# aliftffd/ViT-vs-Raw-IQ

Measured on AMD Instinct MI355X. Metric: IQ frames/sec training (fwd+loss+bwd+clip+AdamW), higher is better.
Workload: dtype bf16; 1 GPU; ViT-Tiny/16 224x224 C=1 19cls (BASELINE configs[1]); config_id=B, per_gpu_batch=256, global_batch=256, parallelism=dp1, hipgraph=True

## Files before the change

### include/iqvit.h

```cpp
#ifndef IQVIT_H
#define IQVIT_H
#include <stddef.h>
#include <stdint.h>

#ifdef __cplusplus
extern "C" {
#endif

typedef void* iq_stream_t;

enum { IQ_STATUS_OK = 0, IQ_STATUS_ARG = 1, IQ_STATUS_UNSUPPORTED = 2, IQ_STATUS_LAUNCH = 3 };

typedef struct iq_dropout {
  uint64_t seed;
  uint32_t step;
  uint32_t site;
  float p;
  const uint32_t* step_dev;
} iq_dropout_t;
#define IQ_SITE_IMPAIR 0xFFFFFFFFu
#define IQ_SITE_SYNTH 0xFFFFFFFEu

int iq_ln_supported(int D);
int iq_ln_fwd(const void* z, const float* gamma, const float* beta, void* x, float* mean, float* rstd, int M, int D,
              float eps, iq_stream_t stream);
size_t iq_ln_bwd_ws_bytes(int D);
int iq_ln_bwd(const void* dx, const void* z, const float* mean, const float* rstd, const float* gamma, void* dz,
              void* dy, const iq_dropout_t* drop, float* dgamma, float* dbeta, float* ws, int accumulate, int M,
              int D, iq_stream_t stream);
int iq_ln_bwd_partial_rows(int M, int D);

typedef struct iq_epilogue {
  const float* bias;
  int relu;
  const float* pe;
  int tok, seq, cls_off;
  iq_dropout_t drop;
  const void* gate;
  int ldg;
  float gate_scale;
  const void* residual;
  int ldr;
} iq_epilogue_t;
int iq_gemm_bf16_nt(const void* A, int lda, const void* B, int ldb, void* C, int ldc, int M, int N, int K,
                    const iq_epilogue_t* epi, iq_stream_t stream);

int iq_gemm_ln_supported(int D, int K);
int iq_gemm_bf16_ln(const void* A, int lda, const void* W, int ldw, const float* bias, const void* residual, int ldr,
                    const iq_dropout_t* drop, const float* gamma, const float* beta, float eps, void* Z, void* X,
                    float* mean, float* rstd, int M, int D, int K, iq_stream_t stream);

int iq_gemm_lnbwd_supported(int D, int K);
int iq_gemm_lnbwd_partial_rows(int M);
int iq_gemm_bf16_lnbwd(const void* A, int lda, const void* Wt, int ldw, const void* residual, int ldr, const void* z,
                       const float* mean, const float* rstd, const float* gamma, const iq_dropout_t* drop, void* dz,
                       void* dy, float* partial, int M, int D, int K, iq_stream_t stream);

int iq_ffn_chain_supported(int S, int D, int F);
int iq_ffn_chain_bwd_partial_rows(int M);
size_t iq_ffn_chain_gate_bytes(int M, int F);
int iq_ffn_chain_bwd(const void* dO, const void* W2t, const void* gate_bits, float gate_scale, void* gH, const void* W1t,
                     const void* residual, const void* z1, const float* mean, const float* rstd, const float* gamma,
                     const iq_dropout_t* drop, void* dz, void* dy, float* partial, const void* Wot, void* dA, int frames, int S,
                     int D, int F, iq_stream_t stream);
int iq_qkv_dgrad_ffn_chain_bwd(const void* gQKV, const void* Wqkv_t, const void* residual0, const void* z2, const float* mean2,
                               const float* rstd2, const float* gamma2, const iq_dropout_t* drop2, void* dz2, void* dy2, float* partial2,
                               const void* W2t, const void* gate_bits, float gate_scale, void* gH, const void* W1t, const void* residual,
                               const void* z1, const float* mean, const float* rstd, const float* gamma, const iq_dropout_t* drop, void* dz,
                               void* dy, float* partial, const void* Wot, void* dA, int frames, int S, int D, int F, iq_stream_t stream);
int iq_ffn_chain_fwd(const void* X1, const void* W1, const float* b1, const iq_dropout_t* drop1, void* H, const void* W2,
                     const float* b2, const iq_dropout_t* drop2, const float* gamma, const float* beta, float eps, void* Z,
                     void* X, float* mean, float* rstd, void* gate_bits, int frames, int S, int D, int F, iq_stream_t stream);
int iq_attn_out_ffn_chain_fwd(const void* A, const void* Wo, const float* bo, const iq_dropout_t* drop0, const void* R,
                              const float* gamma1, const float* beta1, void* Z1, void* X1, float* mean1, float* rstd1,
                              const void* W1, const float* b1, const iq_dropout_t* drop1, void* H, const void* W2, const float* b2,
                              const iq_dropout_t* drop2, const float* gamma2, const float* beta2, float eps, void* Z2, void* X,
                              float* mean2, float* rstd2, void* gate_bits, const void* Wq, const float* bq, void* Yq, int frames,
                              int S, int D, int F, iq_stream_t stream);

size_t iq_wgrad_ws_bytes(int M, int N, int K);
int iq_gemm_bf16_wgrad(const void* dY, int ldy, const void* X, int ldx, float* dW, float* dbias, int M, int N, int K,
                       float* ws, size_t ws_bytes, int accumulate, iq_stream_t stream);

typedef struct iq_wgrad_problem {
  const void* dY;
  int ldy;
  const void* X;
  int ldx;
  float* dW;
  float* dbias;
  int N, K;
} iq_wgrad_problem_t;
typedef struct iq_reduce_seg {
  const float* partials;
  int rows;
  int64_t row_stride;
  float* out;
  int64_t n;
} iq_reduce_seg_t;
size_t iq_wgrad_grouped_ws_bytes(const iq_wgrad_problem_t* probs, int nprob, int M, int max_workgroups);
int iq_gemm_bf16_wgrad_grouped(const iq_wgrad_problem_t* probs, int nprob, int M, float* ws, size_t ws_bytes,
                               int accumulate, int max_workgroups, const iq_reduce_seg_t* extra, int nextra,
                               iq_stream_t stream);

#define IQ_REDUCE_JOB_SEGS 12
typedef struct iq_reduce_job_seg {
  const float* partials;
  float* out;
  int64_t n;
  int64_t stride;
  int rows;
  int blk0;
  int tall;
} iq_reduce_job_seg_t;
typedef struct iq_reduce_job {
  iq_reduce_job_seg_t seg[IQ_REDUCE_JOB_SEGS];
  int nseg;
  int nblk;
  int accumulate;
} iq_reduce_job_t;
int iq_gemm_bf16_wgrad_grouped_deferred(const iq_wgrad_problem_t* probs, int nprob, int M, float* ws, size_t ws_bytes,
                                        int accumulate, int max_workgroups, const iq_reduce_seg_t* extra, int nextra,
                                        iq_reduce_job_t* job, iq_stream_t stream);
int iq_reduce_job_run(const iq_reduce_job_t* job, iq_stream_t stream);
int iq_gemm_lnbwd_ride_workgroups(int M, int D, int K, int job_blocks);
int iq_gemm_bf16_lnbwd_ride(const void* A, int lda, const void* Wt, int ldw, const void* residual, int ldr, const void* z,
                            const float* mean, const float* rstd, const float* gamma, const iq_dropout_t* drop, void* dz,
                            void* dy, float* partial, int M, int D, int K, const iq_reduce_job_t* job, iq_stream_t stream);

int iq_attn_supported(int S, int dh);
int iq_attn_fwd(const void* qkv, void* out, float* lse, int B, int S, int H, int dh, iq_stream_t stream);
int iq_attn_bwd(const void* qkv, const void* out, const void* dout, const float* lse, void* dqkv, int B, int S, int H,
                int dh, iq_stream_t stream);
int iq_attn_fwd_masked(const void* qkv, void* out, float* lse, const uint8_t* mask, long mask_hstride, int B, int S,
                       int H, int dh, iq_stream_t stream);
int iq_attn_bwd_masked(const void* qkv, const void* out, const void* dout, const float* lse, void* dqkv,
                       const uint8_t* mask, long mask_hstride, int B, int S, int H, int dh, iq_stream_t stream);
int iq_attn_probs(const void* qkv, const float* lse, float* out, long out_bstride, int B, int S, int H, int dh,
                  int rows, int heads, iq_stream_t stream);
int iq_attn_grad_probs(const void* qkv, const float* lse, const void* dout, float* out, long out_bstride, int B, int S,
                       int H, int dh, int rows, int heads, int positive, iq_stream_t stream);
int iq_attn_relevance_step(const void* qkv, const float* lse, const void* dout, const float* r_in, float* r_out, int B,
                           int S, int H, int dh, iq_stream_t stream);

int iq_frames_preprocess(const float* raw, float* out, int n_frames, int len, int take, const float* stats,
                         iq_stream_t stream);
typedef struct iq_impair {
  float phase_lo, phase_hi;
  float cfo_lo, cfo_hi;
  int   rot90;
  int   conj;
  int   shift_max;
  float gain_db_lo, gain_db_hi;
  float snr_db_lo, snr_db_hi;
  uint64_t seed; uint32_t step;
  uint64_t frame_base;
} iq_impair_t;
int iq_frames_impair(const float* raw, float* out, float* drawn, int n_frames, int len, int take, const float* stats,
                     const iq_impair_t* imp, iq_stream_t stream);
#define IQ_SYNTH_MAX_CLASSES 128
#define IQ_SYNTH_MAX_SNRS 64
typedef struct iq_synth_class { int kind; int offset; int count; } iq_synth_class_t;
typedef struct iq_synth {
  const float* points;
  const iq_synth_class_t* classes; int n_classes;
  const float* snrs_db; int n_snrs;
  int balanced;
  uint64_t seed; uint32_t stream;
  uint64_t frame_base;
} iq_synth_t;
int iq_frames_synth(float* raw , int64_t* labels, float* snr ,
                    float* drawn ,
                    int32_t* symbols , int n_frames, int len, const iq_synth_t* par, iq_stream_t stream);
typedef struct iq_waveform {
  const float* points; const iq_synth_class_t* classes; int n_classes;
  const float* snrs_db; int n_snrs; int balanced;
  uint64_t seed; uint32_t stream; uint64_t frame_base;
  int sps;
  int span;
  int n_phase;
  int timing;
  const float* pulse;
  const int32_t* fpulse;
  int n_taps;
  float los;
  float tap_sigma[8];
} iq_waveform_t;
int iq_frames_waveform(float* raw , int64_t* labels, float* snr, float* drawn ,
                       int32_t* symbols , float* taps , int n_frames, int len,
                       const iq_waveform_t* par, iq_stream_t stream);
enum { IQ_RX_GIVEN = 0, IQ_RX_OERDER_MEYR = 1, IQ_RX_ENERGY = 2 };
typedef struct iq_receiver {
  int sps;
  int span;
  int n_frac;
  int mode;
  int normalise;
  const float* table;
  const int32_t* u;
} iq_receiver_t;
int iq_frames_receive(const float* raw , float* sym , float* est ,
                      float* energy , int n_frames, int len, const iq_receiver_t* par, iq_stream_t stream);
int iq_frames_receive_bwd(const float* dsym , const float* sym, const float* est, float* dx ,
                          int n_frames, int len, const iq_receiver_t* par, iq_stream_t stream);
typedef struct iq_spectrogram {
  int n_fft;
  int hop;
  int pad;
  int width;
  int mode;
  float inv_norm, floor, scale, shift;
} iq_spectrogram_t;
int iq_frames_spectrogram(const float* x , const float* table ,
                          float* out , int n_frames, int len, const iq_spectrogram_t* par,
                          iq_stream_t stream);
int iq_frames_spectrogram_bwd(const float* x, const float* table, const float* dout ,
                              float* dx , int n_frames, int len, const iq_spectrogram_t* par,
                              iq_stream_t stream);
typedef struct iq_cyclic {
  int n_fft;
  int hop;
  int pad;
  int columns;
  int kind;
  int mode;
  float inv_norm, floor, scale, shift;
} iq_cyclic_t;
int iq_frames_cyclic(const float* x , const float* table , const float* rot ,
                     float* out , int n_frames, int len, const iq_cyclic_t* par, iq_stream_t stream);
int iq_frames_cyclic_bwd(const float* x, const float* table, const float* rot, const float* dout ,
                         float* dx , int n_frames, int len, const iq_cyclic_t* par, iq_stream_t stream);
typedef struct iq_constellation {
  int height, width;
  int radius;
  int n_frac;
  int mode;
  float x_scale, x_off, y_scale, y_off;
  float inv_norm, floor, scale, shift;
} iq_constellation_t;
int iq_frames_constellation(const float* x , const float* table ,
                            float* out , int n_frames, int len, const iq_constellation_t* par,
                            iq_stream_t stream);
int iq_frames_constellation_bwd(const float* x, const float* table, const float* dout ,
                                float* dx , int n_frames, int len, const iq_constellation_t* par,
                                iq_stream_t stream);
enum { IQ_CR_GIVEN = 0, IQ_CR_ESTIMATE = 1 };
typedef struct iq_carrier {
  int order;
  int n1, n2;
  int k_max;
  int refine;
  int planar;
  int mode;
  const float* t1;
  const float* t2;
  const float* tw;
  const int32_t* fth;
} iq_carrier_t;
int iq_frames_carrier(const float* x, float* out, float* est , int32_t* fth_out ,
                      float* power , int n_frames, int len,
                      const iq_carrier_t* par, iq_stream_t stream);
int iq_frames_carrier_bwd(const float* dout, float* dx, int n_frames, int len, const iq_carrier_t* par, iq_stream_t stream);
enum { IQ_EQ_GIVEN = 0, IQ_EQ_CMA = 1 };
typedef struct iq_equaliser {
  int taps;
  int iters;
  int planar;
  int mode;
  float mu;
  float modulus;
  const float* w;
  const float* w0;
} iq_equaliser_t;
int iq_frames_equalise(const float* x, float* out, float* w_out , float* est , int n_frames,
                       int len, const iq_equaliser_t* par, iq_stream_t stream);
int iq_frames_equalise_bwd(const float* dout, float* dx, int n_frames, int len, const iq_equaliser_t* par, iq_stream_t stream);
enum { IQ_LIK_MAX = 0, IQ_LIK_MEAN = 1 };
typedef struct iq_likelihood {
  const float* points;
  const iq_synth_class_t* classes;
  int n_classes;
  const float* rot;
  int n_rot;
  int planar;
  int mode;
  const float* gain;
} iq_likelihood_t;
int iq_frames_likelihood(const float* x, const float* sigma2 , float* loglik ,
                         float* rot_ll , int* best_rot ,
                         int* pred , int n_frames, int len,
                         const iq_likelihood_t* par, iq_stream_t stream);
enum { IQ_EM_TABLE = 0, IQ_EM_GIVEN = 1 };
typedef struct iq_likelihood_em {
  const float* points;
  const iq_synth_class_t* classes;
  int n_classes;
  const float* starts;
  int n_starts;
  int iters;
  int planar;
  int mode;
  float f0;
  float floor;
  const float* h0;
  const float* v0;
} iq_likelihood_em_t;
int iq_frames_likelihood_em(const float* x, float* loglik , float* h , float* v ,
                            int* best_start , float* start_ll , int* pred ,
                            float* snr_db , int n_frames, int len, const iq_likelihood_em_t* par,
                            iq_stream_t stream);
int iq_frames_likelihood_bwd(const float* x, const float* sigma2 , const float* dloglik ,
                             const float* loglik , const float* rot_ll ,
                             const int* best_rot , float* dx , int n_frames, int len,
                             const iq_likelihood_t* par, iq_stream_t stream);
int iq_frames_likelihood_em_bwd(const float* x, const float* dloglik , const float* h ,
                                const float* v , float* dx , int n_frames, int len,
                                const iq_likelihood_em_t* par, iq_stream_t stream);
typedef struct iq_cumulants {
  int planar;
  const float* sigma2;
  const float* mu;
  const float* w;
  const float* bias;
  int n_classes;
} iq_cumulants_t;
int iq_frames_cumulants(const float* x, float* feat , float* mom ,
                        float* score , int* pred ,
                        int n_frames, int len, const iq_cumulants_t* par, iq_stream_t stream);
int iq_patchify(const float* src, void* patches, int kind, int B, int C, int H, int W, int p, int Kpad,
                iq_stream_t stream);
int iq_cls_rows(const float* cls, const float* pe, void* x0, int B, int S, int D, const iq_dropout_t* drop,
                iq_stream_t stream);
int iq_embed_bwd_gather(const void* dx0, void* demb, float* dcls, int B, int S, int tok, int D, int has_cls,
                        const iq_dropout_t* drop, int accumulate, iq_stream_t stream);
int iq_embed_dgrad(const void* demb, const void* w_bf16, int Kpad, float* dsrc, int kind, int B, int C, int H, int W, int p,
                   int D, iq_stream_t stream);
int iq_linf_step(float* x_adv, const float* grad, const float* x0, float alpha, float eps, float lo, float hi, size_t n,
                 iq_stream_t stream);

int iq_head_fwd(const void* x, const float* ln_g, const float* ln_b, const float* W, const float* b, float* featn,
                float* hstat, float* logits, int B, int S, int D, int K, int pool, iq_stream_t stream);
int iq_ce_fwd_bwd(const float* logits, const int64_t* labels, int B, int K, float smoothing, float denom,
                  float* loss_sum, int32_t* n_correct, float* dlogits, iq_stream_t stream);
int iq_head_bwd(const float* dlogits, const float* featn, const float* hstat, const float* ln_g, const float* ln_b,
                const float* W, float* dW, float* db, float* dln_g, float* dln_b, void* dx, int B, int S, int D, int K,
                int pool, int accumulate, iq_stream_t stream);

size_t iq_gradnorm_ws_bytes(size_t n);
int iq_gradnorm_sq(const float* g, size_t n, float grad_scale, float* ws, float* out, iq_stream_t stream);
int iq_adamw_step(float* p, const float* g, float* m, float* v, void* shadow_bf16, size_t n, float lr, float beta1,
                  float beta2, float eps, float weight_decay, int step, const float* gnorm_sq, float max_norm,
                  float grad_scale, const float* dyn, iq_stream_t stream);
int iq_counter_add(uint32_t* ctr_u32, uint32_t inc_u32, float* ctr_f32, float inc_f32, iq_stream_t stream);
int iq_cast_bf16(const float* src, void* dst, size_t n, iq_stream_t stream);
int iq_transpose_cast_bf16(const float* src, void* dst, int rows, int cols, iq_stream_t stream);

typedef struct iq_model_cfg {
  int kind;
  int in_channels;
  int img_h, img_w, patch;
  int seq_length, conv_k, use_cls;
  int num_classes, d_model, n_head, n_layers, ffn_hidden;
  float drop_prob;
} iq_model_cfg_t;

typedef struct iq_model iq_model_t;

int iq_model_create(const iq_model_cfg_t* cfg, iq_model_t** out);
void iq_model_destroy(iq_model_t* m);
const char* iq_model_last_error(const iq_model_t* m);
int iq_model_tokens(const iq_model_t* m);
size_t iq_model_param_floats(const iq_model_t* m);
int iq_model_param_entries(const iq_model_t* m);
int iq_model_param_entry(const iq_model_t* m, int i, char* name, int name_cap, size_t* offset, int* ndim, int* dims);
size_t iq_model_shadow_bytes(const iq_model_t* m);
size_t iq_model_workspace_bytes(const iq_model_t* m, int batch, int training);
int iq_model_bind(iq_model_t* m, float* params, float* grads, const float* pe, void* shadow);
int iq_model_bind_step_counter(iq_model_t* m, uint32_t* counter);
int iq_model_refresh_shadow(iq_model_t* m, iq_stream_t stream);
int iq_model_refresh_transposed(iq_model_t* m, iq_stream_t stream);
int iq_model_forward(iq_model_t* m, const float* src, int batch, void* workspace, size_t ws_bytes, int training,
                     uint64_t seed, uint32_t step, float* enc_out, float* logits, iq_stream_t stream);
int iq_model_backward(iq_model_t* m, const float* dlogits, const float* denc, int batch, void* workspace,
                      size_t ws_bytes, int accumulate, int stage_hi, int stage_lo, iq_stream_t stream);
int iq_model_grad_range(const iq_model_t* m, int stage_hi, int stage_lo, size_t* off, size_t* len);
#define IQ_BWD_PARAM_GRADS 1
int iq_model_backward_input(iq_model_t* m, const float* dlogits, const float* denc, int batch, void* workspace,
                            size_t ws_bytes, float* dsrc, int flags, iq_stream_t stream);
int iq_model_attention(iq_model_t* m, const void* workspace, size_t ws_bytes, int batch, int layer, int rows,
                       int heads, float* out, long out_bstride, iq_stream_t stream);
int iq_model_attention_rollout(iq_model_t* m, const void* workspace, size_t ws_bytes, int batch, float alpha,
                               float* out, iq_stream_t stream);
int iq_model_attention_relevance(iq_model_t* m, const float* dlogits, int batch, void* workspace, size_t ws_bytes,
                                 float* rel, float* const* maps, int rows, int heads, int positive, long out_bstride,
                                 iq_stream_t stream);

#define IQ_PROF_FAMILIES 8
int iq_prof_enable(int on);
int iq_prof_collect(double* ms, long long* count);
size_t iq_prof_kernels(char* out, size_t cap, int reset);

#ifdef __cplusplus
}
#endif
#endif
```

### vit-vs-raw-iq_amd/_native.py

```python
from __future__ import annotations

import ctypes as C
import os

_HERE = os.path.dirname(os.path.abspath(__file__))
LIB_PATH = os.environ.get("IQ_LIBIQVIT") or os.path.join(_HERE, "libiqvit.so")

BWD_PARAM_GRADS = 1

STATUS = {0: "ok", 1: "invalid argument", 2: "unsupported shape/configuration", 3: "HIP launch error"}


class IqError(RuntimeError):
    pass


class Dropout(C.Structure):
    _fields_ = [("seed", C.c_uint64), ("step", C.c_uint32), ("site", C.c_uint32), ("p", C.c_float),
                ("step_dev", C.c_void_p)]


class Impair(C.Structure):
    _fields_ = [("phase_lo", C.c_float), ("phase_hi", C.c_float), ("cfo_lo", C.c_float), ("cfo_hi", C.c_float),
                ("rot90", C.c_int), ("conj", C.c_int), ("shift_max", C.c_int), ("gain_db_lo", C.c_float),
                ("gain_db_hi", C.c_float), ("snr_db_lo", C.c_float), ("snr_db_hi", C.c_float), ("seed", C.c_uint64),
                ("step", C.c_uint32), ("frame_base", C.c_uint64)]


class SynthClass(C.Structure):
    _fields_ = [("kind", C.c_int), ("offset", C.c_int), ("count", C.c_int)]


class Synth(C.Structure):
    _fields_ = [("points", C.c_void_p), ("classes", C.POINTER(SynthClass)), ("n_classes", C.c_int),
                ("snrs_db", C.POINTER(C.c_float)), ("n_snrs", C.c_int), ("balanced", C.c_int), ("seed", C.c_uint64),
                ("stream", C.c_uint32), ("frame_base", C.c_uint64)]


class Waveform(C.Structure):
    _fields_ = [("points", C.c_void_p), ("classes", C.POINTER(SynthClass)), ("n_classes", C.c_int),
                ("snrs_db", C.POINTER(C.c_float)), ("n_snrs", C.c_int), ("balanced", C.c_int), ("seed", C.c_uint64),
                ("stream", C.c_uint32), ("frame_base", C.c_uint64), ("sps", C.c_int), ("span", C.c_int), ("n_phase", C.c_int),
                ("timing", C.c_int), ("pulse", C.c_void_p), ("fpulse", C.c_void_p), ("n_taps", C.c_int), ("los", C.c_float),
                ("tap_sigma", C.c_float * 8)]


class Receiver(C.Structure):
    _fields_ = [("sps", C.c_int), ("span", C.c_int), ("n_frac", C.c_int), ("mode", C.c_int), ("normalise", C.c_int),
                ("table", C.c_void_p), ("u", C.c_void_p)]


class Spectrogram(C.Structure):
    _fields_ = [("n_fft", C.c_int), ("hop", C.c_int), ("pad", C.c_int), ("width", C.c_int), ("mode", C.c_int),
                ("inv_norm", C.c_float), ("floor", C.c_float), ("scale", C.c_float), ("shift", C.c_float)]


class Constellation(C.Structure):
    _fields_ = [("height", C.c_int), ("width", C.c_int), ("radius", C.c_int), ("n_frac", C.c_int), ("mode", C.c_int),
                ("x_scale", C.c_float), ("x_off", C.c_float), ("y_scale", C.c_float), ("y_off", C.c_float),
                ("inv_norm", C.c_float), ("floor", C.c_float), ("scale", C.c_float), ("shift", C.c_float)]


class Carrier(C.Structure):
    _fields_ = [("order", C.c_int), ("n1", C.c_int), ("n2", C.c_int), ("k_max", C.c_int), ("refine", C.c_int),
                ("planar", C.c_int), ("mode", C.c_int), ("t1", C.c_void_p), ("t2", C.c_void_p), ("tw", C.c_void_p),
                ("fth", C.c_void_p)]


class Equaliser(C.Structure):
    _fields_ = [("taps", C.c_int), ("iters", C.c_int), ("planar", C.c_int), ("mode", C.c_int), ("mu", C.c_float),
                ("modulus", C.c_float), ("w", C.c_void_p), ("w0", C.c_void_p)]


class Likelihood(C.Structure):
    _fields_ = [("points", C.c_void_p), ("classes", C.POINTER(SynthClass)), ("n_classes", C.c_int), ("rot", C.c_void_p),
                ("n_rot", C.c_int), ("planar", C.c_int), ("mode", C.c_int), ("gain", C.c_void_p)]


class LikelihoodEm(C.Structure):
    _fields_ = [("points", C.c_void_p), ("classes", C.POINTER(SynthClass)), ("n_classes", C.c_int), ("starts", C.c_void_p),
                ("n_starts", C.c_int), ("iters", C.c_int), ("planar", C.c_int), ("mode", C.c_int), ("f0", C.c_float),
                ("floor", C.c_float), ("h0", C.c_void_p), ("v0", C.c_void_p)]


class Cumulants(C.Structure):
    _fields_ = [("planar", C.c_int), ("sigma2", C.c_void_p), ("mu", C.c_void_p), ("w", C.c_void_p), ("bias", C.c_void_p),
                ("n_classes", C.c_int)]


class Cyclic(C.Structure):
    _fields_ = [("n_fft", C.c_int), ("hop", C.c_int), ("pad", C.c_int), ("columns", C.c_int), ("kind", C.c_int),
                ("mode", C.c_int), ("inv_norm", C.c_float), ("floor", C.c_float), ("scale", C.c_float), ("shift", C.c_float)]


class Epilogue(C.Structure):
    _fields_ = [("bias", C.c_void_p), ("relu", C.c_int), ("pe", C.c_void_p), ("tok", C.c_int), ("seq", C.c_int),
                ("cls_off", C.c_int), ("drop", Dropout), ("gate", C.c_void_p), ("ldg", C.c_int),
                ("gate_scale", C.c_float), ("residual", C.c_void_p), ("ldr", C.c_int)]


class WgradProblem(C.Structure):
    _fields_ = [("dY", C.c_void_p), ("ldy", C.c_int), ("X", C.c_void_p), ("ldx", C.c_int), ("dW", C.c_void_p),
                ("dbias", C.c_void_p), ("N", C.c_int), ("K", C.c_int)]


class ReduceSeg(C.Structure):
    _fields_ = [("partials", C.c_void_p), ("rows", C.c_int), ("row_stride", C.c_int64), ("out", C.c_void_p),
                ("n", C.c_int64)]


class ReduceJobSeg(C.Structure):
    _fields_ = [("partials", C.c_void_p), ("out", C.c_void_p), ("n", C.c_int64), ("stride", C.c_int64), ("rows", C.c_int),
                ("blk0", C.c_int), ("tall", C.c_int)]


class ReduceJob(C.Structure):
    _fields_ = [("seg", ReduceJobSeg * 12), ("nseg", C.c_int), ("nblk", C.c_int), ("accumulate", C.c_int)]


class ModelCfg(C.Structure):
    _fields_ = [("kind", C.c_int), ("in_channels", C.c_int), ("img_h", C.c_int), ("img_w", C.c_int),
                ("patch", C.c_int), ("seq_length", C.c_int), ("conv_k", C.c_int), ("use_cls", C.c_int),
                ("num_classes", C.c_int), ("d_model", C.c_int), ("n_head", C.c_int), ("n_layers", C.c_int),
                ("ffn_hidden", C.c_int), ("drop_prob", C.c_float)]


_P, _I, _Z, _F = C.c_void_p, C.c_int, C.c_size_t, C.c_float
_U64, _U32 = C.c_uint64, C.c_uint32

SIGNATURES = {
    "iq_ln_supported": (_I, [_I]),
    "iq_ln_fwd": (_I, [_P, _P, _P, _P, _P, _P, _I, _I, _F, _P]),
    "iq_ln_bwd_ws_bytes": (_Z, [_I]),
    "iq_ln_bwd_partial_rows": (_I, [_I, _I]),
    "iq_ln_bwd": (_I, [_P, _P, _P, _P, _P, _P, _P, C.POINTER(Dropout), _P, _P, _P, _I, _I, _I, _P]),
    "iq_gemm_bf16_nt": (_I, [_P, _I, _P, _I, _P, _I, _I, _I, _I, C.POINTER(Epilogue), _P]),
    "iq_gemm_ln_supported": (_I, [_I, _I]),
    "iq_gemm_bf16_ln": (_I, [_P, _I, _P, _I, _P, _P, _I, C.POINTER(Dropout), _P, _P, _F, _P, _P, _P, _P, _I, _I, _I, _P]),
    "iq_gemm_lnbwd_supported": (_I, [_I, _I]),
    "iq_gemm_lnbwd_partial_rows": (_I, [_I]),
    "iq_gemm_bf16_lnbwd": (_I, [_P, _I, _P, _I, _P, _I, _P, _P, _P, _P, C.POINTER(Dropout), _P, _P, _P, _I, _I, _I, _P]),
    "iq_ffn_chain_supported": (_I, [_I, _I, _I]),
    "iq_ffn_chain_bwd_partial_rows": (_I, [_I]),
    "iq_ffn_chain_bwd": (_I, [_P, _P, _P, _F, _P, _P, _P, _P, _P, _P, _P, C.POINTER(Dropout), _P, _P, _P, _P, _P, _I, _I, _I, _I, _P]),
    "iq_qkv_dgrad_ffn_chain_bwd": (_I, [_P, _P, _P, _P, _P, _P, _P, C.POINTER(Dropout), _P, _P, _P,
                                        _P, _P, _F, _P, _P, _P, _P, _P, _P, _P, C.POINTER(Dropout), _P, _P, _P, _P, _P, _I, _I, _I, _I, _P]),
    "iq_ffn_chain_gate_bytes": (_Z, [_I, _I]),
    "iq_ffn_chain_fwd": (_I, [_P, _P, _P, C.POINTER(Dropout), _P, _P, _P, C.POINTER(Dropout), _P, _P, _F, _P, _P, _P, _P, _P, _I, _I,
                              _I, _I, _P]),
    "iq_attn_out_ffn_chain_fwd": (_I, [_P, _P, _P, C.POINTER(Dropout), _P, _P, _P, _P, _P, _P, _P,
                                       _P, _P, C.POINTER(Dropout), _P, _P, _P, C.POINTER(Dropout), _P, _P, _F, _P, _P, _P, _P, _P,
                                       _P, _P, _P, _I, _I, _I, _I, _P]),
    "iq_wgrad_ws_bytes": (_Z, [_I, _I, _I]),
    "iq_gemm_bf16_wgrad": (_I, [_P, _I, _P, _I, _P, _P, _I, _I, _I, _P, _Z, _I, _P]),
    "iq_wgrad_grouped_ws_bytes": (_Z, [_P, _I, _I, _I]),
    "iq_gemm_bf16_wgrad_grouped": (_I, [_P, _I, _I, _P, _Z, _I, _I, _P, _I, _P]),
    "iq_gemm_bf16_wgrad_grouped_deferred": (_I, [_P, _I, _I, _P, _Z, _I, _I, _P, _I, C.POINTER(ReduceJob), _P]),
    "iq_reduce_job_run": (_I, [C.POINTER(ReduceJob), _P]),
    "iq_gemm_bf16_lnbwd_ride": (_I, [_P, _I, _P, _I, _P, _I, _P, _P, _P, _P, C.POINTER(Dropout), _P, _P, _P, _I, _I, _I,
                                     C.POINTER(ReduceJob), _P]),
    "iq_gemm_lnbwd_ride_workgroups": (_I, [_I, _I, _I, _I]),
    "iq_attn_supported": (_I, [_I, _I]),
    "iq_attn_fwd": (_I, [_P, _P, _P, _I, _I, _I, _I, _P]),
    "iq_attn_bwd": (_I, [_P, _P, _P, _P, _P, _I, _I, _I, _I, _P]),
    "iq_attn_fwd_masked": (_I, [_P, _P, _P, _P, C.c_long, _I, _I, _I, _I, _P]),
    "iq_attn_bwd_masked": (_I, [_P, _P, _P, _P, _P, _P, C.c_long, _I, _I, _I, _I, _P]),
    "iq_attn_probs": (_I, [_P, _P, _P, C.c_long, _I, _I, _I, _I, _I, _I, _P]),
    "iq_attn_grad_probs": (_I, [_P, _P, _P, _P, C.c_long, _I, _I, _I, _I, _I, _I, _I, _P]),
    "iq_attn_relevance_step": (_I, [_P, _P, _P, _P, _P, _I, _I, _I, _I, _P]),
    "iq_frames_preprocess": (_I, [_P, _P, _I, _I, _I, C.POINTER(C.c_float), _P]),
    "iq_frames_impair": (_I, [_P, _P, _P, _I, _I, _I, C.POINTER(C.c_float), C.POINTER(Impair), _P]),
    "iq_frames_synth": (_I, [_P, _P, _P, _P, _P, _I, _I, C.POINTER(Synth), _P]),
    "iq_frames_waveform": (_I, [_P, _P, _P, _P, _P, _P, _I, _I, C.POINTER(Waveform), _P]),
    "iq_frames_receive": (_I, [_P, _P, _P, _P, _I, _I, C.POINTER(Receiver), _P]),
    "iq_frames_receive_bwd": (_I, [_P, _P, _P, _P, _I, _I, C.POINTER(Receiver), _P]),
    "iq_frames_spectrogram": (_I, [_P, _P, _P, _I, _I, C.POINTER(Spectrogram), _P]),
    "iq_frames_spectrogram_bwd": (_I, [_P, _P, _P, _P, _I, _I, C.POINTER(Spectrogram), _P]),
    "iq_frames_cyclic": (_I, [_P, _P, _P, _P, _I, _I, C.POINTER(Cyclic), _P]),
    "iq_frames_cyclic_bwd": (_I, [_P, _P, _P, _P, _P, _I, _I, C.POINTER(Cyclic), _P]),
    "iq_frames_constellation": (_I, [_P, _P, _P, _I, _I, C.POINTER(Constellation), _P]),
    "iq_frames_constellation_bwd": (_I, [_P, _P, _P, _P, _I, _I, C.POINTER(Constellation), _P]),
    "iq_frames_carrier": (_I, [_P, _P, _P, _P, _P, _I, _I, C.POINTER(Carrier), _P]),
    "iq_frames_carrier_bwd": (_I, [_P, _P, _I, _I, C.POINTER(Carrier), _P]),
    "iq_frames_equalise": (_I, [_P, _P, _P, _P, _I, _I, C.POINTER(Equaliser), _P]),
    "iq_frames_equalise_bwd": (_I, [_P, _P, _I, _I, C.POINTER(Equaliser), _P]),
    "iq_frames_likelihood": (_I, [_P, _P, _P, _P, _P, _P, _I, _I, C.POINTER(Likelihood), _P]),
    "iq_frames_likelihood_em": (_I, [_P, _P, _P, _P, _P, _P, _P, _P, _I, _I, C.POINTER(LikelihoodEm), _P]),
    "iq_frames_likelihood_bwd": (_I, [_P, _P, _P, _P, _P, _P, _P, _I, _I, C.POINTER(Likelihood), _P]),
    "iq_frames_likelihood_em_bwd": (_I, [_P, _P, _P, _P, _P, _I, _I, C.POINTER(LikelihoodEm), _P]),
    "iq_frames_cumulants": (_I, [_P, _P, _P, _P, _P, _I, _I, C.POINTER(Cumulants), _P]),
    "iq_patchify": (_I, [_P, _P, _I, _I, _I, _I, _I, _I, _I, _P]),
    "iq_cls_rows": (_I, [_P, _P, _P, _I, _I, _I, C.POINTER(Dropout), _P]),
    "iq_embed_bwd_gather": (_I, [_P, _P, _P, _I, _I, _I, _I, _I, C.POINTER(Dropout), _I, _P]),
    "iq_embed_dgrad": (_I, [_P, _P, _I, _P, _I, _I, _I, _I, _I, _I, _I, _P]),
    "iq_linf_step": (_I, [_P, _P, _P, _F, _F, _F, _F, _Z, _P]),
    "iq_head_fwd": (_I, [_P, _P, _P, _P, _P, _P, _P, _P, _I, _I, _I, _I, _I, _P]),
    "iq_ce_fwd_bwd": (_I, [_P, _P, _I, _I, _F, _F, _P, _P, _P, _P]),
    "iq_head_bwd": (_I, [_P, _P, _P, _P, _P, _P, _P, _P, _P, _P, _P, _I, _I, _I, _I, _I, _I, _P]),
    "iq_gradnorm_ws_bytes": (_Z, [_Z]),
    "iq_gradnorm_sq": (_I, [_P, _Z, _F, _P, _P, _P]),
    "iq_adamw_step": (_I, [_P, _P, _P, _P, _P, _Z, _F, _F, _F, _F, _F, _I, _P, _F, _F, _P, _P]),
    "iq_counter_add": (_I, [_P, _U32, _P, _F, _P]),
    "iq_cast_bf16": (_I, [_P, _P, _Z, _P]),
    "iq_transpose_cast_bf16": (_I, [_P, _P, _I, _I, _P]),
    "iq_model_create": (_I, [C.POINTER(ModelCfg), C.POINTER(_P)]),
    "iq_model_destroy": (None, [_P]),
    "iq_model_last_error": (C.c_char_p, [_P]),
    "iq_model_tokens": (_I, [_P]),
    "iq_model_param_floats": (_Z, [_P]),
    "iq_model_param_entries": (_I, [_P]),
    "iq_model_param_entry": (_I, [_P, _I, C.c_char_p, _I, C.POINTER(_Z), C.POINTER(_I), C.POINTER(_I)]),
    "iq_model_shadow_bytes": (_Z, [_P]),
    "iq_model_workspace_bytes": (_Z, [_P, _I, _I]),
    "iq_model_bind": (_I, [_P, _P, _P, _P, _P]),
    "iq_model_bind_step_counter": (_I, [_P, _P]),
    "iq_model_refresh_shadow": (_I, [_P, _P]),
    "iq_model_refresh_transposed": (_I, [_P, _P]),
    "iq_model_forward": (_I, [_P, _P, _I, _P, _Z, _I, _U64, _U32, _P, _P, _P]),
    "iq_model_backward": (_I, [_P, _P, _P, _I, _P, _Z, _I, _I, _I, _P]),
    "iq_model_grad_range": (_I, [_P, _I, _I, C.POINTER(_Z), C.POINTER(_Z)]),
    "iq_model_backward_input": (_I, [_P, _P, _P, _I, _P, _Z, _P, _I, _P]),
    "iq_model_attention": (_I, [_P, _P, _Z, _I, _I, _I, _I, _P, C.c_long, _P]),
    "iq_model_attention_rollout": (_I, [_P, _P, _Z, _I, _F, _P, _P]),
    "iq_model_attention_relevance": (_I, [_P, _P, _I, _P, _Z, _P, C.POINTER(_P), _I, _I, _I, C.c_long, _P]),
    "iq_prof_enable": (_I, [_I]),
    "iq_prof_collect": (_I, [C.POINTER(C.c_double), C.POINTER(C.c_longlong)]),
    "iq_prof_kernels": (_Z, [C.c_char_p, _Z, _I]),
}

_lib = None


def lib():
    global _lib
    if _lib is None:
        if not os.path.exists(LIB_PATH):
            raise IqError(
                f"{LIB_PATH} not found: the HIP extension is not built. Run "
                "`python -c 'import __graft_entry__ as g; g.build()'` (or `make -C vit-vs-raw-iq_amd/csrc`). "
                "There is no CPU fallback.")
        L = C.CDLL(LIB_PATH)
        for name, (res, args) in SIGNATURES.items():
            fn = getattr(L, name)
            fn.restype = res
            fn.argtypes = args
        _lib = L
    return _lib


def check(rc, what, model=None):
    if rc != 0:
        detail = ""
        if model is not None:
            msg = lib().iq_model_last_error(model)
            if msg:
                detail = ": " + msg.decode()
        raise IqError(f"{what} failed: {STATUS.get(rc, rc)}{detail}")


def ptr(t):
    return None if t is None else t.data_ptr()


def stream_handle():
    import torch
    return torch.cuda.current_stream().cuda_stream
```

### vit-vs-raw-iq_amd/csrc/ffn_chain.hip

```cpp
#include <stdlib.h>

#include <type_traits>

#include "common.h"
#include "iqvit.h"
#include "prof.h"

namespace {

constexpr int FC_CHUNK = 64, FC_NS = 3, FC_MAXW = 7;

struct FfnChainParams {
  const bf16* X1; const bf16* W1; const bf16* W2;
  const float* b1; const float* b2; const float* gamma; const float* beta;
  bf16* H; bf16* Z; bf16* X; float* mean; float* rstd;
  uint32_t* gate;
  int M, F;
  float eps;
  int drop1_on, drop2_on; IqRng rng1, rng2; uint32_t thresh1, thresh2; float dscale1, dscale2;
  const bf16* A0; const bf16* W0; const bf16* R0; const float* b0; const float* gamma0; const float* beta0;
  bf16* Z0; bf16* X1out; float* mean0; float* rstd0;
  int drop0_on; IqRng rng0; uint32_t thresh0; float dscale0;
  const bf16* Wq; const float* bq; bf16* Yq;
};

template <int CPR> __device__ __forceinline__ int fc_swz(int row, int ch) {
  return CPR == 16 ? (ch ^ (row & 15)) : CPR == 8 ? (ch ^ ((row >> 1) & 7)) : ((ch & ~7) | ((ch & 7) ^ ((row >> 1) & 7)));
}
template <int OFF>
__device__ __forceinline__ void lds_read128(bf16x8& dst, uint32_t addr) {
  asm volatile("ds_read_b128 %0, %1 offset:%2" : "=v"(dst) : "v"(addr), "n"(OFF));
}
#define FC_LGKM_WAIT(N)                                  \
  do {                                                   \
    asm volatile("s_waitcnt lgkmcnt(%0)" ::"n"(N) : "memory"); \
    __builtin_amdgcn_sched_barrier(0);                   \
  } while (0)

__device__ __forceinline__ int fc_kperm(int g) { return ((g & 1) << 1) | (g >> 1); }

template <int D, int NW, int RG, bool DROP1, int MODE>
__global__ __launch_bounds__(NW * 64, 2) void ffn_chain_fwd_kernel(const FfnChainParams p) {
  constexpr int RW = 16 * RG;
  constexpr bool PRE = MODE >= 1, POST = MODE == 2;
  constexpr int XCPR = D / 8;
  constexpr int KS1 = D / 32;
  constexpr int NT2 = D / 16, NP2 = NT2 / 2;
  constexpr int W1_BYTES = FC_CHUNK * D * 2, W2_BYTES = D * FC_CHUNK * 2, SLOT = W1_BYTES + W2_BYTES;
  constexpr int W1_PIECES = W1_BYTES / 1024, PIECES = SLOT / 1024;
  constexpr int PPW = (PIECES + NW - 1) / NW;
  static_assert(PPW + 8 * RG < 64, "counted vmcnt");
  extern __shared__ __attribute__((aligned(16))) unsigned char smem[];
  const int tid = threadIdx.x, lane = tid & 63;
  const int wave = __builtin_amdgcn_readfirstlane(tid >> 6);
  constexpr int nwave = NW;
  const int g = lane >> 4, c16 = lane & 15;
  const bool odd = (g & 1) != 0;
  const int F = p.F;
  const int nchunk = F / FC_CHUNK;
  const long row0 = ((long)blockIdx.x * nwave + wave) * RW;
  const bool have = row0 < p.M;

  auto issue_chunk = [&](int c) {
    unsigned char* slot = smem + (c % FC_NS) * SLOT;
    const char* base1 = reinterpret_cast<const char*>(p.W1 + (long)c * FC_CHUNK * D);
    const char* base2 = reinterpret_cast<const char*>(p.W2 + (long)c * FC_CHUNK);
    int ln = lane;
    asm volatile("" : "+v"(ln));
#pragma unroll
    for (int i = 0; i < PPW; ++i) {
      const int pc = min(wave + i * NW, PIECES - 1);
      const int lin = pc * 64 + ln;
      unsigned off;
      if (pc < W1_PIECES) {
        const int r = lin / XCPR, sl = lin - r * XCPR;
        const int q = fc_swz<XCPR>(r, sl);
        off = (unsigned)((r * D + ((q & ~3) | fc_kperm(q & 3)) * 8) * 2);
      } else {
        const int l2 = lin - W1_PIECES * 64;
        const int r = l2 >> 3, sl = l2 & 7;
        const int q = fc_swz<8>(r, sl);
        off = (unsigned)((r * F + ((q & ~3) | fc_kperm(q & 3)) * 8) * 2);
      }
      const char* base = pc < W1_PIECES ? base1 : base2;
      __builtin_amdgcn_global_load_lds((gbl_cvoid_t*)(base + off), (lds_void_t*)(slot + pc * 1024), 16, 0, 0);
    }
  };
  constexpr int NBQ = 3 * D / FC_CHUNK, NQ = (NBQ + 1) / 2;
  static_assert(2 * W1_BYTES == SLOT, "two projection blocks fill a ring slot");
  const int ntot = nchunk + (POST ? NQ : 0);
  auto issue_any = [&](int c) {
    if (!POST || c < nchunk) { issue_chunk(c); return; }
    const int q = c - nchunk;
    unsigned char* slot = smem + (c % FC_NS) * SLOT;
    int ln = lane;
    asm volatile("" : "+v"(ln));
#pragma unroll
    for (int i = 0; i < PPW; ++i) {
      const int pc = min(wave + i * NW, PIECES - 1);
      const int lin = pc * 64 + ln;
      const int r = lin / XCPR, sl = lin - r * XCPR;
      const int qq = fc_swz<XCPR>(r & 63, sl);
      const int grow = min(q * 2 * FC_CHUNK + r, 3 * D - 1);
      const unsigned off = (unsigned)((grow * D + ((qq & ~3) | fc_kperm(qq & 3)) * 8) * 2);
      __builtin_amdgcn_global_load_lds((gbl_cvoid_t*)(reinterpret_cast<const char*>(p.Wq) + off), (lds_void_t*)(slot + pc * 1024), 16, 0, 0);
    }
  };
  constexpr int NB0 = D / FC_CHUNK;
  if (PRE) {
    constexpr int PRE_PIECES = NB0 * W1_PIECES, PRE_PPW = (PRE_PIECES + NW - 1) / NW;
    static_assert(NB0 * W1_BYTES <= 2 * SLOT, "projection weight blocks fit ring slots 1 and 2");
#pragma unroll
    for (int i = 0; i < PRE_PPW; ++i) {
      const int pc = min(wave + i * NW, PRE_PIECES - 1);
      const int lin = pc * 64 + lane;
      const int r = lin / XCPR, sl = lin - r * XCPR;
      const int q = fc_swz<XCPR>(r & 63, sl);
      const unsigned off = (unsigned)((r * D + ((q & ~3) | fc_kperm(q & 3)) * 8) * 2);
      __builtin_amdgcn_global_load_lds((gbl_cvoid_t*)(reinterpret_cast<const char*>(p.W0) + off),
                                       (lds_void_t*)(smem + SLOT + pc * 1024), 16, 0, 0);
    }
  }
  issue_chunk(0);
  if (!PRE && ntot > 1) issue_any(1);

  bf16x8 xf[RG][KS1];
  {
    const bf16* src = PRE ? p.A0 : p.X1;
#pragma unroll
    for (int rg = 0; rg < RG; ++rg) {
      const long r = min(row0 + rg * 16 + c16, (long)p.M - 1);
#pragma unroll
      for (int ks = 0; ks < KS1; ++ks)
        xf[rg][ks] = have ? *reinterpret_cast<const bf16x8*>(src + r * D + 32 * ks + 8 * fc_kperm(g)) : bf16x8{};
    }
  }
  bf16x8 res0[PRE ? RG : 1][PRE ? KS1 : 1];
  if (PRE) {
#pragma unroll
    for (int rg = 0; rg < RG; ++rg) {
      const long r = min(row0 + rg * 16 + c16, (long)p.M - 1);
#pragma unroll
      for (int jp = 0; jp < KS1; ++jp)
        res0[rg][jp] = have ? *reinterpret_cast<const bf16x8*>(p.R0 + r * D + 32 * jp + 8 * fc_kperm(g)) : bf16x8{};
    }
  }
  const IqRng rng1 = DROP1 ? rng_resolve(p.rng1) : p.rng1;
  const IqRng rng2 = p.drop2_on ? rng_resolve(p.rng2) : p.rng2;
  float* b1s = reinterpret_cast<float*>(smem + FC_NS * SLOT);
  float* vecs = b1s + F;
  for (int i = tid; i < F / 4; i += NW * 64) reinterpret_cast<f32x4*>(b1s)[i] = reinterpret_cast<const f32x4*>(p.b1)[i];
  for (int i = tid; i < (PRE ? 6 : 3) * (D / 4); i += NW * 64) {
    const int v = i / (D / 4), j = i - v * (D / 4);
    const float* src = v == 0 ? p.b2 : v == 1 ? p.gamma : v == 2 ? p.beta : v == 3 ? p.b0 : v == 4 ? p.gamma0 : p.beta0;
    reinterpret_cast<f32x4*>(vecs)[i] = reinterpret_cast<const f32x4*>(src)[j];
  }
  if (POST)
    for (int i = tid; i < 3 * D / 4; i += NW * 64) reinterpret_cast<f32x4*>(vecs + 6 * D)[i] = reinterpret_cast<const f32x4*>(p.bq)[i];
  asm volatile("s_waitcnt vmcnt(0)" ::: "memory");
#pragma unroll
  for (int rg = 0; rg < RG; ++rg)
#pragma unroll
    for (int ks = 0; ks < KS1; ++ks) asm volatile("" : "+v"(xf[rg][ks]));
  if (PRE) {
#pragma unroll
    for (int rg = 0; rg < RG; ++rg)
#pragma unroll
      for (int jp = 0; jp < KS1; ++jp) asm volatile("" : "+v"(res0[rg][jp]));
  }

  const uint32_t lds0 = (uint32_t)(uintptr_t)(lds_void_t*)smem;
  constexpr int W1_KMASK = XCPR == 24 ? 1 : KS1 - 1;
  uint32_t w1off[KS1], w2off[2];
  auto w1at = [&](int ks) -> uint32_t { return w1off[ks & W1_KMASK] + (XCPR == 24 ? 128u * (uint32_t)(ks >> 1) : 0u); };
#pragma unroll
  for (int ks = 0; ks < KS1; ++ks) w1off[ks] = (uint32_t)(c16 * (D * 2) + fc_swz<XCPR>(c16, 4 * (ks & W1_KMASK) + g) * 16);
#pragma unroll
  for (int jp = 0; jp < 2; ++jp) w2off[jp] = (uint32_t)(W1_BYTES + c16 * 128 + fc_swz<8>(c16, 4 * jp + g) * 16);

  if (PRE) {
    __syncthreads();
    if (have) {
      const IqRng rng0 = p.drop0_on ? rng_resolve(p.rng0) : p.rng0;
      bf16x8 zb[RG][KS1];
#pragma unroll
      for (int b = 0; b < NB0; ++b) {
#pragma unroll
        for (int jp = 0; jp < 2; ++jp) {
          const int col = 32 * (2 * b + jp) + (odd ? 16 + 4 * (g - 1) : 4 * g);
          f32x4 acc1[RG][2];
#pragma unroll
          for (int rg = 0; rg < RG; ++rg) { acc1[rg][0] = f32x4{0.f, 0.f, 0.f, 0.f}; acc1[rg][1] = f32x4{0.f, 0.f, 0.f, 0.f}; }
          bf16x8 wp[2][2];
          const uint32_t blk = lds0 + SLOT + b * W1_BYTES;
          auto read_w0 = [&](int ks, bf16x8 (&dst)[2]) {
            const uint32_t a0 = blk + w1at(ks);
            if (jp == 0) { lds_read128<0 * 16 * D * 2>(dst[0], a0); lds_read128<1 * 16 * D * 2>(dst[1], a0); }
            else { lds_read128<2 * 16 * D * 2>(dst[0], a0); lds_read128<3 * 16 * D * 2>(dst[1], a0); }
          };
          read_w0(0, wp[0]);
#pragma unroll
          for (int ks = 0; ks < KS1; ++ks) {
            if (ks + 1 < KS1) { read_w0(ks + 1, wp[(ks + 1) & 1]); FC_LGKM_WAIT(2); }
            else FC_LGKM_WAIT(0);
#pragma unroll
            for (int t = 0; t < 2; ++t) {
#pragma unroll
              for (int rg = 0; rg < RG; ++rg)
                acc1[rg][t] = __builtin_amdgcn_mfma_f32_16x16x32_bf16(wp[ks & 1][t], xf[rg][ks], acc1[rg][t], 0, 0, 0);
            }
            __builtin_amdgcn_sched_barrier(0);
          }
          const f32x4 b_lo = *reinterpret_cast<const f32x4*>(vecs + 3 * D + col), b_hi = *reinterpret_cast<const f32x4*>(vecs + 3 * D + col + 4);
#pragma unroll
          for (int rg = 0; rg < RG; ++rg) {
            float w[8];
#pragma unroll
            for (int r = 0; r < 4; ++r) {
              const float va = acc1[rg][0][r], vb = acc1[rg][1][r];
              const auto sw = __builtin_amdgcn_permlane16_swap(__float_as_uint(va), __float_as_uint(vb), false, false);
              w[r] = __uint_as_float(sw[0]) + b_lo[r];
              w[4 + r] = __uint_as_float(sw[1]) + b_hi[r];
            }
            const long grow = row0 + rg * 16 + c16;
            if (p.drop0_on) {
              const uint32_t keep = dropout_keep8(rng0, (uint64_t)(grow * D + col) >> 3, p.thresh0);
#pragma unroll
              for (int e = 0; e < 8; ++e) w[e] = ((keep >> e) & 1u) ? w[e] * p.dscale0 : 0.f;
            }
#pragma unroll
            for (int e = 0; e < 8; ++e) w[e] += (float)res0[rg][2 * b + jp][e];
            zb[rg][2 * b + jp] = pack8(w);
            if (grow < p.M) *reinterpret_cast<bf16x8*>(p.Z0 + grow * D + col) = zb[rg][2 * b + jp];
          }
        }
      }
      const float invD0 = 1.0f / (float)D;
#pragma unroll
      for (int rg = 0; rg < RG; ++rg) {
        const long grow = row0 + rg * 16 + c16;
        float s1 = 0.f;
#pragma unroll
        for (int jp = 0; jp < KS1; ++jp)
#pragma unroll
          for (int e = 0; e < 8; ++e) s1 += (float)zb[rg][jp][e];
        s1 += __shfl_xor(s1, 16, 64);
        s1 += __shfl_xor(s1, 32, 64);
        const float mean = s1 * invD0;
        float s2 = 0.f;
#pragma unroll
        for (int jp = 0; jp < KS1; ++jp)
#pragma unroll
          for (int e = 0; e < 8; ++e) { const float d = (float)zb[rg][jp][e] - mean; s2 += d * d; }
        s2 += __shfl_xor(s2, 16, 64);
        s2 += __shfl_xor(s2, 32, 64);
        const float rstd = 1.0f / sqrtf(s2 * invD0 + p.eps);
        if (g == 0 && grow < p.M) { p.mean0[grow] = mean; p.rstd0[grow] = rstd; }
#pragma unroll
        for (int jp = 0; jp < KS1; ++jp) {
          const int col = 32 * jp + (odd ? 16 + 4 * (g - 1) : 4 * g);
          const f32x4 g_lo = *reinterpret_cast<const f32x4*>(vecs + 4 * D + col), g_hi = *reinterpret_cast<const f32x4*>(vecs + 4 * D + col + 4);
          const f32x4 e_lo = *reinterpret_cast<const f32x4*>(vecs + 5 * D + col), e_hi = *reinterpret_cast<const f32x4*>(vecs + 5 * D + col + 4);
          float y[8];
#pragma unroll
          for (int e = 0; e < 4; ++e) {
            y[e] = g_lo[e] * (((float)zb[rg][jp][e] - mean) * rstd) + e_lo[e];
            y[4 + e] = g_hi[e] * (((float)zb[rg][jp][4 + e] - mean) * rstd) + e_hi[e];
          }
          xf[rg][jp] = pack8(y);
          if (grow < p.M) *reinterpret_cast<bf16x8*>(p.X1out + grow * D + col) = xf[rg][jp];
        }
      }
    }
    __syncthreads();
    if (ntot > 1) issue_any(1);
#pragma unroll
    for (int rg = 0; rg < RG; ++rg)
#pragma unroll
      for (int ks = 0; ks < KS1; ++ks) asm volatile("" : "+v"(xf[rg][ks]));
  }

  f32x4 acc2[RG][NT2];
#pragma unroll
  for (int rg = 0; rg < RG; ++rg)
#pragma unroll
    for (int j = 0; j < NT2; ++j) acc2[rg][j] = f32x4{0.f, 0.f, 0.f, 0.f};
  const bool full = row0 + RW <= p.M;
  const bool gated = p.gate != nullptr;
  for (int c = 0; c < nchunk; ++c) {
#ifdef FC_NO_RING
    if (c > 0) goto ring_done;
#endif
    if (c == 0) asm volatile("s_waitcnt lgkmcnt(0)" ::: "memory");
    else if (!full || nchunk < 3) asm volatile("s_waitcnt vmcnt(0)" ::: "memory");
    else if (gated && c + 1 < ntot) asm volatile("s_waitcnt vmcnt(%0)" :: "n"(PPW + 4 * RG + 2) : "memory");
    else if (gated) asm volatile("s_waitcnt vmcnt(%0)" :: "n"(4 * RG + 2) : "memory");
    else if (c + 1 < ntot) asm volatile("s_waitcnt vmcnt(%0)" :: "n"(PPW + 4 * RG) : "memory");
    else asm volatile("s_waitcnt vmcnt(%0)" :: "n"(4 * RG) : "memory");
    __builtin_amdgcn_s_barrier();
    asm volatile("" ::: "memory");
    if (c + 2 < ntot) issue_any(c + 2);
#ifdef FC_NO_RING
  ring_done:
#endif
    if (!have) continue;
    const int f0 = c * FC_CHUNK;
    const uint32_t slot_addr = lds0 + (c % FC_NS) * SLOT;
    bf16x8 hf[RG][2];
    uint32_t gbits = 0;
    bf16x8 wp[2][2];
#pragma unroll
    for (int jp = 0; jp < 2; ++jp) {
      f32x4 acc1[RG][2];
#pragma unroll
      for (int rg = 0; rg < RG; ++rg) { acc1[rg][0] = f32x4{0.f, 0.f, 0.f, 0.f}; acc1[rg][1] = f32x4{0.f, 0.f, 0.f, 0.f}; }
      auto read_w1 = [&](int ks, bf16x8 (&dst)[2]) {
        const uint32_t a0 = slot_addr + w1at(ks);
        if (jp == 0) { lds_read128<0 * 16 * D * 2>(dst[0], a0); lds_read128<1 * 16 * D * 2>(dst[1], a0); }
        else { lds_read128<2 * 16 * D * 2>(dst[0], a0); lds_read128<3 * 16 * D * 2>(dst[1], a0); }
      };
      read_w1(0, wp[0]);
#pragma unroll
      for (int ks = 0; ks < KS1; ++ks) {
        if (ks + 1 < KS1) { read_w1(ks + 1, wp[(ks + 1) & 1]); FC_LGKM_WAIT(2); }
        else FC_LGKM_WAIT(0);
#pragma unroll
        for (int t = 0; t < 2; ++t) {
#ifdef FC_NO_MFMA
          asm volatile("" :: "v"(wp[ks & 1][t]));
#else
#pragma unroll
          for (int rg = 0; rg < RG; ++rg)
            acc1[rg][t] = __builtin_amdgcn_mfma_f32_16x16x32_bf16(wp[ks & 1][t], xf[rg][ks], acc1[rg][t], 0, 0, 0);
#endif
        }
        __builtin_amdgcn_sched_barrier(0);
      }
      const int col = f0 + 32 * jp + (odd ? 16 + 4 * (g - 1) : 4 * g);
      const f32x4 b_lo = *reinterpret_cast<const f32x4*>(b1s + col), b_hi = *reinterpret_cast<const f32x4*>(b1s + col + 4);
#pragma unroll
      for (int rg = 0; rg < RG; ++rg) {
        float w[8];
#pragma unroll
        for (int r = 0; r < 4; ++r) {
          const float va = acc1[rg][0][r], vb = acc1[rg][1][r];
          const auto sw = __builtin_amdgcn_permlane16_swap(__float_as_uint(va), __float_as_uint(vb), false, false);
          w[r] = fmaxf(__uint_as_float(sw[0]) + b_lo[r], 0.f);
          w[4 + r] = fmaxf(__uint_as_float(sw[1]) + b_hi[r], 0.f);
        }
        const long grow = row0 + rg * 16 + c16;
        if (DROP1) {
          const uint32_t keep = dropout_keep8(rng1, (uint64_t)(grow * F + col) >> 3, p.thresh1);
#pragma unroll
          for (int e = 0; e < 8; ++e) w[e] = ((keep >> e) & 1u) ? w[e] * p.dscale1 : 0.f;
        }
        hf[rg][jp] = pack8(w);
#pragma unroll
        for (int e = 0; e < 8; ++e) gbits |= (w[e] > 0.f ? 1u : 0u) << (8 * (2 * jp + rg) + e);
#ifndef FC_NO_HSTORE
        if (grow < p.M) *reinterpret_cast<bf16x8*>(p.H + grow * F + col) = hf[rg][jp];
#endif
      }
    }
    {
      if (gated) p.gate[((row0 / RW) * nchunk + c) * 64 + lane] = gbits;
    }
    constexpr int NG4 = NT2 / 4, NGRP = 2 * NG4;
    bf16x8 wq[2][4];
    auto read_w2 = [&](auto qc, bf16x8 (&dst)[4]) {
      constexpr int q = decltype(qc)::value;
      constexpr int jp = q / NG4, j0 = 4 * (q % NG4);
      const uint32_t a0 = slot_addr + w2off[jp];
      lds_read128<(j0 + 0) * 16 * 128>(dst[0], a0);
      lds_read128<(j0 + 1) * 16 * 128>(dst[1], a0);
      lds_read128<(j0 + 2) * 16 * 128>(dst[2], a0);
      lds_read128<(j0 + 3) * 16 * 128>(dst[3], a0);
    };
    auto p2 = [&](auto self, auto qc) -> void {
      constexpr int q = decltype(qc)::value;
      if constexpr (q < NGRP) {
        if constexpr (q + 1 < NGRP) { read_w2(std::integral_constant<int, q + 1>{}, wq[(q + 1) & 1]); FC_LGKM_WAIT(4); }
        else FC_LGKM_WAIT(0);
        constexpr int jp = q / NG4, j0 = 4 * (q % NG4);
#pragma unroll
        for (int t = 0; t < 4; ++t) {
#ifdef FC_NO_MFMA
          asm volatile("" :: "v"(wq[q & 1][t]), "v"(hf[0][jp]), "v"(hf[RG - 1][jp]));
#else
#pragma unroll
          for (int rg = 0; rg < RG; ++rg)
            acc2[rg][j0 + t] = __builtin_amdgcn_mfma_f32_16x16x32_bf16(wq[q & 1][t], hf[rg][jp], acc2[rg][j0 + t], 0, 0, 0);
#endif
        }
        __builtin_amdgcn_sched_barrier(0);
        self(self, std::integral_constant<int, q + 1>{});
      }
    };
    read_w2(std::integral_constant<int, 0>{}, wq[0]);
    p2(p2, std::integral_constant<int, 0>{});
  }
  if (!POST && !have) return;

  const float invD = 1.0f / (float)D;
  if (have) {
#pragma unroll
  for (int rg = 0; rg < RG; ++rg) {
    const long grow = row0 + rg * 16 + c16;
    float z[NP2][8];
    float s1 = 0.f;
#pragma unroll
    for (int jp = 0; jp < NP2; ++jp) {
      const int col = 32 * jp + (odd ? 16 + 4 * (g - 1) : 4 * g);
      const f32x4 b_lo = *reinterpret_cast<const f32x4*>(vecs + col), b_hi = *reinterpret_cast<const f32x4*>(vecs + col + 4);
      float w[8];
#pragma unroll
      for (int r = 0; r < 4; ++r) {
        const float va = acc2[rg][2 * jp][r], vb = acc2[rg][2 * jp + 1][r];
        const auto sw = __builtin_amdgcn_permlane16_swap(__float_as_uint(va), __float_as_uint(vb), false, false);
        w[r] = __uint_as_float(sw[0]) + b_lo[r];
        w[4 + r] = __uint_as_float(sw[1]) + b_hi[r];
      }
      if (p.drop2_on) {
        const uint32_t keep = dropout_keep8(rng2, (uint64_t)(grow * D + col) >> 3, p.thresh2);
#pragma unroll
        for (int e = 0; e < 8; ++e) w[e] = ((keep >> e) & 1u) ? w[e] * p.dscale2 : 0.f;
      }
#pragma unroll
      for (int e = 0; e < 8; ++e) w[e] += (float)xf[rg][jp][e];
      const bf16x8 zb = pack8(w);
      if (grow < p.M) *reinterpret_cast<bf16x8*>(p.Z + grow * D + col) = zb;
      unpack8(zb, z[jp]);
#pragma unroll
      for (int e = 0; e < 8; ++e) s1 += z[jp][e];
    }
    s1 += __shfl_xor(s1, 16, 64);
    s1 += __shfl_xor(s1, 32, 64);
    const float mean = s1 * invD;
    float s2 = 0.f;
#pragma unroll
    for (int jp = 0; jp < NP2; ++jp)
#pragma unroll
      for (int e = 0; e < 8; ++e) { const float d = z[jp][e] - mean; s2 += d * d; }
    s2 += __shfl_xor(s2, 16, 64);
    s2 += __shfl_xor(s2, 32, 64);
    const float rstd = 1.0f / sqrtf(s2 * invD + p.eps);
    if (grow < p.M) {
      if (g == 0) { p.mean[grow] = mean; p.rstd[grow] = rstd; }
#pragma unroll
      for (int jp = 0; jp < NP2; ++jp) {
        const int col = 32 * jp + (odd ? 16 + 4 * (g - 1) : 4 * g);
        const f32x4 g_lo = *reinterpret_cast<const f32x4*>(vecs + D + col), g_hi = *reinterpret_cast<const f32x4*>(vecs + D + col + 4);
        const f32x4 e_lo = *reinterpret_cast<const f32x4*>(vecs + 2 * D + col), e_hi = *reinterpret_cast<const f32x4*>(vecs + 2 * D + col + 4);
        float y[8];
#pragma unroll
        for (int e = 0; e < 4; ++e) {
          y[e] = g_lo[e] * ((z[jp][e] - mean) * rstd) + e_lo[e];
          y[4 + e] = g_hi[e] * ((z[jp][4 + e] - mean) * rstd) + e_hi[e];
        }
        const bf16x8 yb = pack8(y);
        *reinterpret_cast<bf16x8*>(p.X + grow * D + col) = yb;
        if (POST) xf[rg][jp] = yb;
      }
    }
  }
  }
  if (!POST) return;

  for (int q = 0; q < NQ; ++q) {
    const int c = nchunk + q;
    if (q == 0 || !full) asm volatile("s_waitcnt vmcnt(0)" ::: "memory");
    else if (c + 1 < ntot) asm volatile("s_waitcnt vmcnt(%0)" :: "n"(PPW + 8 * RG) : "memory");
    else asm volatile("s_waitcnt vmcnt(%0)" :: "n"(8 * RG) : "memory");
    __builtin_amdgcn_s_barrier();
    asm volatile("" ::: "memory");
    if (c + 2 < ntot) issue_any(c + 2);
    if (!have) continue;
    const uint32_t slot_addr = lds0 + (c % FC_NS) * SLOT;
#pragma unroll
    for (int bl = 0; bl < 2; ++bl) {
      if (2 * q + bl >= NBQ) break;
#pragma unroll
      for (int jp = 0; jp < 2; ++jp) {
        f32x4 acc1[RG][2];
#pragma unroll
        for (int rg = 0; rg < RG; ++rg) { acc1[rg][0] = f32x4{0.f, 0.f, 0.f, 0.f}; acc1[rg][1] = f32x4{0.f, 0.f, 0.f, 0.f}; }
        bf16x8 wp[2][2];
        const uint32_t blk = slot_addr + bl * W1_BYTES;
        auto read_wq = [&](int ks, bf16x8 (&dst)[2]) {
          const uint32_t a0 = blk + w1at(ks);
          if (jp == 0) { lds_read128<0 * 16 * D * 2>(dst[0], a0); lds_read128<1 * 16 * D * 2>(dst[1], a0); }
          else { lds_read128<2 * 16 * D * 2>(dst[0], a0); lds_read128<3 * 16 * D * 2>(dst[1], a0); }
        };
        read_wq(0, wp[0]);
#pragma unroll
        for (int ks = 0; ks < KS1; ++ks) {
          if (ks + 1 < KS1) { read_wq(ks + 1, wp[(ks + 1) & 1]); FC_LGKM_WAIT(2); }
          else FC_LGKM_WAIT(0);
#pragma unroll
          for (int t = 0; t < 2; ++t) {
#pragma unroll
            for (int rg = 0; rg < RG; ++rg)
              acc1[rg][t] = __builtin_amdgcn_mfma_f32_16x16x32_bf16(wp[ks & 1][t], xf[rg][ks], acc1[rg][t], 0, 0, 0);
          }
          __builtin_amdgcn_sched_barrier(0);
        }
        const int col = FC_CHUNK * (2 * q + bl) + 32 * jp + (odd ? 16 + 4 * (g - 1) : 4 * g);
        const f32x4 b_lo = *reinterpret_cast<const f32x4*>(vecs + 6 * D + col), b_hi = *reinterpret_cast<const f32x4*>(vecs + 6 * D + col + 4);
#pragma unroll
        for (int rg = 0; rg < RG; ++rg) {
          float w[8];
#pragma unroll
          for (int r = 0; r < 4; ++r) {
            const float va = acc1[rg][0][r], vb = acc1[rg][1][r];
            const auto sw = __builtin_amdgcn_permlane16_swap(__float_as_uint(va), __float_as_uint(vb), false, false);
            w[r] = __uint_as_float(sw[0]) + b_lo[r];
            w[4 + r] = __uint_as_float(sw[1]) + b_hi[r];
          }
          const long grow = row0 + rg * 16 + c16;
          if (grow < p.M) *reinterpret_cast<bf16x8*>(p.Yq + grow * (3 * D) + col) = pack8(w);
        }
      }
    }
  }
}

struct FfnChainBwdParams {
  const bf16* dO; const bf16* W2t; const bf16* W1t;
  const uint32_t* gate; const bf16* R; const bf16* Z1;
  const float* mean; const float* rstd; const float* gamma;
  bf16* gH; bf16* dZ; bf16* dY; float* partial;
  int M, F;
  float gate_scale;
  int drop_on; IqRng rng; uint32_t thresh; float dscale;
  const bf16* Wot; bf16* dA;
  const bf16* A0; const bf16* W0t; const bf16* R0; const bf16* Z0; const float* mean0; const float* rstd0; const float* gamma0;
  IqRng rng0; bf16* dZ0; bf16* dY0; float* partial0;
};

template <int D, int NW, int RG, bool DROP, int MODE>
__global__ __launch_bounds__(NW * 64, 2) void ffn_chain_bwd_kernel(const FfnChainBwdParams p) {
  constexpr int RW = 16 * RG;
  constexpr bool POSTB = MODE >= 1, PREB = MODE == 2;
  constexpr int XCPR = D / 8;
  constexpr int KS1 = D / 32;
  constexpr int NT2 = D / 16, NP2 = NT2 / 2;
  constexpr int W1_BYTES = FC_CHUNK * D * 2, W2_BYTES = D * FC_CHUNK * 2, SLOT = W1_BYTES + W2_BYTES;
  constexpr int W1_PIECES = W1_BYTES / 1024, PIECES = SLOT / 1024;
  constexpr int PPW = (PIECES + NW - 1) / NW;
  extern __shared__ __attribute__((aligned(16))) unsigned char smem[];
  const int tid = threadIdx.x, lane = tid & 63;
  const int wave = __builtin_amdgcn_readfirstlane(tid >> 6);
  const int g = lane >> 4, c16 = lane & 15;
  const bool odd = (g & 1) != 0;
  const int F = p.F;
  const int nchunk = F / FC_CHUNK;
  const long row0 = ((long)blockIdx.x * NW + wave) * RW;
  const bool have = row0 < p.M;
  const bool full = row0 + RW <= p.M;

  auto issue_chunk = [&](int c) {
    unsigned char* slot = smem + (c % FC_NS) * SLOT;
    const char* base1 = reinterpret_cast<const char*>(p.W2t + (long)c * FC_CHUNK * D);
    const char* base2 = reinterpret_cast<const char*>(p.W1t + (long)c * FC_CHUNK);
#pragma unroll
    for (int i = 0; i < PPW; ++i) {
      const int pc = min(wave + i * NW, PIECES - 1);
      const int lin = pc * 64 + lane;
      unsigned off;
      if (pc < W1_PIECES) {
        const int r = lin / XCPR, sl = lin - r * XCPR;
        const int q = fc_swz<XCPR>(r, sl);
        off = (unsigned)((r * D + ((q & ~3) | fc_kperm(q & 3)) * 8) * 2);
      } else {
        const int l2 = lin - W1_PIECES * 64;
        const int r = l2 >> 3, sl = l2 & 7;
        const int q = fc_swz<8>(r, sl);
        off = (unsigned)((r * F + ((q & ~3) | fc_kperm(q & 3)) * 8) * 2);
      }
      const char* base = pc < W1_PIECES ? base1 : base2;
      __builtin_amdgcn_global_load_lds((gbl_cvoid_t*)(base + off), (lds_void_t*)(slot + pc * 1024), 16, 0, 0);
    }
  };
  long rowc[RG];
#pragma unroll
  for (int rg = 0; rg < RG; ++rg) rowc[rg] = min(row0 + rg * 16 + c16, (long)p.M - 1);
  const uint32_t lds0 = (uint32_t)(uintptr_t)(lds_void_t*)smem;
  constexpr int W1_KMASK = XCPR == 24 ? 1 : KS1 - 1;
  uint32_t w1off[KS1], w2off[2];
  auto w1at = [&](int ks) -> uint32_t { return w1off[ks & W1_KMASK] + (XCPR == 24 ? 128u * (uint32_t)(ks >> 1) : 0u); };
#pragma unroll
  for (int ks = 0; ks < KS1; ++ks) w1off[ks] = (uint32_t)(c16 * (D * 2) + fc_swz<XCPR>(c16, 4 * (ks & W1_KMASK) + g) * 16);
#pragma unroll
  for (int jp = 0; jp < 2; ++jp) w2off[jp] = (uint32_t)(W1_BYTES + c16 * 128 + fc_swz<8>(c16, 4 * jp + g) * 16);

  bf16x8 xf[RG][KS1];
  f32x4 acc2[RG][NT2];
#pragma unroll
  for (int rg = 0; rg < RG; ++rg)
#pragma unroll
    for (int j = 0; j < NT2; ++j) acc2[rg][j] = f32x4{0.f, 0.f, 0.f, 0.f};
  auto second_product = [&](uint32_t img2, bf16x8 (&h)[RG][2]) {
    constexpr int NG4 = NT2 / 4, NGRP = 2 * NG4;
    bf16x8 wq[2][4];
    auto read_w2 = [&](auto qc, bf16x8 (&dst)[4]) {
      constexpr int q = decltype(qc)::value;
      constexpr int jp = q / NG4, j0 = 4 * (q % NG4);
      const uint32_t a0 = img2 + w2off[jp];
      lds_read128<(j0 + 0) * 16 * 128>(dst[0], a0);
      lds_read128<(j0 + 1) * 16 * 128>(dst[1], a0);
      lds_read128<(j0 + 2) * 16 * 128>(dst[2], a0);
      lds_read128<(j0 + 3) * 16 * 128>(dst[3], a0);
    };
    auto p2 = [&](auto self, auto qc) -> void {
      constexpr int q = decltype(qc)::value;
      if constexpr (q < NGRP) {
        if constexpr (q + 1 < NGRP) { read_w2(std::integral_constant<int, q + 1>{}, wq[(q + 1) & 1]); FC_LGKM_WAIT(4); }
        else FC_LGKM_WAIT(0);
        constexpr int jp = q / NG4, j0 = 4 * (q % NG4);
#pragma unroll
        for (int t = 0; t < 4; ++t) {
#pragma unroll
          for (int rg = 0; rg < RG; ++rg)
            acc2[rg][j0 + t] = __builtin_amdgcn_mfma_f32_16x16x32_bf16(wq[q & 1][t], h[rg][jp], acc2[rg][j0 + t], 0, 0, 0);
        }
        __builtin_amdgcn_sched_barrier(0);
        self(self, std::integral_constant<int, q + 1>{});
      }
    };
    read_w2(std::integral_constant<int, 0>{}, wq[0]);
    p2(p2, std::integral_constant<int, 0>{});
  };

  constexpr int LDI = D;
  constexpr int IMG = RW * LDI * 2;
  static_assert(SLOT % IMG == 0 && NW <= 2 * (SLOT / IMG), "whole wave images, all of them in two ring slots");
  auto ln_tail = [&](const bf16* Rp, const bf16* Zp, const float* meanp, const float* rstdp, const float* gammap, const IqRng& rngx,
                     uint32_t thr, float dsc, bf16* dZp, bf16* dYp, bf16* img, float* wsp, auto reload_c) {
    constexpr bool reload = decltype(reload_c)::value;
#pragma unroll
    for (int rg = 0; rg < RG; ++rg) {
      const long gr = min(row0 + rg * 16 + c16, (long)p.M - 1);
  #pragma unroll
      for (int jp = 0; jp < NP2; ++jp) {
        const int col = 32 * jp + (odd ? 16 + 4 * (g - 1) : 4 * g);
        const bf16x8 res = *reinterpret_cast<const bf16x8*>(Rp + gr * D + col);
        float w[8];
  #pragma unroll
        for (int r = 0; r < 4; ++r) {
          const float va = acc2[rg][2 * jp][r], vb = acc2[rg][2 * jp + 1][r];
          const auto sw = __builtin_amdgcn_permlane16_swap(__float_as_uint(va), __float_as_uint(vb), false, false);
          w[r] = __uint_as_float(sw[0]);
          w[4 + r] = __uint_as_float(sw[1]);
        }
  #pragma unroll
        for (int e = 0; e < 8; ++e) w[e] += (float)res[e];
        *reinterpret_cast<bf16x8*>(img + (rg * 16 + c16) * LDI + col) = pack8(w);
      }
    }
    asm volatile("s_waitcnt lgkmcnt(0)" ::: "memory");
    {
      constexpr int LPR = 8, NV = D / (8 * LPR);
      const int lj = lane & 7, rsub = lane >> 3;
      const float invD = 1.0f / (float)D;
      float gmm[NV][8], ag[NV][8], ab[NV][8];
  #pragma unroll
      for (int v = 0; v < NV; ++v) {
        const f32x4 a4 = *reinterpret_cast<const f32x4*>(gammap + (v * LPR + lj) * 8), b4 = *reinterpret_cast<const f32x4*>(gammap + (v * LPR + lj) * 8 + 4);
  #pragma unroll
        for (int e = 0; e < 4; ++e) { gmm[v][e] = a4[e]; gmm[v][4 + e] = b4[e]; }
  #pragma unroll
        for (int e = 0; e < 8; ++e) { ag[v][e] = 0.f; ab[v][e] = 0.f; }
      }
  #pragma unroll 1
      for (int it = 0; it < RW / 8; ++it) {
        const int rl = it * 8 + rsub;
        const long row = row0 + rl;
        const bool ok = row < p.M;
        const long gr = min(row, (long)p.M - 1);
        const float mean = meanp[gr], rstd = rstdp[gr];
        float xh[NV][8], dy[NV][8];
        float s1 = 0.f, s2 = 0.f;
  #pragma unroll
        for (int v = 0; v < NV; ++v) {
          bf16x8 td = *reinterpret_cast<const bf16x8*>(img + rl * LDI + (v * LPR + lj) * 8);
          bf16x8 tz = *reinterpret_cast<const bf16x8*>(Zp + gr * D + (v * LPR + lj) * 8);
          if (!ok) { td = bf16x8{}; tz = bf16x8{}; }
          unpack8(tz, xh[v]);
          unpack8(td, dy[v]);
  #pragma unroll
          for (int e = 0; e < 8; ++e) {
            xh[v][e] = ok ? (xh[v][e] - mean) * rstd : 0.f;
            ag[v][e] += dy[v][e] * xh[v][e];
            ab[v][e] += dy[v][e];
            dy[v][e] *= gmm[v][e];
            s1 += dy[v][e];
            s2 += dy[v][e] * xh[v][e];
          }
        }
  #pragma unroll
        for (int o = LPR / 2; o > 0; o >>= 1) { s1 += __shfl_xor(s1, o, 64); s2 += __shfl_xor(s2, o, 64); }
        const float c1 = s1 * invD, c2 = s2 * invD;
        if (ok) {
  #pragma unroll
          for (int v = 0; v < NV; ++v) {
            float o[8];
  #pragma unroll
            for (int e = 0; e < 8; ++e) o[e] = rstd * (dy[v][e] - c1 - xh[v][e] * c2);
            const long off = row * D + (v * LPR + lj) * 8;
            bf16x8 ob = pack8(o);
            *reinterpret_cast<bf16x8*>(dZp + off) = ob;
            if (DROP) {
              const uint32_t keep = dropout_keep8(rngx, (uint64_t)off >> 3, thr);
  #pragma unroll
              for (int e = 0; e < 8; ++e) o[e] = ((keep >> e) & 1u) ? o[e] * dsc : 0.f;
              ob = pack8(o);
              *reinterpret_cast<bf16x8*>(dYp + off) = ob;
            }
            if (reload) *reinterpret_cast<bf16x8*>(img + rl * LDI + (v * LPR + lj) * 8) = ob;
          }
        }
      }
      if (reload) {
        asm volatile("s_waitcnt lgkmcnt(0)" ::: "memory");
  #pragma unroll
        for (int rg = 0; rg < RG; ++rg)
  #pragma unroll
          for (int ks = 0; ks < KS1; ++ks)
            xf[rg][ks] = *reinterpret_cast<const bf16x8*>(img + (rg * 16 + c16) * LDI + 32 * ks + 8 * fc_kperm(g));
      }
      float* prow = wsp;
  #pragma unroll
      for (int v = 0; v < NV; ++v) {
  #pragma unroll
        for (int e = 0; e < 8; ++e) {
          float a = ag[v][e], b2 = ab[v][e];
  #pragma unroll
          for (int o = 8; o < 64; o <<= 1) { a += __shfl_xor(a, o, 64); b2 += __shfl_xor(b2, o, 64); }
          ag[v][e] = a; ab[v][e] = b2;
        }
        if (rsub == 0) {
          const int c = (v * LPR + lj) * 8;
          *reinterpret_cast<f32x4*>(prow + c) = f32x4{ag[v][0], ag[v][1], ag[v][2], ag[v][3]};
          *reinterpret_cast<f32x4*>(prow + c + 4) = f32x4{ag[v][4], ag[v][5], ag[v][6], ag[v][7]};
          *reinterpret_cast<f32x4*>(prow + D + c) = f32x4{ab[v][0], ab[v][1], ab[v][2], ab[v][3]};
          *reinterpret_cast<f32x4*>(prow + D + c + 4) = f32x4{ab[v][4], ab[v][5], ab[v][6], ab[v][7]};
        }
      }
    }
};
  float* wsum = reinterpret_cast<float*>(smem + FC_NS * SLOT) + wave * (2 * D);
  auto reduce_partial = [&](float* dst) {
    for (int i = tid; i < 2 * D; i += NW * 64) {
      float t = 0.f;
#pragma unroll
      for (int w = 0; w < NW; ++w) t += reinterpret_cast<const float*>(smem + FC_NS * SLOT)[w * (2 * D) + i];
      dst[(long)blockIdx.x * (2 * D) + i] = t;
    }
  };
  const uint32_t* gate_wave = p.gate + (row0 / RW) * nchunk * 64;
  const uint32_t lane4 = (uint32_t)lane * 4u;
  uint32_t gnext;
  auto load_gate = [&](int c) {
    const uint32_t* src = gate_wave + c * 64;
    asm volatile("s_nop 4\n\tglobal_load_dword %0, %1, %2" : "=v"(gnext) : "v"(lane4), "s"(src) : "memory");
  };
  const uint32_t gh_lane = (uint32_t)((c16 * F + (odd ? 16 + 4 * (g - 1) : 4 * g)) * 2);
  const IqRng rng = DROP ? rng_resolve(p.rng) : p.rng;

  if (PREB) {
    constexpr int K0 = 3 * D, NC0 = K0 / FC_CHUNK, NQ0 = (NC0 + 1) / 2;
    auto issue_pre = [&](int i) {
      unsigned char* slot = smem + (i % FC_NS) * SLOT;
      int ln = lane;
      asm volatile("" : "+v"(ln));
#pragma unroll
      for (int k = 0; k < PPW; ++k) {
        const int pc = min(wave + k * NW, PIECES - 1);
        const int h = pc >= W1_PIECES ? 1 : 0;
        const int l2 = (pc - h * W1_PIECES) * 64 + ln;
        const int r = l2 >> 3, sl = l2 & 7;
        const int q = fc_swz<8>(r, sl);
        const int col = min((2 * i + h) * FC_CHUNK, K0 - FC_CHUNK) + ((q & ~3) | fc_kperm(q & 3)) * 8;
        const unsigned off = (unsigned)((r * K0 + col) * 2);
        __builtin_amdgcn_global_load_lds((gbl_cvoid_t*)(reinterpret_cast<const char*>(p.W0t) + off), (lds_void_t*)(slot + pc * 1024), 16, 0, 0);
      }
    };
    bf16x8 aF[2][2][RG][2];
    auto load_a = [&](int i) {
#pragma unroll
      for (int h = 0; h < 2; ++h) {
        if (2 * i + h >= NC0) break;
#pragma unroll
        for (int rg = 0; rg < RG; ++rg)
#pragma unroll
          for (int jp = 0; jp < 2; ++jp) {
            const bf16* src = p.A0 + rowc[rg] * K0 + (2 * i + h) * FC_CHUNK + 32 * jp + 8 * fc_kperm(g);
            asm volatile("global_load_dwordx4 %0, %1, off" : "=v"(aF[i & 1][h][rg][jp]) : "v"(src) : "memory");
          }
      }
    };
    if (have) load_a(0);
    issue_pre(0);
    if (NQ0 > 1) issue_pre(1);
    const IqRng rng0 = DROP ? rng_resolve(p.rng0) : p.rng0;
#pragma unroll
    for (int i = 0; i < NQ0; ++i) {
      if (i == 0 || i + 1 >= NQ0) asm volatile("s_waitcnt vmcnt(0)" ::: "memory");
      else asm volatile("s_waitcnt vmcnt(%0)" :: "n"(PPW) : "memory");
      __builtin_amdgcn_s_barrier();
      asm volatile("" ::: "memory");
      if (have && i + 1 < NQ0) load_a(i + 1);
      if (i + 2 < NQ0) issue_pre(i + 2);
      if (!have) continue;
      const uint32_t slot_addr = lds0 + (i % FC_NS) * SLOT;
#pragma unroll
      for (int h = 0; h < 2; ++h) {
        if (2 * i + h >= NC0) break;
#pragma unroll
        for (int rg = 0; rg < RG; ++rg)
#pragma unroll
          for (int jp = 0; jp < 2; ++jp) asm volatile("" : "+v"(aF[i & 1][h][rg][jp]));
        second_product(slot_addr + h * W1_BYTES - W1_BYTES, aF[i & 1][h]);
      }
    }
    __syncthreads();
    issue_chunk(0);
    if (have) load_gate(0);
    bf16* img0 = reinterpret_cast<bf16*>(smem + (wave < SLOT / IMG ? SLOT + wave * IMG : 2 * SLOT + (wave - SLOT / IMG) * IMG));
    if (have) ln_tail(p.R0, p.Z0, p.mean0, p.rstd0, p.gamma0, rng0, p.thresh, p.dscale, p.dZ0, p.dY0, img0, wsum, std::true_type{});
    else for (int i = lane; i < 2 * D; i += 64) wsum[i] = 0.f;
    asm volatile("s_waitcnt vmcnt(0)" ::: "memory");
    __syncthreads();
    if (nchunk > 1) issue_chunk(1);
    reduce_partial(p.partial0);
#pragma unroll
    for (int rg = 0; rg < RG; ++rg)
#pragma unroll
      for (int j = 0; j < NT2; ++j) acc2[rg][j] = f32x4{0.f, 0.f, 0.f, 0.f};
  } else {
    issue_chunk(0);
    if (nchunk > 1) issue_chunk(1);
#pragma unroll
    for (int rg = 0; rg < RG; ++rg)
#pragma unroll
      for (int ks = 0; ks < KS1; ++ks)
        xf[rg][ks] = have ? *reinterpret_cast<const bf16x8*>(p.dO + rowc[rg] * D + 32 * ks + 8 * fc_kperm(g)) : bf16x8{};
    if (have) load_gate(0);
    asm volatile("s_waitcnt vmcnt(0)" ::: "memory");
  }
#pragma unroll
  for (int rg = 0; rg < RG; ++rg) {
#pragma unroll
    for (int ks = 0; ks < KS1; ++ks) asm volatile("" : "+v"(xf[rg][ks]));
  }
  asm volatile("" : "+v"(gnext));

  for (int c = 0; c < nchunk; ++c) {
    if (c > 0) {
      if (full) asm volatile("s_waitcnt vmcnt(%0)" :: "n"(2 * RG) : "memory");
      else asm volatile("s_waitcnt vmcnt(0)" ::: "memory");
    }
    __builtin_amdgcn_s_barrier();
    asm volatile("" ::: "memory");
    if (c + 2 < nchunk) issue_chunk(c + 2);
    if (!have) continue;
    asm volatile("" : "+v"(gnext));
    const uint32_t gmask = gnext;
    const int f0 = c * FC_CHUNK;
    const uint32_t slot_addr = lds0 + (c % FC_NS) * SLOT;
    bf16x8 hf[RG][2];
    bf16x8 wp[2][2];
#pragma unroll
    for (int jp = 0; jp < 2; ++jp) {
      f32x4 acc1[RG][2];
#pragma unroll
      for (int rg = 0; rg < RG; ++rg) { acc1[rg][0] = f32x4{0.f, 0.f, 0.f, 0.f}; acc1[rg][1] = f32x4{0.f, 0.f, 0.f, 0.f}; }
      auto read_w1 = [&](int ks, bf16x8 (&dst)[2]) {
        const uint32_t a0 = slot_addr + w1at(ks);
        if (jp == 0) { lds_read128<0 * 16 * D * 2>(dst[0], a0); lds_read128<1 * 16 * D * 2>(dst[1], a0); }
        else { lds_read128<2 * 16 * D * 2>(dst[0], a0); lds_read128<3 * 16 * D * 2>(dst[1], a0); }
      };
      read_w1(0, wp[0]);
#pragma unroll
      for (int ks = 0; ks < KS1; ++ks) {
        if (ks + 1 < KS1) { read_w1(ks + 1, wp[(ks + 1) & 1]); FC_LGKM_WAIT(2); }
        else FC_LGKM_WAIT(0);
#pragma unroll
        for (int t = 0; t < 2; ++t) {
#pragma unroll
          for (int rg = 0; rg < RG; ++rg)
            acc1[rg][t] = __builtin_amdgcn_mfma_f32_16x16x32_bf16(wp[ks & 1][t], xf[rg][ks], acc1[rg][t], 0, 0, 0);
        }
        __builtin_amdgcn_sched_barrier(0);
      }
#pragma unroll
      for (int rg = 0; rg < RG; ++rg) {
        float w[8];
#pragma unroll
        for (int r = 0; r < 4; ++r) {
          const float va = acc1[rg][0][r], vb = acc1[rg][1][r];
          const auto sw = __builtin_amdgcn_permlane16_swap(__float_as_uint(va), __float_as_uint(vb), false, false);
          w[r] = __uint_as_float(sw[0]);
          w[4 + r] = __uint_as_float(sw[1]);
        }
#pragma unroll
        for (int e = 0; e < 8; ++e) w[e] = ((gmask >> (8 * (2 * jp + rg) + e)) & 1u) ? w[e] * p.gate_scale : 0.f;
        hf[rg][jp] = pack8(w);
      }
    }
    asm volatile("" ::: "memory");
    if (c + 1 < nchunk) load_gate(c + 1);
#pragma unroll
    for (int rg = 0; rg < RG; ++rg) {
      const bf16* base = p.gH + (row0 + rg * 16) * F + f0;
      if (row0 + rg * 16 + c16 < p.M) {
        asm volatile("s_nop 4\n\tglobal_store_dwordx4 %0, %1, %2\n\tglobal_store_dwordx4 %0, %3, %2 offset:64"
                     :: "v"(gh_lane), "v"(hf[rg][0]), "s"(base), "v"(hf[rg][1]) : "memory");
      }
    }
    second_product(slot_addr, hf);
  }
  const int sC = (nchunk - 1) % FC_NS;
  const int s2 = (sC + 2) % FC_NS, s3 = (sC + 1) % FC_NS;
  bf16* img = reinterpret_cast<bf16*>(smem + (wave < SLOT / IMG ? s2 * SLOT + wave * IMG : s3 * SLOT + (wave - SLOT / IMG) * IMG));
  constexpr int NB0 = D / FC_CHUNK;
  auto issue_wot = [&](int b0, int nb, unsigned char* dst) {
    const int pieces = nb * W1_PIECES;
    for (int pc = wave; pc < pieces; pc += NW) {
      const int lin = pc * 64 + lane;
      const int r = lin / XCPR, sl = lin - r * XCPR;
      const int q = fc_swz<XCPR>(r & 63, sl);
      const unsigned off = (unsigned)(((b0 * FC_CHUNK + r) * D + ((q & ~3) | fc_kperm(q & 3)) * 8) * 2);
      __builtin_amdgcn_global_load_lds((gbl_cvoid_t*)(reinterpret_cast<const char*>(p.Wot) + off), (lds_void_t*)(dst + pc * 1024), 16, 0, 0);
    }
  };
  if (POSTB) {
    __syncthreads();
    issue_wot(0, 2, smem + sC * SLOT);
  }
  if (have) ln_tail(p.R, p.Z1, p.mean, p.rstd, p.gamma, rng, p.thresh, p.dscale, p.dZ, p.dY, img, wsum, std::integral_constant<bool, POSTB>{});
  else for (int i = lane; i < 2 * D; i += 64) wsum[i] = 0.f;
  if (POSTB) asm volatile("s_waitcnt vmcnt(0)" ::: "memory");
  __syncthreads();
  if (POSTB && NB0 > 2) issue_wot(2, NB0 - 2, smem + s2 * SLOT);
  reduce_partial(p.partial);
  if (!POSTB) return;
#pragma unroll
  for (int b = 0; b < NB0; ++b) {
    if (b == 2) {
      asm volatile("s_waitcnt vmcnt(0)" ::: "memory");
      __syncthreads();
    }
    if (!have) continue;
    const uint32_t blk = lds0 + (b < 2 ? sC * SLOT + b * W1_BYTES : s2 * SLOT);
#pragma unroll
    for (int jp = 0; jp < 2; ++jp) {
      f32x4 acc1[RG][2];
#pragma unroll
      for (int rg = 0; rg < RG; ++rg) { acc1[rg][0] = f32x4{0.f, 0.f, 0.f, 0.f}; acc1[rg][1] = f32x4{0.f, 0.f, 0.f, 0.f}; }
      bf16x8 wp[2][2];
      auto read_w = [&](int ks, bf16x8 (&dst)[2]) {
        const uint32_t a0 = blk + w1at(ks);
        if (jp == 0) { lds_read128<0 * 16 * D * 2>(dst[0], a0); lds_read128<1 * 16 * D * 2>(dst[1], a0); }
        else { lds_read128<2 * 16 * D * 2>(dst[0], a0); lds_read128<3 * 16 * D * 2>(dst[1], a0); }
      };
      read_w(0, wp[0]);
#pragma unroll
      for (int ks = 0; ks < KS1; ++ks) {
        if (ks + 1 < KS1) { read_w(ks + 1, wp[(ks + 1) & 1]); FC_LGKM_WAIT(2); }
        else FC_LGKM_WAIT(0);
#pragma unroll
        for (int t = 0; t < 2; ++t) {
#pragma unroll
          for (int rg = 0; rg < RG; ++rg)
            acc1[rg][t] = __builtin_amdgcn_mfma_f32_16x16x32_bf16(wp[ks & 1][t], xf[rg][ks], acc1[rg][t], 0, 0, 0);
        }
        __builtin_amdgcn_sched_barrier(0);
      }
      const int col = FC_CHUNK * b + 32 * jp + (odd ? 16 + 4 * (g - 1) : 4 * g);
#pragma unroll
      for (int rg = 0; rg < RG; ++rg) {
        float w[8];
#pragma unroll
        for (int r = 0; r < 4; ++r) {
          const float va = acc1[rg][0][r], vb = acc1[rg][1][r];
          const auto sw = __builtin_amdgcn_permlane16_swap(__float_as_uint(va), __float_as_uint(vb), false, false);
          w[r] = __uint_as_float(sw[0]);
          w[4 + r] = __uint_as_float(sw[1]);
        }
        const long grow = row0 + rg * 16 + c16;
        if (grow < p.M) *reinterpret_cast<bf16x8*>(p.dA + grow * D + col) = pack8(w);
      }
    }
  }
}

struct ChainShape { int rg, nw; };
inline ChainShape chain_shape(int M) {
  if (M <= 20480) return ChainShape{1, 5};
  if (M <= 32768) return ChainShape{1, 8};
  return ChainShape{2, FC_MAXW};
}
inline int chain_waves(int M) { return chain_shape(M).nw; }
inline long chain_units(int M) { const int rw = 16 * chain_shape(M).rg; return ((long)M + rw - 1) / rw; }

template <int D, int NW, int RG>
int launch_chain(const FfnChainParams& p, hipStream_t st) {
  constexpr int SLOT = 2 * FC_CHUNK * D * 2;
  const size_t lds = (size_t)FC_NS * SLOT + ((size_t)p.F + 9 * D) * sizeof(float);
  const long units = ((long)p.M + 16 * RG - 1) / (16 * RG);
  const int grid = (int)((units + NW - 1) / NW);
#define FC_LAUNCH(DROP_, MODE_)                                                                                               \
  do {                                                                                                                        \
    auto k = ffn_chain_fwd_kernel<D, NW, RG, DROP_, MODE_>;                                                                   \
    static const hipError_t attr = hipFuncSetAttribute((const void*)k, hipFuncAttributeMaxDynamicSharedMemorySize, 160 * 1024); \
    (void)attr;                                                                                                               \
    k<<<grid, NW * 64, lds, st>>>(p);                                                                                         \
  } while (0)
  if (p.A0 && p.Wq) { if (p.drop1_on) FC_LAUNCH(true, 2); else FC_LAUNCH(false, 2); }
  else if (p.A0) { if (p.drop1_on) FC_LAUNCH(true, 1); else FC_LAUNCH(false, 1); }
  else { if (p.drop1_on) FC_LAUNCH(true, 0); else FC_LAUNCH(false, 0); }
#undef FC_LAUNCH
  return iq_launch_status();
}
template <int D>
int launch_chain_d(const FfnChainParams& p, hipStream_t st) {
  const ChainShape sh = chain_shape(p.M);
  if (sh.rg == 2) return launch_chain<D, FC_MAXW, 2>(p, st);
  return sh.nw == 5 ? launch_chain<D, 5, 1>(p, st) : launch_chain<D, 8, 1>(p, st);
}

template <int D, int NW, int RG>
int launch_chain_bwd(const FfnChainBwdParams& p, hipStream_t st) {
  constexpr int SLOT = 2 * FC_CHUNK * D * 2;
  const size_t lds = (size_t)FC_NS * SLOT + (size_t)NW * 2 * D * sizeof(float);
  const long units = ((long)p.M + 16 * RG - 1) / (16 * RG);
  const int grid = (int)((units + NW - 1) / NW);
#define FC_LAUNCHB(DROP_, MODE_)                                                                                              \
  do {                                                                                                                        \
    auto k = ffn_chain_bwd_kernel<D, NW, RG, DROP_, MODE_>;                                                                   \
    static const hipError_t attr = hipFuncSetAttribute((const void*)k, hipFuncAttributeMaxDynamicSharedMemorySize, 160 * 1024); \
    (void)attr;                                                                                                               \
    k<<<grid, NW * 64, lds, st>>>(p);                                                                                         \
  } while (0)
  if (p.A0) { if (p.drop_on) FC_LAUNCHB(true, 2); else FC_LAUNCHB(false, 2); }
  else if (p.Wot) { if (p.drop_on) FC_LAUNCHB(true, 1); else FC_LAUNCHB(false, 1); }
  else { if (p.drop_on) FC_LAUNCHB(true, 0); else FC_LAUNCHB(false, 0); }
#undef FC_LAUNCHB
  return iq_launch_status();
}
template <int D>
int launch_chain_bwd_d(const FfnChainBwdParams& p, hipStream_t st) {
  const ChainShape sh = chain_shape(p.M);
  if (sh.rg == 2) return launch_chain_bwd<D, FC_MAXW, 2>(p, st);
  return sh.nw == 5 ? launch_chain_bwd<D, 5, 1>(p, st) : launch_chain_bwd<D, 8, 1>(p, st);
}

}

extern "C" int iq_ffn_chain_supported(int S, int D, int F) {
  if (!(D == 128 || D == 192) || F < FC_CHUNK || (F % FC_CHUNK) || S <= 0) return 0;
  return (size_t)FC_NS * 2 * FC_CHUNK * D * 2 + ((size_t)F + 9 * D) * sizeof(float) <= (size_t)160 * 1024 ? 1 : 0;
}

namespace {
struct ChainPre {
  const void* A0; const void* W0; const float* b0; const iq_dropout_t* drop0; const void* R0;
  const float* gamma0; const float* beta0; void* Z0; float* mean0; float* rstd0;
  const void* Wq; const float* bq; void* Yq;
};

int chain_fwd(const ChainPre* pre, const void* X1, const void* W1, const float* b1, const iq_dropout_t* drop1, void* H, const void* W2,
              const float* b2, const iq_dropout_t* drop2, const float* gamma, const float* beta, float eps, void* Z, void* X,
              float* mean, float* rstd, void* gate_bits, int frames, int S, int D, int F, iq_stream_t stream) {
  if (frames <= 0) return IQ_OK;
  if (!X1 || !W1 || !b1 || !H || !W2 || !b2 || !gamma || !beta || !Z || !X || !mean || !rstd) return IQ_ERR_ARG;
  if (!iq_ffn_chain_supported(S, D, F)) return IQ_ERR_UNSUPPORTED;
  if (((uintptr_t)X1 | (uintptr_t)W1 | (uintptr_t)W2 | (uintptr_t)H | (uintptr_t)Z | (uintptr_t)X | (uintptr_t)b1 | (uintptr_t)b2 |
       (uintptr_t)gamma | (uintptr_t)beta) % 16) return IQ_ERR_ARG;
  if ((long)frames * S > 0x7FFFFFFFL) return IQ_ERR_UNSUPPORTED;
  FfnChainParams p = {};
  p.X1 = (const bf16*)X1; p.W1 = (const bf16*)W1; p.W2 = (const bf16*)W2;
  p.b1 = b1; p.b2 = b2; p.gamma = gamma; p.beta = beta;
  p.H = (bf16*)H; p.Z = (bf16*)Z; p.X = (bf16*)X; p.mean = mean; p.rstd = rstd;
  p.gate = (uint32_t*)gate_bits;
  if ((uintptr_t)gate_bits % 16) return IQ_ERR_ARG;
  p.M = frames * S; p.F = F; p.eps = eps;
  if (!dropout_unpack(drop1, &p.drop1_on, &p.rng1, &p.thresh1, &p.dscale1) ||
      !dropout_unpack(drop2, &p.drop2_on, &p.rng2, &p.thresh2, &p.dscale2)) return IQ_ERR_ARG;
  if (pre) {
    if (!pre->A0 || !pre->W0 || !pre->b0 || !pre->R0 || !pre->gamma0 || !pre->beta0 || !pre->Z0 || !pre->mean0 || !pre->rstd0)
      return IQ_ERR_ARG;
    if (((uintptr_t)pre->A0 | (uintptr_t)pre->W0 | (uintptr_t)pre->b0 | (uintptr_t)pre->R0 | (uintptr_t)pre->gamma0 |
         (uintptr_t)pre->beta0 | (uintptr_t)pre->Z0) % 16) return IQ_ERR_ARG;
    p.A0 = (const bf16*)pre->A0; p.W0 = (const bf16*)pre->W0; p.R0 = (const bf16*)pre->R0; p.b0 = pre->b0;
    p.gamma0 = pre->gamma0; p.beta0 = pre->beta0; p.Z0 = (bf16*)pre->Z0; p.X1out = (bf16*)X1; p.mean0 = pre->mean0; p.rstd0 = pre->rstd0;
    if (!dropout_unpack(pre->drop0, &p.drop0_on, &p.rng0, &p.thresh0, &p.dscale0)) return IQ_ERR_ARG;
    if (pre->Wq || pre->bq || pre->Yq) {
      if (!pre->Wq || !pre->bq || !pre->Yq || ((uintptr_t)pre->Wq | (uintptr_t)pre->bq | (uintptr_t)pre->Yq) % 16) return IQ_ERR_ARG;
      p.Wq = (const bf16*)pre->Wq; p.bq = pre->bq; p.Yq = (bf16*)pre->Yq;
    }
  }
  hipStream_t st = (hipStream_t)stream;
  IQ_PROF(IQ_FAM_GEMM_NT, st);
  const double M = (double)p.M;
  double more_bytes = 0.0, more_flops = 0.0;
  if (pre) { more_bytes += 2.0 * (M * D * 3 + (double)D * D) + 8.0 * M; more_flops += 2.0 * M * D * D; }
  if (p.Wq) { more_bytes += 2.0 * (M * 3 * D + 3.0 * D * D); more_flops += 6.0 * M * D * D; }
  IQ_PROF_K(2.0 * (M * D * 3 + M * F + 2.0 * D * F) + 8.0 * M + more_bytes, 4.0 * M * D * F + more_flops,
            "ffn_chain_fwd_kernel<%d, %d, %d, %s, %d>", D, chain_waves(p.M), chain_shape(p.M).rg, p.drop1_on ? "true" : "false", p.Wq ? 2 : pre ? 1 : 0);
  return D == 192 ? launch_chain_d<192>(p, st) : launch_chain_d<128>(p, st);
}
}

extern "C" int iq_ffn_chain_fwd(const void* X1, const void* W1, const float* b1, const iq_dropout_t* drop1, void* H,
                                const void* W2, const float* b2, const iq_dropout_t* drop2, const float* gamma,
                                const float* beta, float eps, void* Z, void* X, float* mean, float* rstd, void* gate_bits,
                                int frames, int S, int D, int F, iq_stream_t stream) {
  return chain_fwd(nullptr, X1, W1, b1, drop1, H, W2, b2, drop2, gamma, beta, eps, Z, X, mean, rstd, gate_bits, frames, S, D, F, stream);
}

extern "C" int iq_attn_out_ffn_chain_fwd(const void* A, const void* Wo, const float* bo, const iq_dropout_t* drop0, const void* R,
                                         const float* gamma1, const float* beta1, void* Z1, void* X1, float* mean1, float* rstd1,
                                         const void* W1, const float* b1, const iq_dropout_t* drop1, void* H, const void* W2,
                                         const float* b2, const iq_dropout_t* drop2, const float* gamma2, const float* beta2, float eps,
                                         void* Z2, void* X, float* mean2, float* rstd2, void* gate_bits, const void* Wq,
                                         const float* bq, void* Yq, int frames, int S, int D, int F, iq_stream_t stream) {
  const ChainPre pre = {A, Wo, bo, drop0, R, gamma1, beta1, Z1, mean1, rstd1, Wq, bq, Yq};
  return chain_fwd(&pre, X1, W1, b1, drop1, H, W2, b2, drop2, gamma2, beta2, eps, Z2, X, mean2, rstd2, gate_bits, frames, S, D, F, stream);
}

extern "C" int iq_ffn_chain_bwd_partial_rows(int M) {
  if (M <= 0) return 0;
  const int nw = chain_waves(M);
  return (int)((chain_units(M) + nw - 1) / nw);
}

extern "C" size_t iq_ffn_chain_gate_bytes(int M, int F) {
  if (M <= 0 || F <= 0) return 0;
  return (size_t)chain_units(M) * (size_t)(F / FC_CHUNK) * 64 * sizeof(uint32_t);
}

namespace {
struct ChainBwdPre {
  const void* A0; const void* W0t; const void* R0; const void* Z0; const float* mean0; const float* rstd0; const float* gamma0;
  const iq_dropout_t* drop0; void* dZ0; void* dY0; float* partial0;
};

int chain_bwd(const ChainBwdPre* pre, const void* dO, const void* W2t, const void* gate_bits, float gate_scale, void* gH, const void* W1t,
              const void* residual, const void* z1, const float* mean, const float* rstd, const float* gamma, const iq_dropout_t* drop,
              void* dz, void* dy, float* partial, const void* Wot, void* dA, int frames, int S, int D, int F, iq_stream_t stream) {
  if (frames <= 0) return IQ_OK;
  if ((Wot == nullptr) != (dA == nullptr) || ((uintptr_t)Wot | (uintptr_t)dA) % 16) return IQ_ERR_ARG;
  if ((!pre && !dO) || !W2t || !gate_bits || !gH || !W1t || !residual || !z1 || !mean || !rstd || !gamma || !dz || !partial) return IQ_ERR_ARG;
  if (!iq_ffn_chain_supported(S, D, F)) return IQ_ERR_UNSUPPORTED;
  if (((uintptr_t)dO | (uintptr_t)W2t | (uintptr_t)W1t | (uintptr_t)gate_bits | (uintptr_t)gH | (uintptr_t)residual | (uintptr_t)z1 |
       (uintptr_t)dz | (uintptr_t)dy | (uintptr_t)gamma | (uintptr_t)partial) % 16) return IQ_ERR_ARG;
  if ((long)frames * S > 0x7FFFFFFFL) return IQ_ERR_UNSUPPORTED;
  FfnChainBwdParams p = {};
  p.dO = (const bf16*)dO; p.W2t = (const bf16*)W2t; p.W1t = (const bf16*)W1t;
  p.gate = (const uint32_t*)gate_bits; p.R = (const bf16*)residual; p.Z1 = (const bf16*)z1;
  p.mean = mean; p.rstd = rstd; p.gamma = gamma;
  p.gH = (bf16*)gH; p.dZ = (bf16*)dz; p.dY = (bf16*)dy; p.partial = partial;
  p.M = frames * S; p.F = F; p.gate_scale = gate_scale;
  p.Wot = (const bf16*)Wot; p.dA = (bf16*)dA;
  if (!dropout_unpack(drop, &p.drop_on, &p.rng, &p.thresh, &p.dscale) || (p.drop_on && !dy)) return IQ_ERR_ARG;
  if (pre) {
    if (!Wot) return IQ_ERR_ARG;
    if (!pre->A0 || !pre->W0t || !pre->R0 || !pre->Z0 || !pre->mean0 || !pre->rstd0 || !pre->gamma0 || !pre->dZ0 || !pre->partial0)
      return IQ_ERR_ARG;
    if (((uintptr_t)pre->A0 | (uintptr_t)pre->W0t | (uintptr_t)pre->R0 | (uintptr_t)pre->Z0 | (uintptr_t)pre->gamma0 |
         (uintptr_t)pre->dZ0 | (uintptr_t)pre->dY0 | (uintptr_t)pre->partial0) % 16) return IQ_ERR_ARG;
    const float p0 = pre->drop0 ? pre->drop0->p : 0.f, p1 = drop ? drop->p : 0.f;
    if (p0 != p1 || (p.drop_on && !pre->dY0)) return IQ_ERR_ARG;
    p.A0 = (const bf16*)pre->A0; p.W0t = (const bf16*)pre->W0t; p.R0 = (const bf16*)pre->R0; p.Z0 = (const bf16*)pre->Z0;
    p.mean0 = pre->mean0; p.rstd0 = pre->rstd0; p.gamma0 = pre->gamma0;
    p.dZ0 = (bf16*)pre->dZ0; p.dY0 = (bf16*)pre->dY0; p.partial0 = pre->partial0;
    int on0; uint32_t thresh0; float dscale0;
    (void)dropout_unpack(pre->drop0, &on0, &p.rng0, &thresh0, &dscale0);
  }
  hipStream_t st = (hipStream_t)stream;
  IQ_PROF(IQ_FAM_GEMM_NT, st);
  const double M = (double)p.M;
  double bytes = 2.0 * (M * D * (4 + (p.drop_on ? 1 : 0) + (Wot ? 1 : 0)) + 2.0 * M * F + 2.0 * D * F + (Wot ? (double)D * D : 0.0)) + 8.0 * M;
  double flops = 4.0 * M * D * F + (Wot ? 2.0 * M * D * D : 0.0);
  if (pre) {
    bytes += 2.0 * (M * 3 * D + M * D * (3 + (p.drop_on ? 1 : 0) - 1) + 3.0 * D * D) + 8.0 * M;
    flops += 6.0 * M * D * D;
  }
  IQ_PROF_K(bytes, flops, "ffn_chain_bwd_kernel<%d, %d, %d, %s, %d>", D, chain_waves(p.M), chain_shape(p.M).rg, p.drop_on ? "true" : "false", pre ? 2 : Wot ? 1 : 0);
  return D == 192 ? launch_chain_bwd_d<192>(p, st) : launch_chain_bwd_d<128>(p, st);
}
}

extern "C" int iq_ffn_chain_bwd(const void* dO, const void* W2t, const void* gate_bits, float gate_scale, void* gH, const void* W1t,
                                const void* residual, const void* z1, const float* mean, const float* rstd, const float* gamma,
                                const iq_dropout_t* drop, void* dz, void* dy, float* partial, const void* Wot, void* dA, int frames,
                                int S, int D, int F, iq_stream_t stream) {
  return chain_bwd(nullptr, dO, W2t, gate_bits, gate_scale, gH, W1t, residual, z1, mean, rstd, gamma, drop, dz, dy, partial, Wot, dA,
                   frames, S, D, F, stream);
}

extern "C" int iq_qkv_dgrad_ffn_chain_bwd(const void* gQKV, const void* Wqkv_t, const void* residual0, const void* z2, const float* mean2,
                                          const float* rstd2, const float* gamma2, const iq_dropout_t* drop2, void* dz2, void* dy2,
                                          float* partial2, const void* W2t, const void* gate_bits, float gate_scale, void* gH,
                                          const void* W1t, const void* residual, const void* z1, const float* mean, const float* rstd,
                                          const float* gamma, const iq_dropout_t* drop, void* dz, void* dy, float* partial, const void* Wot,
                                          void* dA, int frames, int S, int D, int F, iq_stream_t stream) {
  const ChainBwdPre pre = {gQKV, Wqkv_t, residual0, z2, mean2, rstd2, gamma2, drop2, dz2, dy2, partial2};
  return chain_bwd(&pre, nullptr, W2t, gate_bits, gate_scale, gH, W1t, residual, z1, mean, rstd, gamma, drop, dz, dy, partial, Wot, dA,
                   frames, S, D, F, stream);
}
```

### vit-vs-raw-iq_amd/csrc/model.hip

```cpp
#include <hip/hip_runtime.h>
#include <stdio.h>
#include <string.h>

#include <string>
#include <vector>

#include "attn_maps.h"
#include "common.h"
#include "iqvit.h"
#include "prof.h"

int head_bwd_dx_launch(const float* dlogits, const float* featn, const float* hstat, const float* ln_g, const float* W, void* dx,
                       int B, int S, int D, int K, int pool, hipStream_t st);
int embed_bwd_gather_launch(const void* dx0, void* demb, int B, int S, int tok, int D, int has_cls, const iq_dropout_t* drop,
                            hipStream_t st);

namespace {

struct Entry {
  std::string name;
  size_t off;
  int ndim;
  int dims[4];
};

struct LayerOff {
  size_t wqkv, bqkv, wo, bo, g1, be1, w1, b1, w2, b2, g2, be2, end;
  size_t t_wqkv, t_wo, t_w1, t_w2;
};

inline size_t align_up(size_t v, size_t a) { return (v + a - 1) / a * a; }

struct WsPlan {
  size_t step_ctr, patches, x0, head_feat, head_stat;
  struct L { size_t qkv, att, lse, z1, mean1, rstd1, x1, hid, gate, z2, mean2, rstd2, x2; };
  std::vector<L> layers;
  size_t gA, gB, gAtt, demb, wgrad_ws, wgrad_ws_bytes, ln_part[3], embw_scratch;
  size_t gZ, gY, gZ1, gY1, gH, gQKV;
  size_t total;
};

__global__ void bf16_to_f32_kernel(const bf16* __restrict__ s, float* __restrict__ d, size_t n8) {
  for (size_t i = (size_t)blockIdx.x * blockDim.x + threadIdx.x; i < n8; i += (size_t)gridDim.x * blockDim.x) {
    const bf16x8 v = reinterpret_cast<const bf16x8*>(s)[i];
    f32x4 a = {(float)v[0], (float)v[1], (float)v[2], (float)v[3]};
    f32x4 b = {(float)v[4], (float)v[5], (float)v[6], (float)v[7]};
    reinterpret_cast<f32x4*>(d)[2 * i] = a;
    reinterpret_cast<f32x4*>(d)[2 * i + 1] = b;
  }
}
__global__ void f32_into_bf16_kernel(const float* __restrict__ s, bf16* __restrict__ d, size_t n8, int add) {
  for (size_t i = (size_t)blockIdx.x * blockDim.x + threadIdx.x; i < n8; i += (size_t)gridDim.x * blockDim.x) {
    const f32x4 a = reinterpret_cast<const f32x4*>(s)[2 * i], b = reinterpret_cast<const f32x4*>(s)[2 * i + 1];
    float f[8] = {a[0], a[1], a[2], a[3], b[0], b[1], b[2], b[3]};
    if (add) {
      const bf16x8 o = reinterpret_cast<const bf16x8*>(d)[i];
#pragma unroll
      for (int e = 0; e < 8; ++e) f[e] += (float)o[e];
    }
    reinterpret_cast<bf16x8*>(d)[i] = pack8(f);
  }
}
__global__ void cast_pad_kernel(const float* __restrict__ s, bf16* __restrict__ d, int rows, int cols, int ld) {
  const long n = (long)rows * ld;
  for (long i = (long)blockIdx.x * blockDim.x + threadIdx.x; i < n; i += (long)gridDim.x * blockDim.x) {
    const int r = (int)(i / ld), c = (int)(i % ld);
    d[i] = (bf16)(c < cols ? s[(long)r * cols + c] : 0.f);
  }
}
__global__ void unpad_kernel(const float* __restrict__ s, float* __restrict__ d, int rows, int cols, int ld, int add) {
  const long n = (long)rows * cols;
  for (long i = (long)blockIdx.x * blockDim.x + threadIdx.x; i < n; i += (long)gridDim.x * blockDim.x) {
    const int r = (int)(i / cols), c = (int)(i % cols);
    const float v = s[(long)r * ld + c];
    d[i] = add ? d[i] + v : v;
  }
}
struct TransDesc { unsigned long long src_off, dst_off; int rows, cols, tile0, tiles_x; };
__global__ __launch_bounds__(256) void transpose_table_kernel(const float* __restrict__ params, unsigned char* __restrict__ shadow,
                                                              const TransDesc* __restrict__ tab, int nent) {
  __shared__ float t[32][33];
  int e = 0;
  while (e + 1 < nent && (int)blockIdx.x >= tab[e + 1].tile0) ++e;
  const TransDesc d = tab[e];
  const int local = blockIdx.x - d.tile0;
  const int bx = (local % d.tiles_x) * 32, by = (local / d.tiles_x) * 32;
  const float* src = params + d.src_off;
  bf16* dst = reinterpret_cast<bf16*>(shadow + d.dst_off);
  const int tx = threadIdx.x & 31, ty = threadIdx.x >> 5;
  for (int i = ty; i < 32; i += 8) {
    const int r = by + i, c = bx + tx;
    t[i][tx] = (r < d.rows && c < d.cols) ? src[(long)r * d.cols + c] : 0.f;
  }
  __syncthreads();
  for (int i = ty; i < 32; i += 8) {
    const int c = bx + i, r = by + tx;
    if (c < d.cols && r < d.rows) dst[(long)c * d.rows + r] = (bf16)t[tx][i];
  }
}

__global__ void rel_start_kernel(float* r, int n, int S, int cls) {
  for (int i = blockIdx.x * blockDim.x + threadIdx.x; i < n; i += gridDim.x * blockDim.x) {
    const int k = i % S;
    r[i] = cls ? (k == 0 ? 1.f : 0.f) : 1.0f / S;
  }
}

struct RelHook {
  float* const* maps;
  int rows, heads, positive;
  long bstride;
  float* rel;
  float* r[2];
};

__global__ void set_u32_kernel(uint32_t* p, uint32_t v, int bump) {
  if (threadIdx.x == 0 && blockIdx.x == 0) *p = bump ? *p + 1u : v;
}

inline int blocks_for(size_t n, int cap = 4096) {
  size_t b = (n + 255) / 256;
  if (b > (size_t)cap) b = cap;
  if (b < 1) b = 1;
  return (int)b;
}

}

struct iq_model {
  iq_model_cfg_t c;
  int S, tok, has_cls, P, Ppad, dh, pool, head_ln;
  std::vector<Entry> entries;
  size_t nparam;
  size_t emb_w, emb_b, cls, emb_end;
  std::vector<LayerOff> L;
  size_t hln_g, hln_b, head_w, head_b, head_begin;
  size_t sh_flat, sh_embw, sh_table, shadow_bytes;
  std::vector<TransDesc> ttab;
  int ttiles = 0;
  const void* table_uploaded_to = nullptr;
  float* params = nullptr;
  float* grads = nullptr;
  const float* pe = nullptr;
  unsigned char* shadow = nullptr;
  std::string err;
  uint32_t* step_ctr = nullptr;
  uint64_t last_seed = 0;
  bool last_tr = false;
  bool last_train_fwd = false;
  const void* fwd_ws = nullptr;
  int fwd_batch = 0;

  iq_dropout_t bwd_site(uint32_t id, const uint32_t* step_dev, bool tr) const {
    iq_dropout_t d;
    d.seed = last_seed; d.step = 0; d.site = id; d.p = tr ? c.drop_prob : 0.f; d.step_dev = step_dev;
    return d;
  }

  size_t add(const std::string& name, std::vector<int> dims, size_t& cur, bool aligned = true) {
    if (aligned) cur = align_up(cur, 64);
    Entry e;
    e.name = name; e.off = cur; e.ndim = (int)dims.size();
    size_t n = 1;
    for (int i = 0; i < 4; ++i) { e.dims[i] = i < e.ndim ? dims[i] : 1; n *= (size_t)e.dims[i]; }
    entries.push_back(e);
    cur += n;
    return e.off;
  }
  const bf16* sh(size_t off) const { return reinterpret_cast<const bf16*>(shadow + sh_flat) + off; }
  const bf16* sht(size_t byte_off) const { return reinterpret_cast<const bf16*>(shadow + byte_off); }
};

namespace {

int fail(iq_model* m, int code, const std::string& msg) {
  if (m) m->err = msg;
  return code;
}

WsPlan plan_ws(const iq_model* m, int B) {
  WsPlan w;
  const size_t D = m->c.d_model, F = m->c.ffn_hidden, S = m->S, H = m->c.n_head;
  const size_t M = (size_t)B * S, MT = (size_t)B * m->tok;
  size_t cur = 0;
  auto take = [&](size_t bytes) { size_t o = cur; cur = align_up(cur + bytes, 256); return o; };
  w.step_ctr = take(256);
  w.patches = take(MT * m->Ppad * 2);
  w.x0 = take(M * D * 2);
  w.head_feat = take((size_t)B * D * 4);
  w.head_stat = take((size_t)B * 2 * 4);
  w.layers.resize(m->c.n_layers);
  for (auto& l : w.layers) {
    l.qkv = take(M * 3 * D * 2);
    l.att = take(M * D * 2);
    l.lse = take((size_t)B * H * S * 4);
    l.z1 = take(M * D * 2);
    l.mean1 = take(M * 4);
    l.rstd1 = take(M * 4);
    l.x1 = take(M * D * 2);
    l.hid = take(M * F * 2);
    l.gate = take(iq_ffn_chain_gate_bytes((int)M, (int)F));
    l.z2 = take(M * D * 2);
    l.mean2 = take(M * 4);
    l.rstd2 = take(M * 4);
    l.x2 = take(M * D * 2);
  }
  w.gA = take(M * D * 2);
  w.gB = take(M * D * 2);
  w.gZ = take(M * D * 2);
  w.gY = take(M * D * 2);
  w.gZ1 = take(M * D * 2);
  w.gY1 = take(M * D * 2);
  w.gH = take(M * F * 2);
  w.gQKV = take(M * 3 * D * 2);
  w.gAtt = take(M * D * 2);
  w.demb = take(MT * D * 2);
  size_t wb = 0;
  auto mx = [&](size_t v) { if (v > wb) wb = v; };
  {
    iq_wgrad_problem_t g[4];
    memset(g, 0, sizeof(g));
    g[0].N = (int)D; g[0].K = (int)F;
    g[1].N = (int)F; g[1].K = (int)D;
    g[2].N = (int)D; g[2].K = (int)D;
    g[3].N = (int)(3 * D); g[3].K = (int)D;
    mx(iq_wgrad_grouped_ws_bytes(g, 4, (int)M, 0));
    for (int k = 0; k < 4; ++k) mx(iq_wgrad_grouped_ws_bytes(g + k, 1, (int)M, 0));
  }
  mx(iq_wgrad_ws_bytes((int)MT, (int)D, m->Ppad));
  w.wgrad_ws_bytes = wb;
  w.wgrad_ws = take(wb);
  size_t ln_rows_fused = (size_t)iq_gemm_lnbwd_partial_rows((int)M);
  if ((size_t)iq_ffn_chain_bwd_partial_rows((int)M) > ln_rows_fused) ln_rows_fused = (size_t)iq_ffn_chain_bwd_partial_rows((int)M);
  ln_rows_fused *= 2 * D * sizeof(float);
  const size_t ln_bytes = ln_rows_fused > iq_ln_bwd_ws_bytes((int)D) ? ln_rows_fused : iq_ln_bwd_ws_bytes((int)D);
  for (int k = 0; k < 3; ++k) w.ln_part[k] = take(ln_bytes);
  w.embw_scratch = take((size_t)D * m->Ppad * 4 + 256);
  w.total = cur;
  return w;
}

inline bool use_fused_ln(int D, int K) { return iq_gemm_ln_supported(D, K) && (D <= 192 || K <= 256); }

struct Route {
  bool chain;
  bool chain_takes_qkv_dgrad;
};
inline Route layer_route(int M, int S, int D, int F) {
  Route r;
  r.chain = iq_ffn_chain_supported(S, D, F) && M >= 8192;
  r.chain_takes_qkv_dgrad = r.chain && M <= 32768;
  return r;
}

#define IQ_TRY(expr, what)                                                              \
  do {                                                                                  \
    int rc_ = (expr);                                                                   \
    if (rc_ != IQ_OK) return fail(m, rc_, std::string(what) + " failed (status " + std::to_string(rc_) + ")"); \
  } while (0)

iq_dropout_t site(const iq_model* m, uint64_t seed, const uint32_t* step_dev, uint32_t id, bool training) {
  iq_dropout_t d;
  d.seed = seed; d.step = 0; d.site = id; d.p = training ? m->c.drop_prob : 0.f; d.step_dev = step_dev;
  return d;
}

}

extern "C" int iq_model_create(const iq_model_cfg_t* cfg, iq_model_t** out) {
  if (!cfg || !out) return IQ_ERR_ARG;
  *out = nullptr;
  iq_model* m = new iq_model();
  m->c = *cfg;
  const iq_model_cfg_t& c = m->c;
  auto bad = [&](const char* msg) { fprintf(stderr, "iq_model_create: %s\n", msg); delete m; return IQ_ERR_UNSUPPORTED; };
  if (c.d_model <= 0 || c.n_head <= 0 || c.n_layers < 0 || c.ffn_hidden <= 0 || c.num_classes <= 0 || c.in_channels <= 0)
    { delete m; return IQ_ERR_ARG; }
  if (c.d_model % c.n_head) return bad("d_model must be divisible by n_head");
  m->dh = c.d_model / c.n_head;
  if (m->dh != 16 && m->dh != 32 && m->dh != 64) return bad("head dim (d_model/n_head) must be 16, 32 or 64");
  if (c.ffn_hidden % 8) return bad("ffn_hidden must be a multiple of 8");
  if (!iq_ln_supported(c.d_model)) return bad("d_model not supported by the LayerNorm kernel");
  if (!(c.drop_prob >= 0.f && c.drop_prob < 1.f)) return bad("drop_prob must be in [0,1)");
  if (c.kind == 0) {
    if (c.patch <= 0 || c.img_h < c.patch || c.img_w < c.patch) return bad("bad image / patch size");
    m->tok = (c.img_h / c.patch) * (c.img_w / c.patch);
    m->has_cls = 1;
    m->P = c.in_channels * c.patch * c.patch;
    m->pool = 0;
    m->head_ln = 0;
  } else if (c.kind == 1) {
    if (c.conv_k <= 0 || c.seq_length < c.conv_k || (c.seq_length % c.conv_k)) return bad("bad seq_length / segment_size");
    m->tok = c.seq_length / c.conv_k;
    m->has_cls = c.use_cls ? 1 : 0;
    m->P = c.in_channels * c.conv_k;
    m->pool = m->has_cls ? 0 : 1;
    m->head_ln = 1;
  } else {
    delete m;
    return IQ_ERR_ARG;
  }
  m->S = m->tok + m->has_cls;
  m->Ppad = (int)align_up((size_t)m->P, 32);
  if (!iq_attn_supported(m->S, m->dh)) return bad("sequence too long for the attention backward kernel at this head dim");

  const int D = c.d_model, F = c.ffn_hidden, K = c.num_classes;
  size_t cur = 0;
  const std::string emb = c.kind == 0 ? "encoder.patch_embedding.projection" : "encoder.sequence_embedding.projection";
  if (c.kind == 0) m->emb_w = m->add(emb + ".weight", {D, c.in_channels, c.patch, c.patch}, cur);
  else m->emb_w = m->add(emb + ".weight", {D, c.in_channels, c.conv_k}, cur);
  m->emb_b = m->add(emb + ".bias", {D}, cur);
  m->cls = 0;
  if (m->has_cls) m->cls = m->add("encoder.cls_token", {1, 1, D}, cur);
  cur = align_up(cur, 64);
  m->emb_end = cur;
  m->L.resize(c.n_layers);
  for (int i = 0; i < c.n_layers; ++i) {
    LayerOff& o = m->L[i];
    const std::string p = "encoder.layers." + std::to_string(i) + ".";
    o.wqkv = m->add(p + "attention.w_q.weight", {D, D}, cur);
    m->add(p + "attention.w_k.weight", {D, D}, cur, false);
    m->add(p + "attention.w_v.weight", {D, D}, cur, false);
    o.bqkv = m->add(p + "attention.w_q.bias", {D}, cur);
    m->add(p + "attention.w_k.bias", {D}, cur, false);
    m->add(p + "attention.w_v.bias", {D}, cur, false);
    o.wo = m->add(p + "attention.w_concat.weight", {D, D}, cur);
    o.bo = m->add(p + "attention.w_concat.bias", {D}, cur);
    o.g1 = m->add(p + "norm1.gamma", {D}, cur);
    o.be1 = m->add(p + "norm1.beta", {D}, cur);
    o.w1 = m->add(p + "ffn.linear1.weight", {F, D}, cur);
    o.b1 = m->add(p + "ffn.linear1.bias", {F}, cur);
    o.w2 = m->add(p + "ffn.linear2.weight", {D, F}, cur);
    o.b2 = m->add(p + "ffn.linear2.bias", {D}, cur);
    o.g2 = m->add(p + "norm2.gamma", {D}, cur);
    o.be2 = m->add(p + "norm2.beta", {D}, cur);
    cur = align_up(cur, 64);
    o.end = cur;
  }
  m->head_begin = cur;
  m->hln_g = m->hln_b = 0;
  if (m->head_ln) {
    m->hln_g = m->add("mlp_head.0.weight", {D}, cur);
    m->hln_b = m->add("mlp_head.0.bias", {D}, cur);
    m->head_w = m->add("mlp_head.1.weight", {K, D}, cur);
    m->head_b = m->add("mlp_head.1.bias", {K}, cur);
  } else {
    m->head_w = m->add("mlp_head.weight", {K, D}, cur);
    m->head_b = m->add("mlp_head.bias", {K}, cur);
  }
  m->nparam = align_up(cur, 64);

  size_t sb = 0;
  m->sh_flat = sb; sb = align_up(sb + m->nparam * 2, 256);
  m->sh_embw = sb; sb = align_up(sb + (size_t)D * m->Ppad * 2, 256);
  for (auto& o : m->L) {
    o.t_wqkv = sb; sb = align_up(sb + (size_t)3 * D * D * 2, 256);
    o.t_wo = sb; sb = align_up(sb + (size_t)D * D * 2, 256);
    o.t_w1 = sb; sb = align_up(sb + (size_t)F * D * 2, 256);
    o.t_w2 = sb; sb = align_up(sb + (size_t)D * F * 2, 256);
  }
  for (auto& o : m->L) {
    auto push = [&](size_t src, size_t dst, int rows, int cols) {
      TransDesc d;
      d.src_off = src; d.dst_off = dst; d.rows = rows; d.cols = cols; d.tile0 = m->ttiles; d.tiles_x = (cols + 31) / 32;
      m->ttiles += d.tiles_x * ((rows + 31) / 32);
      m->ttab.push_back(d);
    };
    push(o.wqkv, o.t_wqkv, 3 * D, D);
    push(o.wo, o.t_wo, D, D);
    push(o.w1, o.t_w1, F, D);
    push(o.w2, o.t_w2, D, F);
  }
  m->sh_table = sb; sb = align_up(sb + m->ttab.size() * sizeof(TransDesc) + 64, 256);
  m->shadow_bytes = sb;
  *out = m;
  return IQ_OK;
}

extern "C" void iq_model_destroy(iq_model_t* m) {
  if (!m) return;
  delete m;
}
extern "C" const char* iq_model_last_error(const iq_model_t* m) { return m ? m->err.c_str() : "null model"; }
extern "C" int iq_model_tokens(const iq_model_t* m) { return m ? m->S : 0; }
extern "C" size_t iq_model_param_floats(const iq_model_t* m) { return m ? m->nparam : 0; }
extern "C" int iq_model_param_entries(const iq_model_t* m) { return m ? (int)m->entries.size() : 0; }
extern "C" int iq_model_param_entry(const iq_model_t* m, int i, char* name, int name_cap, size_t* offset, int* ndim,
                                    int* dims) {
  if (!m || i < 0 || i >= (int)m->entries.size() || !name || name_cap <= 0 || !offset || !ndim || !dims) return IQ_ERR_ARG;
  const Entry& e = m->entries[i];
  snprintf(name, (size_t)name_cap, "%s", e.name.c_str());
  *offset = e.off;
  *ndim = e.ndim;
  for (int k = 0; k < 4; ++k) dims[k] = e.dims[k];
  return IQ_OK;
}
extern "C" size_t iq_model_shadow_bytes(const iq_model_t* m) { return m ? m->shadow_bytes : 0; }
extern "C" size_t iq_model_workspace_bytes(const iq_model_t* m, int batch, int training) {
  (void)training;
  if (!m || batch <= 0) return 0;
  return plan_ws(m, batch).total;
}

extern "C" int iq_model_bind(iq_model_t* m, float* params, float* grads, const float* pe, void* shadow) {
  if (!m) return IQ_ERR_ARG;
  if (!params || !pe || !shadow) return fail(m, IQ_ERR_ARG, "bind: params, pe and shadow are required");
  if (((uintptr_t)params | (uintptr_t)grads | (uintptr_t)shadow) & 255) return fail(m, IQ_ERR_ARG, "bind: buffers must be 256 B aligned");
  m->params = params; m->grads = grads; m->pe = pe; m->shadow = (unsigned char*)shadow;
  if (m->table_uploaded_to != shadow && !m->ttab.empty()) {
    if (hipMemcpy(m->shadow + m->sh_table, m->ttab.data(), m->ttab.size() * sizeof(TransDesc), hipMemcpyHostToDevice) != hipSuccess)
      return fail(m, IQ_ERR_LAUNCH, "bind: uploading the transpose table failed");
    m->table_uploaded_to = shadow;
  }
  return IQ_OK;
}

extern "C" int iq_model_bind_step_counter(iq_model_t* m, uint32_t* counter) {
  if (!m) return IQ_ERR_ARG;
  if ((uintptr_t)counter & 3) return fail(m, IQ_ERR_ARG, "bind_step_counter: counter must be 4 B aligned");
  m->step_ctr = counter;
  return IQ_OK;
}

static int refresh_impl(iq_model_t* m, bool cast_flat, iq_stream_t stream) {
  if (!m || !m->params || !m->shadow) return fail(m, IQ_ERR_ARG, "refresh_shadow: model not bound");
  hipStream_t st = (hipStream_t)stream;
  const int D = m->c.d_model;
  if (cast_flat) IQ_TRY(iq_cast_bf16(m->params, m->shadow + m->sh_flat, m->nparam, stream), "cast params");
  IQ_PROF(IQ_FAM_MISC, st);
  cast_pad_kernel<<<blocks_for((size_t)D * m->Ppad), 256, 0, st>>>(m->params + m->emb_w, (bf16*)(m->shadow + m->sh_embw), D,
                                                                  m->P, m->Ppad);
  if (m->ttiles > 0)
    transpose_table_kernel<<<m->ttiles, 256, 0, st>>>(m->params, m->shadow, (const TransDesc*)(m->shadow + m->sh_table),
                                                     (int)m->ttab.size());
  return iq_launch_status();
}

extern "C" int iq_model_refresh_shadow(iq_model_t* m, iq_stream_t stream) { return refresh_impl(m, true, stream); }
extern "C" int iq_model_refresh_transposed(iq_model_t* m, iq_stream_t stream) { return refresh_impl(m, false, stream); }

extern "C" int iq_model_forward(iq_model_t* m, const float* src, int batch, void* workspace, size_t ws_bytes,
                                int training, uint64_t seed, uint32_t step, float* enc_out, float* logits,
                                iq_stream_t stream) {
  if (!m) return IQ_ERR_ARG;
  if (!m->params || !m->shadow || !m->pe) return fail(m, IQ_ERR_ARG, "forward: model not bound");
  if (!src || !workspace || batch <= 0) return fail(m, IQ_ERR_ARG, "forward: bad arguments");
  if ((uintptr_t)workspace & 255) return fail(m, IQ_ERR_ARG, "forward: workspace must be 256 B aligned");
  const WsPlan w = plan_ws(m, batch);
  if (ws_bytes < w.total) return fail(m, IQ_ERR_ARG, "forward: workspace too small");
  hipStream_t st = (hipStream_t)stream;
  unsigned char* ws = (unsigned char*)workspace;
  const iq_model_cfg_t& c = m->c;
  const int D = c.d_model, F = c.ffn_hidden, S = m->S, H = c.n_head, B = batch;
  const int M = B * S, MT = B * m->tok;
  const Route route = layer_route(M, S, D, F);
  const bool tr = training != 0 && c.drop_prob > 0.f;
  uint32_t* step_dev = m->step_ctr ? m->step_ctr : (uint32_t*)(ws + w.step_ctr);
  m->last_tr = tr;
  m->last_train_fwd = true;
  if (tr) {
    set_u32_kernel<<<1, 64, 0, st>>>(step_dev, step, step == 0xFFFFFFFFu ? 1 : 0);
    m->last_seed = seed;
  }
  const float* P = m->params;
  m->fwd_ws = nullptr;

  if (c.kind == 0) IQ_TRY(iq_patchify(src, ws + w.patches, 0, B, c.in_channels, c.img_h, c.img_w, c.patch, m->Ppad, stream), "patchify");
  else IQ_TRY(iq_patchify(src, ws + w.patches, 1, B, c.in_channels, c.seq_length, 0, c.conv_k, m->Ppad, stream), "patchify");
  const iq_dropout_t d0 = site(m, seed, step_dev, 0, tr);
  if (m->has_cls) IQ_TRY(iq_cls_rows(P + m->cls, m->pe, ws + w.x0, B, S, D, &d0, stream), "cls rows");
  {
    iq_epilogue_t e;
    memset(&e, 0, sizeof(e));
    e.bias = P + m->emb_b; e.pe = m->pe; e.tok = m->tok; e.seq = S; e.cls_off = m->has_cls; e.drop = d0;
    IQ_TRY(iq_gemm_bf16_nt(ws + w.patches, m->Ppad, m->shadow + m->sh_embw, m->Ppad, ws + w.x0, D, MT, D, m->Ppad, &e, stream),
           "embedding GEMM");
  }
  const unsigned char* x = ws + w.x0;
  bool qkv_done = false;
  for (int l = 0; l < c.n_layers; ++l) {
    const LayerOff& o = m->L[l];
    const WsPlan::L& a = w.layers[l];
    iq_epilogue_t e;
    if (!qkv_done) {
      memset(&e, 0, sizeof(e));
      e.bias = P + o.bqkv;
      IQ_TRY(iq_gemm_bf16_nt(x, D, m->sh(o.wqkv), D, ws + a.qkv, 3 * D, M, 3 * D, D, &e, stream), "qkv GEMM");
    }
    qkv_done = false;
    IQ_TRY(iq_attn_fwd(ws + a.qkv, ws + a.att, (float*)(ws + a.lse), B, S, H, m->dh, stream), "attention fwd");
    const iq_dropout_t dr1 = site(m, seed, step_dev, 1 + 3 * l, tr);
    const iq_dropout_t drh = site(m, seed, step_dev, 2 + 3 * l, tr);
    const iq_dropout_t dr2 = site(m, seed, step_dev, 3 + 3 * l, tr);
    if (route.chain) {
      const bool next = l + 1 < c.n_layers;
      IQ_TRY(iq_attn_out_ffn_chain_fwd(ws + a.att, m->sh(o.wo), P + o.bo, &dr1, x, P + o.g1, P + o.be1, ws + a.z1, ws + a.x1,
                                       (float*)(ws + a.mean1), (float*)(ws + a.rstd1), m->sh(o.w1), P + o.b1, &drh, ws + a.hid,
                                       m->sh(o.w2), P + o.b2, &dr2, P + o.g2, P + o.be2, 1e-12f, ws + a.z2, ws + a.x2,
                                       (float*)(ws + a.mean2), (float*)(ws + a.rstd2), ws + a.gate,
                                       next ? m->sh(m->L[l + 1].wqkv) : nullptr, next ? P + m->L[l + 1].bqkv : nullptr,
                                       next ? ws + w.layers[l + 1].qkv : nullptr, B, S, D, F, stream),
             "out-proj + norm1 + ffn chain + norm2 (+ next q,k,v)");
      qkv_done = next;
      x = ws + a.x2;
      continue;
    }
    if (use_fused_ln(D, D)) {
      IQ_TRY(iq_gemm_bf16_ln(ws + a.att, D, m->sh(o.wo), D, P + o.bo, x, D, &dr1, P + o.g1, P + o.be1, 1e-12f, ws + a.z1,
                             ws + a.x1, (float*)(ws + a.mean1), (float*)(ws + a.rstd1), M, D, D, stream), "out-proj GEMM + norm1");
    } else {
      memset(&e, 0, sizeof(e));
      e.bias = P + o.bo; e.drop = dr1; e.residual = x; e.ldr = D;
      IQ_TRY(iq_gemm_bf16_nt(ws + a.att, D, m->sh(o.wo), D, ws + a.z1, D, M, D, D, &e, stream), "out-proj GEMM");
      IQ_TRY(iq_ln_fwd(ws + a.z1, P + o.g1, P + o.be1, ws + a.x1, (float*)(ws + a.mean1), (float*)(ws + a.rstd1), M, D, 1e-12f, stream), "norm1");
    }
    memset(&e, 0, sizeof(e));
    e.bias = P + o.b1; e.relu = 1; e.drop = drh;
    IQ_TRY(iq_gemm_bf16_nt(ws + a.x1, D, m->sh(o.w1), D, ws + a.hid, F, M, F, D, &e, stream), "ffn1 GEMM");
    if (use_fused_ln(D, F)) {
      IQ_TRY(iq_gemm_bf16_ln(ws + a.hid, F, m->sh(o.w2), F, P + o.b2, ws + a.x1, D, &dr2, P + o.g2, P + o.be2, 1e-12f,
                             ws + a.z2, ws + a.x2, (float*)(ws + a.mean2), (float*)(ws + a.rstd2), M, D, F, stream), "ffn2 GEMM + norm2");
    } else {
      memset(&e, 0, sizeof(e));
      e.bias = P + o.b2; e.drop = dr2; e.residual = ws + a.x1; e.ldr = D;
      IQ_TRY(iq_gemm_bf16_nt(ws + a.hid, F, m->sh(o.w2), F, ws + a.z2, D, M, D, F, &e, stream), "ffn2 GEMM");
      IQ_TRY(iq_ln_fwd(ws + a.z2, P + o.g2, P + o.be2, ws + a.x2, (float*)(ws + a.mean2), (float*)(ws + a.rstd2), M, D, 1e-12f, stream), "norm2");
    }
    x = ws + a.x2;
  }
  if (logits) {
    IQ_TRY(iq_head_fwd(x, m->head_ln ? P + m->hln_g : nullptr, m->head_ln ? P + m->hln_b : nullptr, P + m->head_w,
                       P + m->head_b, (float*)(ws + w.head_feat), (float*)(ws + w.head_stat), logits, B, S, D,
                       c.num_classes, m->pool, stream), "head");
  }
  if (enc_out) bf16_to_f32_kernel<<<blocks_for((size_t)M * D / 8), 256, 0, st>>>((const bf16*)x, enc_out, (size_t)M * D / 8);
  const int rc = iq_launch_status();
  if (rc == IQ_OK) { m->fwd_ws = workspace; m->fwd_batch = batch; }
  return rc;
}

static int maps_check(iq_model_t* m, const void* workspace, size_t ws_bytes, int batch, const char* what, WsPlan* w) {
  if (!workspace || batch <= 0) return fail(m, IQ_ERR_ARG, std::string(what) + ": bad arguments");
  if (!m->fwd_ws) return fail(m, IQ_ERR_ARG, std::string(what) + ": no forward has run in a workspace");
  if (m->fwd_ws != workspace) return fail(m, IQ_ERR_ARG, std::string(what) + ": the last forward ran in another workspace");
  if (m->fwd_batch != batch)
    return fail(m, IQ_ERR_ARG, std::string(what) + ": the last forward in this workspace had batch " + std::to_string(m->fwd_batch) +
                                   ", not " + std::to_string(batch));
  *w = plan_ws(m, batch);
  if (ws_bytes < w->total) return fail(m, IQ_ERR_ARG, std::string(what) + ": workspace too small");
  return IQ_OK;
}

extern "C" int iq_model_attention(iq_model_t* m, const void* workspace, size_t ws_bytes, int batch, int layer, int rows,
                                  int heads, float* out, long out_bstride, iq_stream_t stream) {
  if (!m) return IQ_ERR_ARG;
  WsPlan w;
  const int rc = maps_check(m, workspace, ws_bytes, batch, "attention", &w);
  if (rc != IQ_OK) return rc;
  if (layer < 0 || layer >= m->c.n_layers) return fail(m, IQ_ERR_ARG, "attention: layer index out of range");
  if (rows < 0 || rows > 2 || heads < 0 || heads > 1) return fail(m, IQ_ERR_ARG, "attention: rows must be 0, 1 or 2 and heads 0 or 1");
  if (!out) return fail(m, IQ_ERR_ARG, "attention: out is NULL");
  const int S = m->S, H = m->c.n_head;
  if (out_bstride < (long)(heads ? 1 : H) * S * (rows == 0 ? S : 1)) return fail(m, IQ_ERR_ARG, "attention: out_bstride too small");
  const unsigned char* ws = (const unsigned char*)workspace;
  const WsPlan::L& a = w.layers[layer];
  IQ_TRY(iq_attn_probs(ws + a.qkv, (const float*)(ws + a.lse), out, out_bstride, batch, S, H, m->dh, rows, heads, stream),
         "attention probabilities");
  return IQ_OK;
}

extern "C" int iq_model_attention_rollout(iq_model_t* m, const void* workspace, size_t ws_bytes, int batch, float alpha,
                                          float* out, iq_stream_t stream) {
  if (!m) return IQ_ERR_ARG;
  WsPlan w;
  const int rc = maps_check(m, workspace, ws_bytes, batch, "attention rollout", &w);
  if (rc != IQ_OK) return rc;
  if (!(alpha >= 0.f && alpha <= 1.f)) return fail(m, IQ_ERR_ARG, "attention rollout: alpha must be in [0, 1]");
  if (!out) return fail(m, IQ_ERR_ARG, "attention rollout: out is NULL");
  const unsigned char* ws = (const unsigned char*)workspace;
  const int L = m->c.n_layers;
  const long qs = L > 1 ? (long)(w.layers[1].qkv - w.layers[0].qkv) : 0, ls = L > 1 ? (long)(w.layers[1].lse - w.layers[0].lse) : 0;
  for (int l = 0; l < L; ++l)
    if ((long)(w.layers[l].qkv - w.layers[0].qkv) != l * qs || (long)(w.layers[l].lse - w.layers[0].lse) != l * ls)
      return fail(m, IQ_ERR_UNSUPPORTED, "attention rollout: workspace layers are not evenly spaced");
  const size_t q0 = L ? w.layers[0].qkv : 0, l0 = L ? w.layers[0].lse : 0;
  IQ_TRY(attn_rollout_launch(ws + q0, qs, ws + l0, ls, L, out, batch, m->S, m->c.n_head, m->dh, m->has_cls, alpha,
                             (hipStream_t)stream),
         "attention rollout");
  return IQ_OK;
}

extern "C" int iq_model_grad_range(const iq_model_t* m, int stage_hi, int stage_lo, size_t* off, size_t* len) {
  if (!m || !off || !len) return IQ_ERR_ARG;
  const int Lr = m->c.n_layers;
  if (stage_lo < 0 || stage_hi > Lr + 1 || stage_lo > stage_hi) return IQ_ERR_ARG;
  auto begin = [&](int s) { return s == 0 ? (size_t)0 : (s <= Lr ? (s == 1 ? m->emb_end : m->L[s - 2].end) : m->head_begin); };
  auto end = [&](int s) { return s == 0 ? m->emb_end : (s <= Lr ? m->L[s - 1].end : m->nparam); };
  *off = begin(stage_lo);
  *len = end(stage_hi) - *off;
  return IQ_OK;
}

static int backward_impl(iq_model_t* m, const float* dlogits, const float* denc, int batch, void* workspace, size_t ws_bytes,
                         int accumulate, int stage_hi, int stage_lo, bool pgrads, iq_stream_t stream,
                         const RelHook* rh = nullptr) {
  if (!m->params || (pgrads && !m->grads) || !m->shadow) return fail(m, IQ_ERR_ARG, "backward: model not bound (grads required)");
  if (!workspace || batch <= 0) return fail(m, IQ_ERR_ARG, "backward: bad arguments");
  const iq_model_cfg_t& c = m->c;
  const int Lr = c.n_layers;
  if (stage_lo < 0 || stage_hi > Lr + 1 || stage_lo > stage_hi) return fail(m, IQ_ERR_ARG, "backward: bad stage range");
  const WsPlan w = plan_ws(m, batch);
  if (ws_bytes < w.total) return fail(m, IQ_ERR_ARG, "backward: workspace too small");
  hipStream_t st = (hipStream_t)stream;
  unsigned char* ws = (unsigned char*)workspace;
  const int D = c.d_model, F = c.ffn_hidden, S = m->S, H = c.n_head, B = batch, K = c.num_classes;
  const int M = B * S, MT = B * m->tok;
  const bool tr = m->last_tr;
  const uint32_t* step_dev = m->step_ctr ? m->step_ctr : (const uint32_t*)(ws + w.step_ctr);
  const float* P = m->params;
  float* G = m->grads;
  float* wws = (float*)(ws + w.wgrad_ws);
  const float dscale = tr ? dropout_scale(c.drop_prob) : 1.f;

  if (stage_hi == Lr + 1) {
    if (!dlogits && !denc) return fail(m, IQ_ERR_ARG, "backward: dlogits or denc required at the head stage");
    if (dlogits && !pgrads) {
      IQ_TRY(head_bwd_dx_launch(dlogits, (const float*)(ws + w.head_feat), (const float*)(ws + w.head_stat),
                                m->head_ln ? P + m->hln_g : nullptr, P + m->head_w, ws + w.gA, B, S, D, K, m->pool, st), "head bwd (dx)");
    } else if (dlogits) {
      IQ_TRY(iq_head_bwd(dlogits, (const float*)(ws + w.head_feat), (const float*)(ws + w.head_stat),
                         m->head_ln ? P + m->hln_g : nullptr, m->head_ln ? P + m->hln_b : nullptr, P + m->head_w,
                         G + m->head_w, G + m->head_b, m->head_ln ? G + m->hln_g : nullptr,
                         m->head_ln ? G + m->hln_b : nullptr, ws + w.gA, B, S, D, K, m->pool, accumulate, stream), "head bwd");
    } else if (!accumulate && pgrads) {
      (void)hipMemsetAsync(G + m->head_begin, 0, (m->nparam - m->head_begin) * sizeof(float), st);
    }
    if (denc) f32_into_bf16_kernel<<<blocks_for((size_t)M * D / 8), 256, 0, st>>>(denc, (bf16*)(ws + w.gA), (size_t)M * D / 8, dlogits ? 1 : 0);
  }
  const bool fuse1 = iq_gemm_lnbwd_supported(D, F) != 0, fuse2 = iq_gemm_lnbwd_supported(D, 3 * D) != 0;
  const Route route = layer_route(M, S, D, F);
  const bool chain = fuse1 && m->last_train_fwd && route.chain;
  bool deferred = false;
  for (int sidx = (stage_hi > Lr ? Lr : stage_hi); sidx >= 1 && sidx >= stage_lo; --sidx) {
    const int l = sidx - 1;
    const LayerOff& o = m->L[l];
    const WsPlan::L& a = w.layers[l];
    const unsigned char* xin = l == 0 ? ws + w.x0 : ws + w.layers[l - 1].x2;
    unsigned char *gZ = ws + w.gZ, *gY = ws + w.gY, *gZ1 = ws + w.gZ1, *gY1 = ws + w.gY1;
    unsigned char *gH = ws + w.gH, *gQKV = ws + w.gQKV;
    iq_epilogue_t e;
    auto ln2_part = [&](int layer) { return (float*)(ws + w.ln_part[(layer & 1) ? 2 : 0]); };
    float* lp2 = ln2_part(l);
    float* lp1 = (float*)(ws + w.ln_part[1]);
    const bool norm2_here = l == Lr - 1 || !fuse2;
    if (norm2_here) {
      const iq_dropout_t dr2 = m->bwd_site(3 + 3 * l, step_dev, tr);
      IQ_TRY(iq_ln_bwd(ws + w.gA, ws + a.z2, (const float*)(ws + a.mean2), (const float*)(ws + a.rstd2), P + o.g2,
                       gZ, gY, &dr2, nullptr, nullptr, lp2, accumulate, M, D, stream), "norm2 bwd");
    }
    const unsigned char* dO2 = tr ? gY : gZ;
    const unsigned char* dAo = tr ? gY1 : gZ1;
    const iq_wgrad_problem_t wg[4] = {
        {dO2, D, ws + a.hid, F, G + o.w2, G + o.b2, D, F},
        {gH, F, ws + a.x1, D, G + o.w1, G + o.b1, F, D},
        {dAo, D, ws + a.att, D, G + o.wo, G + o.bo, D, D},
        {gQKV, 3 * D, xin, D, G + o.wqkv, G + o.bqkv, 3 * D, D}};
    const int rows2 = norm2_here ? iq_ln_bwd_partial_rows(M, D) : deferred ? iq_ffn_chain_bwd_partial_rows(M) : iq_gemm_lnbwd_partial_rows(M);
    const int rows1 = chain ? iq_ffn_chain_bwd_partial_rows(M) : fuse1 ? iq_gemm_lnbwd_partial_rows(M) : iq_ln_bwd_partial_rows(M, D);
    const iq_reduce_seg_t lnseg[4] = {{lp2, rows2, 2L * D, G + o.g2, D}, {lp2 + D, rows2, 2L * D, G + o.be2, D},
                                      {lp1, rows1, 2L * D, G + o.g1, D}, {lp1 + D, rows1, 2L * D, G + o.be1, D}};
    const iq_dropout_t dr1 = m->bwd_site(1 + 3 * l, step_dev, tr);
    if (chain && deferred) {
      const LayerOff& ou = m->L[l + 1];
      const iq_dropout_t dr2b = m->bwd_site(3 + 3 * l, step_dev, tr);
      IQ_TRY(iq_qkv_dgrad_ffn_chain_bwd(gQKV, m->sht(ou.t_wqkv), gZ1, ws + a.z2, (const float*)(ws + a.mean2), (const float*)(ws + a.rstd2),
                                        P + o.g2, &dr2b, gZ, gY, lp2, m->sht(o.t_w2), ws + a.gate, dscale, gH, m->sht(o.t_w1), gZ, ws + a.z1,
                                        (const float*)(ws + a.mean1), (const float*)(ws + a.rstd1), P + o.g1, &dr1, gZ1, gY1, lp1,
                                        m->sht(o.t_wo), ws + w.gAtt, B, S, D, F, stream),
             "qkv dgrad of the layer above + norm2 bwd + ffn chain bwd + norm1 bwd + out-proj dgrad");
    } else if (chain) {
      IQ_TRY(iq_ffn_chain_bwd(dO2, m->sht(o.t_w2), ws + a.gate, dscale, gH, m->sht(o.t_w1), gZ, ws + a.z1, (const float*)(ws + a.mean1),
                              (const float*)(ws + a.rstd1), P + o.g1, &dr1, gZ1, gY1, lp1, m->sht(o.t_wo), ws + w.gAtt, B, S, D, F, stream),
             "ffn chain bwd + norm1 bwd + out-proj dgrad");
    } else {
      memset(&e, 0, sizeof(e));
      e.gate = ws + a.hid; e.ldg = F; e.gate_scale = dscale;
      IQ_TRY(iq_gemm_bf16_nt(dO2, D, m->sht(o.t_w2), D, gH, F, M, F, D, &e, stream), "ffn2 dgrad");
      if (fuse1) {
        IQ_TRY(iq_gemm_bf16_lnbwd(gH, F, m->sht(o.t_w1), F, gZ, D, ws + a.z1, (const float*)(ws + a.mean1),
                                  (const float*)(ws + a.rstd1), P + o.g1, &dr1, gZ1, gY1, lp1, M, D, F, stream), "ffn1 dgrad + norm1 bwd");
      } else {
        memset(&e, 0, sizeof(e));
        e.residual = gZ; e.ldr = D;
        IQ_TRY(iq_gemm_bf16_nt(gH, F, m->sht(o.t_w1), F, ws + w.gB, D, M, D, F, &e, stream), "ffn1 dgrad");
        IQ_TRY(iq_ln_bwd(ws + w.gB, ws + a.z1, (const float*)(ws + a.mean1), (const float*)(ws + a.rstd1), P + o.g1,
                         gZ1, gY1, &dr1, nullptr, nullptr, lp1, accumulate, M, D, stream), "norm1 bwd");
      }
    }
    if (!chain) IQ_TRY(iq_gemm_bf16_nt(dAo, D, m->sht(o.t_wo), D, ws + w.gAtt, D, M, D, D, nullptr, stream), "out-proj dgrad");
    if (rh) {
      const float* lse = (const float*)(ws + a.lse);
      if (rh->maps && rh->maps[l])
        IQ_TRY(iq_attn_grad_probs(ws + a.qkv, lse, ws + w.gAtt, rh->maps[l], rh->bstride, B, S, H, m->dh, rh->rows, rh->heads,
                                  rh->positive, stream), "gradient-weighted attention map");
      if (rh->rel) {
        const int i = Lr - 1 - l;
        IQ_TRY(attn_relevance_step_launch(ws + a.qkv, lse, ws + w.gAtt, i ? rh->r[(i - 1) & 1] : nullptr, l ? rh->r[i & 1] : rh->rel,
                                          B, S, H, m->dh, i ? 0 : m->has_cls ? 1 : 2, st), "relevance step");
      }
      if (l == 0) break;
    }
    IQ_TRY(iq_attn_bwd(ws + a.qkv, ws + a.att, ws + w.gAtt, (const float*)(ws + a.lse), gQKV, B, S, H, m->dh, stream), "attention bwd");
    deferred = l > 0 && fuse2 && chain && route.chain_takes_qkv_dgrad && sidx - 1 >= stage_lo;
    const bool ride = pgrads && l > 0 && fuse2 && !deferred;
    iq_reduce_job_t job;
    if (ride) {
      IQ_TRY(iq_gemm_bf16_wgrad_grouped_deferred(wg, 4, M, wws, w.wgrad_ws_bytes, accumulate, 0, lnseg, 4, &job, stream),
             "layer weight gradients (partial tiles)");
    } else if (pgrads) {
      IQ_TRY(iq_gemm_bf16_wgrad_grouped(wg, 4, M, wws, w.wgrad_ws_bytes, accumulate, 0, lnseg, 4, stream), "layer weight gradients");
    }
    if (deferred) continue;
    if (l > 0 && fuse2) {
      const LayerOff& ob = m->L[l - 1];
      const WsPlan::L& ab = w.layers[l - 1];
      const iq_dropout_t dr2b = m->bwd_site(3 + 3 * (l - 1), step_dev, tr);
      IQ_TRY(iq_gemm_bf16_lnbwd_ride(gQKV, 3 * D, m->sht(o.t_wqkv), 3 * D, gZ1, D, ws + ab.z2, (const float*)(ws + ab.mean2),
                                     (const float*)(ws + ab.rstd2), P + ob.g2, &dr2b, gZ, gY, ln2_part(l - 1), M, D, 3 * D,
                                     ride ? &job : nullptr, stream),
             "qkv dgrad + norm2 bwd of the layer below (+ this layer's slab reduce)");
    } else {
      memset(&e, 0, sizeof(e));
      e.residual = gZ1; e.ldr = D;
      IQ_TRY(iq_gemm_bf16_nt(gQKV, 3 * D, m->sht(o.t_wqkv), 3 * D, ws + w.gA, D, M, D, 3 * D, &e, stream), "qkv dgrad");
    }
  }
  if (stage_lo == 0) {
    const iq_dropout_t dr0 = m->bwd_site(0, step_dev, tr);
    if (!pgrads) {
      IQ_TRY(embed_bwd_gather_launch(ws + w.gA, ws + w.demb, B, S, m->tok, D, m->has_cls, &dr0, st), "embedding bwd gather");
      return iq_launch_status();
    }
    IQ_TRY(iq_embed_bwd_gather(ws + w.gA, ws + w.demb, m->has_cls ? G + m->cls : nullptr, B, S, m->tok, D, m->has_cls,
                               &dr0, accumulate, stream), "embedding bwd gather");
    if (m->Ppad == m->P) {
      IQ_TRY(iq_gemm_bf16_wgrad(ws + w.demb, D, ws + w.patches, m->Ppad, G + m->emb_w, G + m->emb_b, MT, D, m->Ppad, wws,
                                w.wgrad_ws_bytes, accumulate, stream), "embedding wgrad");
    } else {
      float* scratch = (float*)(ws + w.embw_scratch);
      if (accumulate) (void)hipMemsetAsync(scratch, 0, (size_t)D * m->Ppad * sizeof(float), st);
      IQ_TRY(iq_gemm_bf16_wgrad(ws + w.demb, D, ws + w.patches, m->Ppad, scratch, G + m->emb_b, MT, D, m->Ppad, wws,
                                w.wgrad_ws_bytes, accumulate, stream), "embedding wgrad");
      unpad_kernel<<<blocks_for((size_t)D * m->P), 256, 0, st>>>(scratch, G + m->emb_w, D, m->P, m->Ppad, accumulate);
    }
  }
  return iq_launch_status();
}

extern "C" int iq_model_backward(iq_model_t* m, const float* dlogits, const float* denc, int batch, void* workspace,
                                 size_t ws_bytes, int accumulate, int stage_hi, int stage_lo, iq_stream_t stream) {
  if (!m) return IQ_ERR_ARG;
  return backward_impl(m, dlogits, denc, batch, workspace, ws_bytes, accumulate, stage_hi, stage_lo, true, stream);
}

extern "C" int iq_model_backward_input(iq_model_t* m, const float* dlogits, const float* denc, int batch, void* workspace,
                                       size_t ws_bytes, float* dsrc, int flags, iq_stream_t stream) {
  if (!m) return IQ_ERR_ARG;
  if (flags & ~IQ_BWD_PARAM_GRADS) return fail(m, IQ_ERR_ARG, "backward_input: unknown flags");
  if (!dsrc) return fail(m, IQ_ERR_ARG, "backward_input: dsrc is NULL");
  if (!dlogits && !denc) return fail(m, IQ_ERR_ARG, "backward_input: dlogits or denc required");
  const bool pgrads = (flags & IQ_BWD_PARAM_GRADS) != 0;
  if (!m->params || !m->shadow || !m->pe) return fail(m, IQ_ERR_ARG, "backward_input: model not bound");
  if (pgrads && !m->grads) return fail(m, IQ_ERR_ARG, "backward_input: IQ_BWD_PARAM_GRADS needs a bound gradient buffer");
  WsPlan w;
  const int rc = maps_check(m, workspace, ws_bytes, batch, "backward_input", &w);
  if (rc != IQ_OK) return rc;
  const int rb = backward_impl(m, dlogits, denc, batch, workspace, ws_bytes, 0, m->c.n_layers + 1, 0, pgrads, stream);
  if (rb != IQ_OK) return rb;
  const iq_model_cfg_t& c = m->c;
  unsigned char* ws = (unsigned char*)workspace;
  const int kind = c.kind, H = kind == 0 ? c.img_h : c.seq_length, W = kind == 0 ? c.img_w : 0, p = kind == 0 ? c.patch : c.conv_k;
  IQ_TRY(iq_embed_dgrad(ws + w.demb, m->shadow + m->sh_embw, m->Ppad, dsrc, kind, batch, c.in_channels, H, W, p, c.d_model, stream),
         "embedding data gradient");
  return IQ_OK;
}

extern "C" int iq_model_attention_relevance(iq_model_t* m, const float* dlogits, int batch, void* workspace, size_t ws_bytes,
                                            float* rel, float* const* maps, int rows, int heads, int positive, long out_bstride,
                                            iq_stream_t stream) {
  if (!m) return IQ_ERR_ARG;
  if (!m->params || !m->shadow || !m->pe) return fail(m, IQ_ERR_ARG, "attention relevance: model not bound");
  if (!dlogits) return fail(m, IQ_ERR_ARG, "attention relevance: dlogits is NULL");
  WsPlan w;
  const int rc = maps_check(m, workspace, ws_bytes, batch, "attention relevance", &w);
  if (rc != IQ_OK) return rc;
  if (rows < 0 || rows > 2 || heads < 0 || heads > 1)
    return fail(m, IQ_ERR_ARG, "attention relevance: rows must be 0, 1 or 2 and heads 0 or 1");
  if (positive < 0 || positive > 1) return fail(m, IQ_ERR_ARG, "attention relevance: positive must be 0 or 1");
  const int L = m->c.n_layers, S = m->S, H = m->c.n_head;
  bool any_map = false;
  for (int l = 0; maps && l < L; ++l) any_map = any_map || maps[l];
  if (!rel && !any_map) return fail(m, IQ_ERR_ARG, "attention relevance: rel and every map are NULL");
  if (any_map && out_bstride < (long)(heads ? 1 : H) * S * (rows == 0 ? S : 1))
    return fail(m, IQ_ERR_ARG, "attention relevance: out_bstride too small");
  RelHook h;
  h.maps = maps; h.rows = rows; h.heads = heads; h.positive = positive; h.bstride = out_bstride; h.rel = rel;
  h.r[0] = (float*)((unsigned char*)workspace + w.demb);
  h.r[1] = h.r[0] + (size_t)batch * S;
  if (2 * (size_t)batch * S * sizeof(float) > (size_t)batch * m->tok * m->c.d_model * 2)
    return fail(m, IQ_ERR_UNSUPPORTED, "attention relevance: no room for the relevance vectors");
  if (L == 0) {
    if (rel) rel_start_kernel<<<blocks_for((size_t)batch * S), 256, 0, (hipStream_t)stream>>>(rel, batch * S, S, m->has_cls);
    return iq_launch_status() == IQ_OK ? IQ_OK : fail(m, IQ_ERR_LAUNCH, "attention relevance: start vector launch failed");
  }
  return backward_impl(m, dlogits, nullptr, batch, workspace, ws_bytes, 0, L + 1, 1, false, stream, &h);
}
```

Measured before the change: 55090 frames/s.

## Prebuild swizzled weight ring images so chain kernels stream contiguous slots

```diff
diff --git a/include/iqvit.h b/include/iqvit.h
--- a/include/iqvit.h
+++ b/include/iqvit.h
@@ -77,6 +77,34 @@
                               const iq_dropout_t* drop2, const float* gamma2, const float* beta2, float eps, void* Z2, void* X,
                               float* mean2, float* rstd2, void* gate_bits, const void* Wq, const float* bq, void* Yq, int frames,
                               int S, int D, int F, iq_stream_t stream);
+
+enum { IQ_CHAIN_IMG_FFN = 0, IQ_CHAIN_IMG_ROWS = 1, IQ_CHAIN_IMG_QKV = 2, IQ_CHAIN_IMG_QKVT = 3 };
+typedef struct iq_chain_image_job {
+  const void* src1; const void* src2; void* dst;
+  int kind, n;
+  int block0, reserved;
+} iq_chain_image_job_t;
+size_t iq_chain_image_bytes(int kind, int D, int n);
+int iq_chain_images_build(const iq_chain_image_job_t* jobs_dev, int njobs, int nblocks, int D, iq_stream_t stream);
+int iq_ffn_chain_bwd_img(const void* dO, const void* W21t, const void* gate_bits, float gate_scale, void* gH,
+                         const void* residual, const void* z1, const float* mean, const float* rstd, const float* gamma,
+                         const iq_dropout_t* drop, void* dz, void* dy, float* partial, const void* Wot, void* dA, int frames, int S,
+                         int D, int F, iq_stream_t stream);
+int iq_qkv_dgrad_ffn_chain_bwd_img(const void* gQKV, const void* Wqkv_t, const void* residual0, const void* z2, const float* mean2,
+                                   const float* rstd2, const float* gamma2, const iq_dropout_t* drop2, void* dz2, void* dy2,
+                                   float* partial2, const void* W21t, const void* gate_bits, float gate_scale, void* gH,
+                                   const void* residual, const void* z1, const float* mean, const float* rstd, const float* gamma,
+                                   const iq_dropout_t* drop, void* dz, void* dy, float* partial, const void* Wot, void* dA, int frames,
+                                   int S, int D, int F, iq_stream_t stream);
+int iq_ffn_chain_fwd_img(const void* X1, const void* W12, const float* b1, const iq_dropout_t* drop1, void* H, const float* b2,
+                         const iq_dropout_t* drop2, const float* gamma, const float* beta, float eps, void* Z, void* X, float* mean,
+                         float* rstd, void* gate_bits, int frames, int S, int D, int F, iq_stream_t stream);
+int iq_attn_out_ffn_chain_fwd_img(const void* A, const void* Wo, const float* bo, const iq_dropout_t* drop0, const void* R,
+                                  const float* gamma1, const float* beta1, void* Z1, void* X1, float* mean1, float* rstd1,
+                                  const void* W12, const float* b1, const iq_dropout_t* drop1, void* H, const float* b2,
+                                  const iq_dropout_t* drop2, const float* gamma2, const float* beta2, float eps, void* Z2, void* X,
+                                  float* mean2, float* rstd2, void* gate_bits, const void* Wq, const float* bq, void* Yq, int frames,
+                                  int S, int D, int F, iq_stream_t stream);
 
 size_t iq_wgrad_ws_bytes(int M, int N, int K);
 int iq_gemm_bf16_wgrad(const void* dY, int ldy, const void* X, int ldx, float* dW, float* dbias, int M, int N, int K,
diff --git a/vit-vs-raw-iq_amd/_native.py b/vit-vs-raw-iq_amd/_native.py
--- a/vit-vs-raw-iq_amd/_native.py
+++ b/vit-vs-raw-iq_amd/_native.py
@@ -116,6 +116,14 @@
 
 class ReduceJob(C.Structure):
     _fields_ = [("seg", ReduceJobSeg * 12), ("nseg", C.c_int), ("nblk", C.c_int), ("accumulate", C.c_int)]
+
+
+class ChainImageJob(C.Structure):
+    _fields_ = [("src1", C.c_void_p), ("src2", C.c_void_p), ("dst", C.c_void_p), ("kind", C.c_int), ("n", C.c_int),
+                ("block0", C.c_int), ("reserved", C.c_int)]
+
+
+CHAIN_IMG_FFN, CHAIN_IMG_ROWS, CHAIN_IMG_QKV, CHAIN_IMG_QKVT = 0, 1, 2, 3
 
 
 class ModelCfg(C.Structure):
@@ -151,6 +159,16 @@
     "iq_attn_out_ffn_chain_fwd": (_I, [_P, _P, _P, C.POINTER(Dropout), _P, _P, _P, _P, _P, _P, _P,
                                        _P, _P, C.POINTER(Dropout), _P, _P, _P, C.POINTER(Dropout), _P, _P, _F, _P, _P, _P, _P, _P,
                                        _P, _P, _P, _I, _I, _I, _I, _P]),
+    "iq_chain_image_bytes": (_Z, [_I, _I, _I]),
+    "iq_chain_images_build": (_I, [_P, _I, _I, _I, _P]),
+    "iq_ffn_chain_bwd_img": (_I, [_P, _P, _P, _F, _P, _P, _P, _P, _P, _P, C.POINTER(Dropout), _P, _P, _P, _P, _P, _I, _I, _I, _I, _P]),
+    "iq_qkv_dgrad_ffn_chain_bwd_img": (_I, [_P, _P, _P, _P, _P, _P, _P, C.POINTER(Dropout), _P, _P, _P,
+                                            _P, _P, _F, _P, _P, _P, _P, _P, _P, C.POINTER(Dropout), _P, _P, _P, _P, _P, _I, _I, _I, _I, _P]),
+    "iq_ffn_chain_fwd_img": (_I, [_P, _P, _P, C.POINTER(Dropout), _P, _P, C.POINTER(Dropout), _P, _P, _F, _P, _P, _P, _P, _P, _I, _I,
+                                  _I, _I, _P]),
+    "iq_attn_out_ffn_chain_fwd_img": (_I, [_P, _P, _P, C.POINTER(Dropout), _P, _P, _P, _P, _P, _P, _P,
+                                           _P, _P, C.POINTER(Dropout), _P, _P, C.POINTER(Dropout), _P, _P, _F, _P, _P, _P, _P, _P,
+                                           _P, _P, _P, _I, _I, _I, _I, _P]),
     "iq_wgrad_ws_bytes": (_Z, [_I, _I, _I]),
     "iq_gemm_bf16_wgrad": (_I, [_P, _I, _P, _I, _P, _P, _I, _I, _I, _P, _Z, _I, _P]),
     "iq_wgrad_grouped_ws_bytes": (_Z, [_P, _I, _I, _I]),
diff --git a/vit-vs-raw-iq_amd/csrc/ffn_chain.hip b/vit-vs-raw-iq_amd/csrc/ffn_chain.hip
--- a/vit-vs-raw-iq_amd/csrc/ffn_chain.hip
+++ b/vit-vs-raw-iq_amd/csrc/ffn_chain.hip
@@ -1,6 +1,9 @@
 #include <stdlib.h>
 
+#include <map>
+#include <mutex>
 #include <type_traits>
+#include <utility>
 
 #include "common.h"
 #include "iqvit.h"
@@ -11,17 +14,17 @@
 constexpr int FC_CHUNK = 64, FC_NS = 3, FC_MAXW = 7;
 
 struct FfnChainParams {
-  const bf16* X1; const bf16* W1; const bf16* W2;
+  const bf16* X1; const void* W12;
   const float* b1; const float* b2; const float* gamma; const float* beta;
   bf16* H; bf16* Z; bf16* X; float* mean; float* rstd;
   uint32_t* gate;
   int M, F;
   float eps;
   int drop1_on, drop2_on; IqRng rng1, rng2; uint32_t thresh1, thresh2; float dscale1, dscale2;
-  const bf16* A0; const bf16* W0; const bf16* R0; const float* b0; const float* gamma0; const float* beta0;
+  const bf16* A0; const void* W0; const bf16* R0; const float* b0; const float* gamma0; const float* beta0;
   bf16* Z0; bf16* X1out; float* mean0; float* rstd0;
   int drop0_on; IqRng rng0; uint32_t thresh0; float dscale0;
-  const bf16* Wq; const float* bq; bf16* Yq;
+  const void* Wq; const float* bq; bf16* Yq;
 };
 
 template <int CPR> __device__ __forceinline__ int fc_swz(int row, int ch) {
@@ -38,6 +41,17 @@
   } while (0)
 
 __device__ __forceinline__ int fc_kperm(int g) { return ((g & 1) << 1) | (g >> 1); }
+
+template <int XCPR> __device__ __forceinline__ int fc_w1_src(int lin, int& r) {
+  r = lin / XCPR;
+  const int q = fc_swz<XCPR>(r & 63, lin - r * XCPR);
+  return ((q & ~3) | fc_kperm(q & 3)) * 8;
+}
+__device__ __forceinline__ int fc_w2_src(int l2, int& r) {
+  r = l2 >> 3;
+  const int q = fc_swz<8>(r, l2 & 7);
+  return ((q & ~3) | fc_kperm(q & 3)) * 8;
+}
 
 template <int D, int NW, int RG, bool DROP1, int MODE>
 __global__ __launch_bounds__(NW * 64, 2) void ffn_chain_fwd_kernel(const FfnChainParams p) {
@@ -61,65 +75,39 @@
   const long row0 = ((long)blockIdx.x * nwave + wave) * RW;
   const bool have = row0 < p.M;
 
+  unsigned lane4 = (unsigned)lane * 4u;
+  asm volatile("" : "+v"(lane4));
+  auto issue_image = [&](const char* src, unsigned char* dst, auto npc, auto ppw_c) {
+    constexpr int NPC = decltype(npc)::value, N = decltype(ppw_c)::value;
+    unsigned l16 = lane4;
+    asm volatile("" : "+v"(l16));
+    l16 *= 4u;
+#pragma unroll
+    for (int i = 0; i < N; ++i) {
+      const int pc = min(wave + i * NW, NPC - 1);
+      const char* sp = src + pc * 1024;
+      asm volatile("" : "+s"(sp));
+      __builtin_amdgcn_global_load_lds((gbl_cvoid_t*)(sp + l16), (lds_void_t*)(dst + pc * 1024), 16, 0, 0);
+    }
+  };
+  constexpr std::integral_constant<int, PIECES> pieces_c{};
+  constexpr std::integral_constant<int, PPW> ppw_c{};
   auto issue_chunk = [&](int c) {
-    unsigned char* slot = smem + (c % FC_NS) * SLOT;
-    const char* base1 = reinterpret_cast<const char*>(p.W1 + (long)c * FC_CHUNK * D);
-    const char* base2 = reinterpret_cast<const char*>(p.W2 + (long)c * FC_CHUNK);
-    int ln = lane;
-    asm volatile("" : "+v"(ln));
-#pragma unroll
-    for (int i = 0; i < PPW; ++i) {
-      const int pc = min(wave + i * NW, PIECES - 1);
-      const int lin = pc * 64 + ln;
-      unsigned off;
-      if (pc < W1_PIECES) {
-        const int r = lin / XCPR, sl = lin - r * XCPR;
-        const int q = fc_swz<XCPR>(r, sl);
-        off = (unsigned)((r * D + ((q & ~3) | fc_kperm(q & 3)) * 8) * 2);
-      } else {
-        const int l2 = lin - W1_PIECES * 64;
-        const int r = l2 >> 3, sl = l2 & 7;
-        const int q = fc_swz<8>(r, sl);
-        off = (unsigned)((r * F + ((q & ~3) | fc_kperm(q & 3)) * 8) * 2);
-      }
-      const char* base = pc < W1_PIECES ? base1 : base2;
-      __builtin_amdgcn_global_load_lds((gbl_cvoid_t*)(base + off), (lds_void_t*)(slot + pc * 1024), 16, 0, 0);
-    }
+    issue_image(reinterpret_cast<const char*>(p.W12) + (long)c * SLOT, smem + (c % FC_NS) * SLOT, pieces_c, ppw_c);
   };
   constexpr int NBQ = 3 * D / FC_CHUNK, NQ = (NBQ + 1) / 2;
   static_assert(2 * W1_BYTES == SLOT, "two projection blocks fill a ring slot");
   const int ntot = nchunk + (POST ? NQ : 0);
   auto issue_any = [&](int c) {
     if (!POST || c < nchunk) { issue_chunk(c); return; }
-    const int q = c - nchunk;
-    unsigned char* slot = smem + (c % FC_NS) * SLOT;
-    int ln = lane;
-    asm volatile("" : "+v"(ln));
-#pragma unroll
-    for (int i = 0; i < PPW; ++i) {
-      const int pc = min(wave + i * NW, PIECES - 1);
-      const int lin = pc * 64 + ln;
-      const int r = lin / XCPR, sl = lin - r * XCPR;
-      const int qq = fc_swz<XCPR>(r & 63, sl);
-      const int grow = min(q * 2 * FC_CHUNK + r, 3 * D - 1);
-      const unsigned off = (unsigned)((grow * D + ((qq & ~3) | fc_kperm(qq & 3)) * 8) * 2);
-      __builtin_amdgcn_global_load_lds((gbl_cvoid_t*)(reinterpret_cast<const char*>(p.Wq) + off), (lds_void_t*)(slot + pc * 1024), 16, 0, 0);
-    }
+    issue_image(reinterpret_cast<const char*>(p.Wq) + (long)(c - nchunk) * SLOT, smem + (c % FC_NS) * SLOT, pieces_c, ppw_c);
   };
   constexpr int NB0 = D / FC_CHUNK;
   if (PRE) {
     constexpr int PRE_PIECES = NB0 * W1_PIECES, PRE_PPW = (PRE_PIECES + NW - 1) / NW;
     static_assert(NB0 * W1_BYTES <= 2 * SLOT, "projection weight blocks fit ring slots 1 and 2");
-#pragma unroll
-    for (int i = 0; i < PRE_PPW; ++i) {
-      const int pc = min(wave + i * NW, PRE_PIECES - 1);
-      const int lin = pc * 64 + lane;
-      const int r = lin / XCPR, sl = lin - r * XCPR;
-      const int q = fc_swz<XCPR>(r & 63, sl);
-      const unsigned off = (unsigned)((r * D + ((q & ~3) | fc_kperm(q & 3)) * 8) * 2);
-      __builtin_amdgcn_global_load_lds((gbl_cvoid_t*)(reinterpret_cast<const char*>(p.W0) + off),
-                                       (lds_void_t*)(smem + SLOT + pc * 1024), 16, 0, 0);
-    }
+    issue_image(reinterpret_cast<const char*>(p.W0), smem + SLOT, std::integral_constant<int, PRE_PIECES>{},
+                std::integral_constant<int, PRE_PPW>{});
   }
   issue_chunk(0);
   if (!PRE && ntot > 1) issue_any(1);
@@ -255,7 +243,7 @@
         s2 += __shfl_xor(s2, 16, 64);
         s2 += __shfl_xor(s2, 32, 64);
         const float rstd = 1.0f / sqrtf(s2 * invD0 + p.eps);
-        if (g == 0 && grow < p.M) { p.mean0[grow] = mean; p.rstd0[grow] = rstd; }
+        if (lane4 < 64u && grow < p.M) { p.mean0[grow] = mean; p.rstd0[grow] = rstd; }
 #pragma unroll
         for (int jp = 0; jp < KS1; ++jp) {
           const int col = 32 * jp + (odd ? 16 + 4 * (g - 1) : 4 * g);
@@ -363,7 +351,13 @@
       }
     }
     {
-      if (gated) p.gate[((row0 / RW) * nchunk + c) * 64 + lane] = gbits;
+      if (gated) {
+        uint32_t* gp = p.gate + ((row0 / RW) * nchunk + c) * 64;
+        asm volatile("" : "+s"(gp));
+        unsigned l4 = lane4;
+        asm volatile("" : "+v"(l4));
+        *reinterpret_cast<uint32_t*>(reinterpret_cast<char*>(gp) + l4) = gbits;
+      }
     }
     constexpr int NG4 = NT2 / 4, NGRP = 2 * NG4;
     bf16x8 wq[2][4];
@@ -445,7 +439,7 @@
     s2 += __shfl_xor(s2, 32, 64);
     const float rstd = 1.0f / sqrtf(s2 * invD + p.eps);
     if (grow < p.M) {
-      if (g == 0) { p.mean[grow] = mean; p.rstd[grow] = rstd; }
+      if (lane4 < 64u) { p.mean[grow] = mean; p.rstd[grow] = rstd; }
 #pragma unroll
       for (int jp = 0; jp < NP2; ++jp) {
         const int col = 32 * jp + (odd ? 16 + 4 * (g - 1) : 4 * g);
@@ -525,15 +519,15 @@
 }
 
 struct FfnChainBwdParams {
-  const bf16* dO; const bf16* W2t; const bf16* W1t;
+  const bf16* dO; const void* W21t;
   const uint32_t* gate; const bf16* R; const bf16* Z1;
   const float* mean; const float* rstd; const float* gamma;
   bf16* gH; bf16* dZ; bf16* dY; float* partial;
   int M, F;
   float gate_scale;
   int drop_on; IqRng rng; uint32_t thresh; float dscale;
-  const bf16* Wot; bf16* dA;
-  const bf16* A0; const bf16* W0t; const bf16* R0; const bf16* Z0; const float* mean0; const float* rstd0; const float* gamma0;
+  const void* Wot; bf16* dA;
+  const bf16* A0; const void* W0t; const bf16* R0; const bf16* Z0; const float* mean0; const float* rstd0; const float* gamma0;
   IqRng rng0; bf16* dZ0; bf16* dY0; float* partial0;
 };
 
@@ -558,28 +552,24 @@
   const bool have = row0 < p.M;
   const bool full = row0 + RW <= p.M;
 
+  const uint32_t lane4 = (uint32_t)lane * 4u;
+  auto issue_image = [&](const char* src, unsigned char* dst, auto npc, auto ppw_c) {
+    constexpr int NPC = decltype(npc)::value, N = decltype(ppw_c)::value;
+    unsigned l16 = lane4;
+    asm volatile("" : "+v"(l16));
+    l16 *= 4u;
+#pragma unroll
+    for (int i = 0; i < N; ++i) {
+      const int pc = min(wave + i * NW, NPC - 1);
+      const char* sp = src + pc * 1024;
+      asm volatile("" : "+s"(sp));
+      __builtin_amdgcn_global_load_lds((gbl_cvoid_t*)(sp + l16), (lds_void_t*)(dst + pc * 1024), 16, 0, 0);
+    }
+  };
+  constexpr std::integral_constant<int, PIECES> pieces_c{};
+  constexpr std::integral_constant<int, PPW> ppw_c{};
   auto issue_chunk = [&](int c) {
-    unsigned char* slot = smem + (c % FC_NS) * SLOT;
-    const char* base1 = reinterpret_cast<const char*>(p.W2t + (long)c * FC_CHUNK * D);
-    const char* base2 = reinterpret_cast<const char*>(p.W1t + (long)c * FC_CHUNK);
-#pragma unroll
-    for (int i = 0; i < PPW; ++i) {
-      const int pc = min(wave + i * NW, PIECES - 1);
-      const int lin = pc * 64 + lane;
-      unsigned off;
-      if (pc < W1_PIECES) {
-        const int r = lin / XCPR, sl = lin - r * XCPR;
-        const int q = fc_swz<XCPR>(r, sl);
-        off = (unsigned)((r * D + ((q & ~3) | fc_kperm(q & 3)) * 8) * 2);
-      } else {
-        const int l2 = lin - W1_PIECES * 64;
-        const int r = l2 >> 3, sl = l2 & 7;
-        const int q = fc_swz<8>(r, sl);
-        off = (unsigned)((r * F + ((q & ~3) | fc_kperm(q & 3)) * 8) * 2);
-      }
-      const char* base = pc < W1_PIECES ? base1 : base2;
-      __builtin_amdgcn_global_load_lds((gbl_cvoid_t*)(base + off), (lds_void_t*)(slot + pc * 1024), 16, 0, 0);
-    }
+    issue_image(reinterpret_cast<const char*>(p.W21t) + (long)c * SLOT, smem + (c % FC_NS) * SLOT, pieces_c, ppw_c);
   };
   long rowc[RG];
 #pragma unroll
@@ -758,7 +748,6 @@
     }
   };
   const uint32_t* gate_wave = p.gate + (row0 / RW) * nchunk * 64;
-  const uint32_t lane4 = (uint32_t)lane * 4u;
   uint32_t gnext;
   auto load_gate = [&](int c) {
     const uint32_t* src = gate_wave + c * 64;
@@ -770,20 +759,7 @@
   if (PREB) {
     constexpr int K0 = 3 * D, NC0 = K0 / FC_CHUNK, NQ0 = (NC0 + 1) / 2;
     auto issue_pre = [&](int i) {
-      unsigned char* slot = smem + (i % FC_NS) * SLOT;
-      int ln = lane;
-      asm volatile("" : "+v"(ln));
-#pragma unroll
-      for (int k = 0; k < PPW; ++k) {
-        const int pc = min(wave + k * NW, PIECES - 1);
-        const int h = pc >= W1_PIECES ? 1 : 0;
-        const int l2 = (pc - h * W1_PIECES) * 64 + ln;
-        const int r = l2 >> 3, sl = l2 & 7;
-        const int q = fc_swz<8>(r, sl);
-        const int col = min((2 * i + h) * FC_CHUNK, K0 - FC_CHUNK) + ((q & ~3) | fc_kperm(q & 3)) * 8;
-        const unsigned off = (unsigned)((r * K0 + col) * 2);
-        __builtin_amdgcn_global_load_lds((gbl_cvoid_t*)(reinterpret_cast<const char*>(p.W0t) + off), (lds_void_t*)(slot + pc * 1024), 16, 0, 0);
-      }
+      issue_image(reinterpret_cast<const char*>(p.W0t) + (long)i * SLOT, smem + (i % FC_NS) * SLOT, pieces_c, ppw_c);
     };
     bf16x8 aF[2][2][RG][2];
     auto load_a = [&](int i) {
@@ -926,13 +902,10 @@
   constexpr int NB0 = D / FC_CHUNK;
   auto issue_wot = [&](int b0, int nb, unsigned char* dst) {
     const int pieces = nb * W1_PIECES;
-    for (int pc = wave; pc < pieces; pc += NW) {
-      const int lin = pc * 64 + lane;
-      const int r = lin / XCPR, sl = lin - r * XCPR;
-      const int q = fc_swz<XCPR>(r & 63, sl);
-      const unsigned off = (unsigned)(((b0 * FC_CHUNK + r) * D + ((q & ~3) | fc_kperm(q & 3)) * 8) * 2);
-      __builtin_amdgcn_global_load_lds((gbl_cvoid_t*)(reinterpret_cast<const char*>(p.Wot) + off), (lds_void_t*)(dst + pc * 1024), 16, 0, 0);
-    }
+    const char* src = reinterpret_cast<const char*>(p.Wot) + b0 * W1_BYTES;
+    const unsigned l16 = lane4 * 4u;
+    for (int pc = wave; pc < pieces; pc += NW)
+      __builtin_amdgcn_global_load_lds((gbl_cvoid_t*)(src + pc * 1024 + l16), (lds_void_t*)(dst + pc * 1024), 16, 0, 0);
   };
   if (POSTB) {
     __syncthreads();
@@ -993,6 +966,51 @@
       }
     }
   }
+}
+
+template <int D>
+__device__ __forceinline__ void chain_image_block(const iq_chain_image_job_t& j, int block) {
+  constexpr int XCPR = D / 8, BLK = FC_CHUNK * D * 2 / 16;
+  static_assert(BLK % 256 == 0, "whole blocks per image");
+  const int lin = block * 256 + (int)threadIdx.x;
+  const bf16* s1 = reinterpret_cast<const bf16*>(j.src1);
+  const bf16* src;
+  int r;
+  if (j.kind == IQ_CHAIN_IMG_FFN) {
+    const int c = lin / (2 * BLK), l = lin - c * (2 * BLK);
+    if (l < BLK) {
+      const int col = fc_w1_src<XCPR>(l, r);
+      src = s1 + ((long)c * FC_CHUNK + r) * D + col;
+    } else {
+      const int col = fc_w2_src(l - BLK, r);
+      src = reinterpret_cast<const bf16*>(j.src2) + (long)r * j.n + c * FC_CHUNK + col;
+    }
+  } else if (j.kind == IQ_CHAIN_IMG_QKVT) {
+    const int h = lin / BLK;
+    const int col = fc_w2_src(lin - h * BLK, r);
+    src = s1 + (long)r * j.n + min(h * FC_CHUNK, j.n - FC_CHUNK) + col;
+  } else {
+    const int col = fc_w1_src<XCPR>(lin, r);
+    src = s1 + (long)min(r, j.n - 1) * D + col;
+  }
+  reinterpret_cast<bf16x8*>(j.dst)[lin] = *reinterpret_cast<const bf16x8*>(src);
+}
+template <int D>
+__global__ __launch_bounds__(256) void chain_image_table_kernel(const iq_chain_image_job_t* __restrict__ tab, int njobs) {
+  int lo = 0, hi = njobs - 1;
+  while (lo < hi) {
+    const int mid = (lo + hi + 1) >> 1;
+    if ((int)blockIdx.x >= tab[mid].block0) lo = mid; else hi = mid - 1;
+  }
+  const iq_chain_image_job_t j = tab[lo];
+  chain_image_block<D>(j, (int)blockIdx.x - j.block0);
+}
+struct ChainImageArgs { iq_chain_image_job_t j[3]; int n; };
+template <int D>
+__global__ __launch_bounds__(256) void chain_image_args_kernel(const ChainImageArgs a) {
+  const int b = (int)blockIdx.x;
+  const iq_chain_image_job_t j = (a.n > 2 && b >= a.j[2].block0) ? a.j[2] : (a.n > 1 && b >= a.j[1].block0) ? a.j[1] : a.j[0];
+  chain_image_block<D>(j, b - j.block0);
 }
 
 struct ChainShape { int rg, nw; };
@@ -1063,7 +1081,71 @@
   return (size_t)FC_NS * 2 * FC_CHUNK * D * 2 + ((size_t)F + 9 * D) * sizeof(float) <= (size_t)160 * 1024 ? 1 : 0;
 }
 
+extern "C" size_t iq_chain_image_bytes(int kind, int D, int n) {
+  if (!(D == 128 || D == 192) || n <= 0 || (n % FC_CHUNK)) return 0;
+  const size_t blk = (size_t)FC_CHUNK * D * 2;
+  switch (kind) {
+    case IQ_CHAIN_IMG_FFN: return (size_t)(n / FC_CHUNK) * 2 * blk;
+    case IQ_CHAIN_IMG_ROWS: return (size_t)(n / FC_CHUNK) * blk;
+    case IQ_CHAIN_IMG_QKV:
+    case IQ_CHAIN_IMG_QKVT: return n == 3 * D ? (size_t)((n / FC_CHUNK + 1) / 2) * 2 * blk : 0;
+    default: return 0;
+  }
+}
+
+extern "C" int iq_chain_images_build(const iq_chain_image_job_t* jobs_dev, int njobs, int nblocks, int D, iq_stream_t stream) {
+  if (njobs <= 0 || nblocks <= 0) return IQ_OK;
+  if (!jobs_dev || ((uintptr_t)jobs_dev % 8)) return IQ_ERR_ARG;
+  if (!(D == 128 || D == 192)) return IQ_ERR_UNSUPPORTED;
+  hipStream_t st = (hipStream_t)stream;
+  IQ_PROF(IQ_FAM_MISC, st);
+  if (D == 192) chain_image_table_kernel<192><<<nblocks, 256, 0, st>>>(jobs_dev, njobs);
+  else chain_image_table_kernel<128><<<nblocks, 256, 0, st>>>(jobs_dev, njobs);
+  return iq_launch_status();
+}
+
 namespace {
+struct ImageScratch {
+  std::mutex mu;
+  std::map<std::pair<int, hipStream_t>, std::pair<void*, size_t>> buf;
+};
+void* image_scratch(hipStream_t st, size_t bytes) {
+  static ImageScratch* sc = new ImageScratch();
+  int dev = 0;
+  if (hipGetDevice(&dev) != hipSuccess) return nullptr;
+  std::lock_guard<std::mutex> lock(sc->mu);
+  auto& b = sc->buf[std::make_pair(dev, st)];
+  if (b.second >= bytes) return b.first;
+  hipStreamCaptureStatus cap = hipStreamCaptureStatusNone;
+  if (hipStreamIsCapturing(st, &cap) != hipSuccess || cap != hipStreamCaptureStatusNone) return nullptr;
+  if (b.first) (void)hipFree(b.first);
+  b.first = nullptr; b.second = 0;
+  if (hipMalloc(&b.first, bytes) != hipSuccess) { b.first = nullptr; return nullptr; }
+  b.second = bytes;
+  return b.first;
+}
+int build_scratch_images(iq_chain_image_job_t* jobs, int n, int D, hipStream_t st, const void** img) {
+  size_t total = 0;
+  ChainImageArgs a = {};
+  a.n = n;
+  for (int k = 0; k < n; ++k) {
+    const size_t bytes = iq_chain_image_bytes(jobs[k].kind, D, jobs[k].n);
+    if (!bytes) return IQ_ERR_UNSUPPORTED;
+    jobs[k].block0 = (int)(total / 4096);
+    total += bytes;
+  }
+  unsigned char* base = (unsigned char*)image_scratch(st, total);
+  if (!base) return IQ_ERR_UNSUPPORTED;
+  for (int k = 0; k < n; ++k) {
+    jobs[k].dst = base + (size_t)jobs[k].block0 * 4096;
+    img[k] = jobs[k].dst;
+    a.j[k] = jobs[k];
+  }
+  if (D == 192) chain_image_args_kernel<192><<<(int)(total / 4096), 256, 0, st>>>(a);
+  else chain_image_args_kernel<128><<<(int)(total / 4096), 256, 0, st>>>(a);
+  return iq_launch_status();
+}
+
 struct ChainPre {
   const void* A0; const void* W0; const float* b0; const iq_dropout_t* drop0; const void* R0;
   const float* gamma0; const float* beta0; void* Z0; float* mean0; float* rstd0;
@@ -1072,15 +1154,15 @@
 
 int chain_fwd(const ChainPre* pre, const void* X1, const void* W1, const float* b1, const iq_dropout_t* drop1, void* H, const void* W2,
               const float* b2, const iq_dropout_t* drop2, const float* gamma, const float* beta, float eps, void* Z, void* X,
-              float* mean, float* rstd, void* gate_bits, int frames, int S, int D, int F, iq_stream_t stream) {
+              float* mean, float* rstd, void* gate_bits, int frames, int S, int D, int F, iq_stream_t stream, bool imaged) {
   if (frames <= 0) return IQ_OK;
-  if (!X1 || !W1 || !b1 || !H || !W2 || !b2 || !gamma || !beta || !Z || !X || !mean || !rstd) return IQ_ERR_ARG;
+  if (!X1 || !W1 || !b1 || !H || (!imaged && !W2) || !b2 || !gamma || !beta || !Z || !X || !mean || !rstd) return IQ_ERR_ARG;
   if (!iq_ffn_chain_supported(S, D, F)) return IQ_ERR_UNSUPPORTED;
   if (((uintptr_t)X1 | (uintptr_t)W1 | (uintptr_t)W2 | (uintptr_t)H | (uintptr_t)Z | (uintptr_t)X | (uintptr_t)b1 | (uintptr_t)b2 |
        (uintptr_t)gamma | (uintptr_t)beta) % 16) return IQ_ERR_ARG;
   if ((long)frames * S > 0x7FFFFFFFL) return IQ_ERR_UNSUPPORTED;
   FfnChainParams p = {};
-  p.X1 = (const bf16*)X1; p.W1 = (const bf16*)W1; p.W2 = (const bf16*)W2;
+  p.X1 = (const bf16*)X1; p.W12 = W1;
   p.b1 = b1; p.b2 = b2; p.gamma = gamma; p.beta = beta;
   p.H = (bf16*)H; p.Z = (bf16*)Z; p.X = (bf16*)X; p.mean = mean; p.rstd = rstd;
   p.gate = (uint32_t*)gate_bits;
@@ -1093,15 +1175,28 @@
       return IQ_ERR_ARG;
     if (((uintptr_t)pre->A0 | (uintptr_t)pre->W0 | (uintptr_t)pre->b0 | (uintptr_t)pre->R0 | (uintptr_t)pre->gamma0 |
          (uintptr_t)pre->beta0 | (uintptr_t)pre->Z0) % 16) return IQ_ERR_ARG;
-    p.A0 = (const bf16*)pre->A0; p.W0 = (const bf16*)pre->W0; p.R0 = (const bf16*)pre->R0; p.b0 = pre->b0;
+    p.A0 = (const bf16*)pre->A0; p.W0 = pre->W0; p.R0 = (const bf16*)pre->R0; p.b0 = pre->b0;
     p.gamma0 = pre->gamma0; p.beta0 = pre->beta0; p.Z0 = (bf16*)pre->Z0; p.X1out = (bf16*)X1; p.mean0 = pre->mean0; p.rstd0 = pre->rstd0;
     if (!dropout_unpack(pre->drop0, &p.drop0_on, &p.rng0, &p.thresh0, &p.dscale0)) return IQ_ERR_ARG;
     if (pre->Wq || pre->bq || pre->Yq) {
       if (!pre->Wq || !pre->bq || !pre->Yq || ((uintptr_t)pre->Wq | (uintptr_t)pre->bq | (uintptr_t)pre->Yq) % 16) return IQ_ERR_ARG;
-      p.Wq = (const bf16*)pre->Wq; p.bq = pre->bq; p.Yq = (bf16*)pre->Yq;
+      p.Wq = pre->Wq; p.bq = pre->bq; p.Yq = (bf16*)pre->Yq;
     }
   }
   hipStream_t st = (hipStream_t)stream;
+  if (!imaged) {
+    iq_chain_image_job_t jobs[3] = {};
+    const void* img[3];
+    int n = 0;
+    jobs[n].kind = IQ_CHAIN_IMG_FFN; jobs[n].src1 = W1; jobs[n].src2 = W2; jobs[n].n = F; ++n;
+    if (pre) { jobs[n].kind = IQ_CHAIN_IMG_ROWS; jobs[n].src1 = pre->W0; jobs[n].n = D; ++n; }
+    if (p.Wq) { jobs[n].kind = IQ_CHAIN_IMG_QKV; jobs[n].src1 = pre->Wq; jobs[n].n = 3 * D; ++n; }
+    const int rc = build_scratch_images(jobs, n, D, st, img);
+    if (rc != IQ_OK) return rc;
+    p.W12 = img[0];
+    if (pre) p.W0 = img[1];
+    if (p.Wq) p.Wq = img[2];
+  }
   IQ_PROF(IQ_FAM_GEMM_NT, st);
   const double M = (double)p.M;
   double more_bytes = 0.0, more_flops = 0.0;
@@ -1117,7 +1212,14 @@
                                 const void* W2, const float* b2, const iq_dropout_t* drop2, const float* gamma,
                                 const float* beta, float eps, void* Z, void* X, float* mean, float* rstd, void* gate_bits,
                                 int frames, int S, int D, int F, iq_stream_t stream) {
-  return chain_fwd(nullptr, X1, W1, b1, drop1, H, W2, b2, drop2, gamma, beta, eps, Z, X, mean, rstd, gate_bits, frames, S, D, F, stream);
+  return chain_fwd(nullptr, X1, W1, b1, drop1, H, W2, b2, drop2, gamma, beta, eps, Z, X, mean, rstd, gate_bits, frames, S, D, F, stream,
+                   false);
+}
+extern "C" int iq_ffn_chain_fwd_img(const void* X1, const void* W12, const float* b1, const iq_dropout_t* drop1, void* H, const float* b2,
+                                    const iq_dropout_t* drop2, const float* gamma, const float* beta, float eps, void* Z, void* X,
+                                    float* mean, float* rstd, void* gate_bits, int frames, int S, int D, int F, iq_stream_t stream) {
+  return chain_fwd(nullptr, X1, W12, b1, drop1, H, nullptr, b2, drop2, gamma, beta, eps, Z, X, mean, rstd, gate_bits, frames, S, D, F,
+                   stream, true);
 }
 
 extern "C" int iq_attn_out_ffn_chain_fwd(const void* A, const void* Wo, const float* bo, const iq_dropout_t* drop0, const void* R,
@@ -1127,7 +1229,18 @@
                                          void* Z2, void* X, float* mean2, float* rstd2, void* gate_bits, const void* Wq,
                                          const float* bq, void* Yq, int frames, int S, int D, int F, iq_stream_t stream) {
   const ChainPre pre = {A, Wo, bo, drop0, R, gamma1, beta1, Z1, mean1, rstd1, Wq, bq, Yq};
-  return chain_fwd(&pre, X1, W1, b1, drop1, H, W2, b2, drop2, gamma2, beta2, eps, Z2, X, mean2, rstd2, gate_bits, frames, S, D, F, stream);
+  return chain_fwd(&pre, X1, W1, b1, drop1, H, W2, b2, drop2, gamma2, beta2, eps, Z2, X, mean2, rstd2, gate_bits, frames, S, D, F, stream,
+                   false);
+}
+extern "C" int iq_attn_out_ffn_chain_fwd_img(const void* A, const void* Wo, const float* bo, const iq_dropout_t* drop0, const void* R,
+                                             const float* gamma1, const float* beta1, void* Z1, void* X1, float* mean1, float* rstd1,
+                                             const void* W12, const float* b1, const iq_dropout_t* drop1, void* H, const float* b2,
+                                             const iq_dropout_t* drop2, const float* gamma2, const float* beta2, float eps, void* Z2,
+                                             void* X, float* mean2, float* rstd2, void* gate_bits, const void* Wq, const float* bq,
+                                             void* Yq, int frames, int S, int D, int F, iq_stream_t stream) {
+  const ChainPre pre = {A, Wo, bo, drop0, R, gamma1, beta1, Z1, mean1, rstd1, Wq, bq, Yq};
+  return chain_fwd(&pre, X1, W12, b1, drop1, H, nullptr, b2, drop2, gamma2, beta2, eps, Z2, X, mean2, rstd2, gate_bits, frames, S, D, F,
+                   stream, true);
 }
 
 extern "C" int iq_ffn_chain_bwd_partial_rows(int M) {
@@ -1149,21 +1262,22 @@
 
 int chain_bwd(const ChainBwdPre* pre, const void* dO, const void* W2t, const void* gate_bits, float gate_scale, void* gH, const void* W1t,
               const void* residual, const void* z1, const float* mean, const float* rstd, const float* gamma, const iq_dropout_t* drop,
-              void* dz, void* dy, float* partial, const void* Wot, void* dA, int frames, int S, int D, int F, iq_stream_t stream) {
+              void* dz, void* dy, float* partial, const void* Wot, void* dA, int frames, int S, int D, int F, iq_stream_t stream,
+              bool imaged) {
   if (frames <= 0) return IQ_OK;
   if ((Wot == nullptr) != (dA == nullptr) || ((uintptr_t)Wot | (uintptr_t)dA) % 16) return IQ_ERR_ARG;
-  if ((!pre && !dO) || !W2t || !gate_bits || !gH || !W1t || !residual || !z1 || !mean || !rstd || !gamma || !dz || !partial) return IQ_ERR_ARG;
+  if ((!pre && !dO) || !W2t || !gate_bits || !gH || (!imaged && !W1t) || !residual || !z1 || !mean || !rstd || !gamma || !dz || !partial) return IQ_ERR_ARG;
   if (!iq_ffn_chain_supported(S, D, F)) return IQ_ERR_UNSUPPORTED;
   if (((uintptr_t)dO | (uintptr_t)W2t | (uintptr_t)W1t | (uintptr_t)gate_bits | (uintptr_t)gH | (uintptr_t)residual | (uintptr_t)z1 |
        (uintptr_t)dz | (uintptr_t)dy | (uintptr_t)gamma | (uintptr_t)partial) % 16) return IQ_ERR_ARG;
   if ((long)frames * S > 0x7FFFFFFFL) return IQ_ERR_UNSUPPORTED;
   FfnChainBwdParams p = {};
-  p.dO = (const bf16*)dO; p.W2t = (const bf16*)W2t; p.W1t = (const bf16*)W1t;
+  p.dO = (const bf16*)dO; p.W21t = W2t;
   p.gate = (const uint32_t*)gate_bits; p.R = (const bf16*)residual; p.Z1 = (const bf16*)z1;
   p.mean = mean; p.rstd = rstd; p.gamma = gamma;
   p.gH = (bf16*)gH; p.dZ = (bf16*)dz; p.dY = (bf16*)dy; p.partial = partial;
   p.M = frames * S; p.F = F; p.gate_scale = gate_scale;
-  p.Wot = (const bf16*)Wot; p.dA = (bf16*)dA;
+  p.Wot = Wot; p.dA = (bf16*)dA;
   if (!dropout_unpack(drop, &p.drop_on, &p.rng, &p.thresh, &p.dscale) || (p.drop_on && !dy)) return IQ_ERR_ARG;
   if (pre) {
     if (!Wot) return IQ_ERR_ARG;
@@ -1173,13 +1287,26 @@
          (uintptr_t)pre->dZ0 | (uintptr_t)pre->dY0 | (uintptr_t)pre->partial0) % 16) return IQ_ERR_ARG;
     const float p0 = pre->drop0 ? pre->drop0->p : 0.f, p1 = drop ? drop->p : 0.f;
     if (p0 != p1 || (p.drop_on && !pre->dY0)) return IQ_ERR_ARG;
-    p.A0 = (const bf16*)pre->A0; p.W0t = (const bf16*)pre->W0t; p.R0 = (const bf16*)pre->R0; p.Z0 = (const bf16*)pre->Z0;
+    p.A0 = (const bf16*)pre->A0; p.W0t = pre->W0t; p.R0 = (const bf16*)pre->R0; p.Z0 = (const bf16*)pre->Z0;
     p.mean0 = pre->mean0; p.rstd0 = pre->rstd0; p.gamma0 = pre->gamma0;
     p.dZ0 = (bf16*)pre->dZ0; p.dY0 = (bf16*)pre->dY0; p.partial0 = pre->partial0;
     int on0; uint32_t thresh0; float dscale0;
     (void)dropout_unpack(pre->drop0, &on0, &p.rng0, &thresh0, &dscale0);
   }
   hipStream_t st = (hipStream_t)stream;
+  if (!imaged) {
+    iq_chain_image_job_t jobs[3] = {};
+    const void* img[3];
+    int n = 0;
+    jobs[n].kind = IQ_CHAIN_IMG_FFN; jobs[n].src1 = W2t; jobs[n].src2 = W1t; jobs[n].n = F; ++n;
+    if (Wot) { jobs[n].kind = IQ_CHAIN_IMG_ROWS; jobs[n].src1 = Wot; jobs[n].n = D; ++n; }
+    if (pre) { jobs[n].kind = IQ_CHAIN_IMG_QKVT; jobs[n].src1 = pre->W0t; jobs[n].n = 3 * D; ++n; }
+    const int rc = build_scratch_images(jobs, n, D, st, img);
+    if (rc != IQ_OK) return rc;
+    p.W21t = img[0];
+    if (Wot) p.Wot = img[1];
+    if (pre) p.W0t = img[2];
+  }
   IQ_PROF(IQ_FAM_GEMM_NT, st);
   const double M = (double)p.M;
   double bytes = 2.0 * (M * D * (4 + (p.drop_on ? 1 : 0) + (Wot ? 1 : 0)) + 2.0 * M * F + 2.0 * D * F + (Wot ? (double)D * D : 0.0)) + 8.0 * M;
@@ -1198,7 +1325,14 @@
                                 const iq_dropout_t* drop, void* dz, void* dy, float* partial, const void* Wot, void* dA, int frames,
                                 int S, int D, int F, iq_stream_t stream) {
   return chain_bwd(nullptr, dO, W2t, gate_bits, gate_scale, gH, W1t, residual, z1, mean, rstd, gamma, drop, dz, dy, partial, Wot, dA,
-                   frames, S, D, F, stream);
+                   frames, S, D, F, stream, false);
+}
+extern "C" int iq_ffn_chain_bwd_img(const void* dO, const void* W21t, const void* gate_bits, float gate_scale, void* gH,
+                                    const void* residual, const void* z1, const float* mean, const float* rstd, const float* gamma,
+                                    const iq_dropout_t* drop, void* dz, void* dy, float* partial, const void* Wot, void* dA, int frames,
+                                    int S, int D, int F, iq_stream_t stream) {
+  return chain_bwd(nullptr, dO, W21t, gate_bits, gate_scale, gH, nullptr, residual, z1, mean, rstd, gamma, drop, dz, dy, partial, Wot, dA,
+                   frames, S, D, F, stream, true);
 }
 
 extern "C" int iq_qkv_dgrad_ffn_chain_bwd(const void* gQKV, const void* Wqkv_t, const void* residual0, const void* z2, const float* mean2,
@@ -1209,5 +1343,16 @@
                                           void* dA, int frames, int S, int D, int F, iq_stream_t stream) {
   const ChainBwdPre pre = {gQKV, Wqkv_t, residual0, z2, mean2, rstd2, gamma2, drop2, dz2, dy2, partial2};
   return chain_bwd(&pre, nullptr, W2t, gate_bits, gate_scale, gH, W1t, residual, z1, mean, rstd, gamma, drop, dz, dy, partial, Wot, dA,
-                   frames, S, D, F, stream);
-}
+                   frames, S, D, F, stream, false);
+}
+extern "C" int iq_qkv_dgrad_ffn_chain_bwd_img(const void* gQKV, const void* Wqkv_t, const void* residual0, const void* z2,
+                                              const float* mean2, const float* rstd2, const float* gamma2, const iq_dropout_t* drop2,
+                                              void* dz2, void* dy2, float* partial2, const void* W21t, const void* gate_bits,
+                                              float gate_scale, void* gH, const void* residual, const void* z1, const float* mean,
+                                              const float* rstd, const float* gamma, const iq_dropout_t* drop, void* dz, void* dy,
+                                              float* partial, const void* Wot, void* dA, int frames, int S, int D, int F,
+                                              iq_stream_t stream) {
+  const ChainBwdPre pre = {gQKV, Wqkv_t, residual0, z2, mean2, rstd2, gamma2, drop2, dz2, dy2, partial2};
+  return chain_bwd(&pre, nullptr, W21t, gate_bits, gate_scale, gH, nullptr, residual, z1, mean, rstd, gamma, drop, dz, dy, partial, Wot, dA,
+                   frames, S, D, F, stream, true);
+}
diff --git a/vit-vs-raw-iq_amd/csrc/model.hip b/vit-vs-raw-iq_amd/csrc/model.hip
--- a/vit-vs-raw-iq_amd/csrc/model.hip
+++ b/vit-vs-raw-iq_amd/csrc/model.hip
@@ -27,6 +27,7 @@
 struct LayerOff {
   size_t wqkv, bqkv, wo, bo, g1, be1, w1, b1, w2, b2, g2, be2, end;
   size_t t_wqkv, t_wo, t_w1, t_w2;
+  size_t i_ffn, i_wo, i_wqkv, i_ffn_t, i_wo_t, i_wqkv_t;
 };
 
 inline size_t align_up(size_t v, size_t a) { return (v + a - 1) / a * a; }
@@ -138,6 +139,10 @@
   size_t sh_flat, sh_embw, sh_table, shadow_bytes;
   std::vector<TransDesc> ttab;
   int ttiles = 0;
+  bool images = false;
+  std::vector<iq_chain_image_job_t> ijobs;
+  int iblocks = 0;
+  size_t sh_ijobs = 0;
   const void* table_uploaded_to = nullptr;
   float* params = nullptr;
   float* grads = nullptr;
@@ -372,6 +377,32 @@
     push(o.w2, o.t_w2, D, F);
   }
   m->sh_table = sb; sb = align_up(sb + m->ttab.size() * sizeof(TransDesc) + 64, 256);
+  m->images = iq_ffn_chain_supported(m->S, D, F) != 0;
+  if (m->images) {
+    auto image = [&](int kind, size_t src1, size_t src2, int n) {
+      iq_chain_image_job_t j;
+      memset(&j, 0, sizeof(j));
+      const size_t bytes = iq_chain_image_bytes(kind, D, n);
+      j.kind = kind; j.n = n; j.src1 = (const void*)src1; j.src2 = (const void*)src2; j.dst = (void*)sb;
+      j.block0 = m->iblocks;
+      m->iblocks += (int)(bytes / 4096);
+      m->ijobs.push_back(j);
+      const size_t at = sb;
+      sb = align_up(sb + bytes, 256);
+      return at;
+    };
+    auto flat = [&](size_t off) { return m->sh_flat + off * 2; };
+    for (int i = 0; i < c.n_layers; ++i) {
+      LayerOff& o = m->L[i];
+      o.i_ffn = image(IQ_CHAIN_IMG_FFN, flat(o.w1), flat(o.w2), F);
+      o.i_wo = image(IQ_CHAIN_IMG_ROWS, flat(o.wo), 0, D);
+      o.i_wqkv = i ? image(IQ_CHAIN_IMG_QKV, flat(o.wqkv), 0, 3 * D) : 0;
+      o.i_ffn_t = image(IQ_CHAIN_IMG_FFN, o.t_w2, o.t_w1, F);
+      o.i_wo_t = image(IQ_CHAIN_IMG_ROWS, o.t_wo, 0, D);
+      o.i_wqkv_t = i ? image(IQ_CHAIN_IMG_QKVT, o.t_wqkv, 0, 3 * D) : 0;
+    }
+    m->sh_ijobs = sb; sb = align_up(sb + m->ijobs.size() * sizeof(iq_chain_image_job_t) + 64, 256);
+  }
   m->shadow_bytes = sb;
   *out = m;
   return IQ_OK;
@@ -410,6 +441,16 @@
   if (m->table_uploaded_to != shadow && !m->ttab.empty()) {
     if (hipMemcpy(m->shadow + m->sh_table, m->ttab.data(), m->ttab.size() * sizeof(TransDesc), hipMemcpyHostToDevice) != hipSuccess)
       return fail(m, IQ_ERR_LAUNCH, "bind: uploading the transpose table failed");
+    if (!m->ijobs.empty()) {
+      std::vector<iq_chain_image_job_t> jobs = m->ijobs;
+      for (auto& j : jobs) {
+        j.src1 = m->shadow + (size_t)j.src1;
+        j.src2 = j.kind == IQ_CHAIN_IMG_FFN ? m->shadow + (size_t)j.src2 : nullptr;
+        j.dst = m->shadow + (size_t)j.dst;
+      }
+      if (hipMemcpy(m->shadow + m->sh_ijobs, jobs.data(), jobs.size() * sizeof(iq_chain_image_job_t), hipMemcpyHostToDevice) != hipSuccess)
+        return fail(m, IQ_ERR_LAUNCH, "bind: uploading the image table failed");
+    }
     m->table_uploaded_to = shadow;
   }
   return IQ_OK;
@@ -433,6 +474,9 @@
   if (m->ttiles > 0)
     transpose_table_kernel<<<m->ttiles, 256, 0, st>>>(m->params, m->shadow, (const TransDesc*)(m->shadow + m->sh_table),
                                                      (int)m->ttab.size());
+  if (m->images)
+    IQ_TRY(iq_chain_images_build((const iq_chain_image_job_t*)(m->shadow + m->sh_ijobs), (int)m->ijobs.size(), m->iblocks, D, stream),
+           "ring images");
   return iq_launch_status();
 }
 
@@ -494,12 +538,12 @@
     const iq_dropout_t dr2 = site(m, seed, step_dev, 3 + 3 * l, tr);
     if (route.chain) {
       const bool next = l + 1 < c.n_layers;
-      IQ_TRY(iq_attn_out_ffn_chain_fwd(ws + a.att, m->sh(o.wo), P + o.bo, &dr1, x, P + o.g1, P + o.be1, ws + a.z1, ws + a.x1,
-                                       (float*)(ws + a.mean1), (float*)(ws + a.rstd1), m->sh(o.w1), P + o.b1, &drh, ws + a.hid,
-                                       m->sh(o.w2), P + o.b2, &dr2, P + o.g2, P + o.be2, 1e-12f, ws + a.z2, ws + a.x2,
-                                       (float*)(ws + a.mean2), (float*)(ws + a.rstd2), ws + a.gate,
-                                       next ? m->sh(m->L[l + 1].wqkv) : nullptr, next ? P + m->L[l + 1].bqkv : nullptr,
-                                       next ? ws + w.layers[l + 1].qkv : nullptr, B, S, D, F, stream),
+      IQ_TRY(iq_attn_out_ffn_chain_fwd_img(ws + a.att, m->sht(o.i_wo), P + o.bo, &dr1, x, P + o.g1, P + o.be1, ws + a.z1, ws + a.x1,
+                                           (float*)(ws + a.mean1), (float*)(ws + a.rstd1), m->sht(o.i_ffn), P + o.b1, &drh, ws + a.hid,
+                                           P + o.b2, &dr2, P + o.g2, P + o.be2, 1e-12f, ws + a.z2, ws + a.x2,
+                                           (float*)(ws + a.mean2), (float*)(ws + a.rstd2), ws + a.gate,
+                                           next ? m->sht(m->L[l + 1].i_wqkv) : nullptr, next ? P + m->L[l + 1].bqkv : nullptr,
+                                           next ? ws + w.layers[l + 1].qkv : nullptr, B, S, D, F, stream),
              "out-proj + norm1 + ffn chain + norm2 (+ next q,k,v)");
       qkv_done = next;
       x = ws + a.x2;
@@ -673,14 +717,14 @@
     if (chain && deferred) {
       const LayerOff& ou = m->L[l + 1];
       const iq_dropout_t dr2b = m->bwd_site(3 + 3 * l, step_dev, tr);
-      IQ_TRY(iq_qkv_dgrad_ffn_chain_bwd(gQKV, m->sht(ou.t_wqkv), gZ1, ws + a.z2, (const float*)(ws + a.mean2), (const float*)(ws + a.rstd2),
-                                        P + o.g2, &dr2b, gZ, gY, lp2, m->sht(o.t_w2), ws + a.gate, dscale, gH, m->sht(o.t_w1), gZ, ws + a.z1,
-                                        (const float*)(ws + a.mean1), (const float*)(ws + a.rstd1), P + o.g1, &dr1, gZ1, gY1, lp1,
-                                        m->sht(o.t_wo), ws + w.gAtt, B, S, D, F, stream),
+      IQ_TRY(iq_qkv_dgrad_ffn_chain_bwd_img(gQKV, m->sht(ou.i_wqkv_t), gZ1, ws + a.z2, (const float*)(ws + a.mean2),
+                                            (const float*)(ws + a.rstd2), P + o.g2, &dr2b, gZ, gY, lp2, m->sht(o.i_ffn_t), ws + a.gate, dscale,
+                                            gH, gZ, ws + a.z1, (const float*)(ws + a.mean1), (const float*)(ws + a.rstd1), P + o.g1, &dr1,
+                                            gZ1, gY1, lp1, m->sht(o.i_wo_t), ws + w.gAtt, B, S, D, F, stream),
              "qkv dgrad of the layer above + norm2 bwd + ffn chain bwd + norm1 bwd + out-proj dgrad");
     } else if (chain) {
-      IQ_TRY(iq_ffn_chain_bwd(dO2, m->sht(o.t_w2), ws + a.gate, dscale, gH, m->sht(o.t_w1), gZ, ws + a.z1, (const float*)(ws + a.mean1),
-                              (const float*)(ws + a.rstd1), P + o.g1, &dr1, gZ1, gY1, lp1, m->sht(o.t_wo), ws + w.gAtt, B, S, D, F, stream),
+      IQ_TRY(iq_ffn_chain_bwd_img(dO2, m->sht(o.i_ffn_t), ws + a.gate, dscale, gH, gZ, ws + a.z1, (const float*)(ws + a.mean1),
+                                  (const float*)(ws + a.rstd1), P + o.g1, &dr1, gZ1, gY1, lp1, m->sht(o.i_wo_t), ws + w.gAtt, B, S, D, F, stream),
              "ffn chain bwd + norm1 bwd + out-proj dgrad");
     } else {
       memset(&e, 0, sizeof(e));
```

Measured after the change: 55160 frames/s, median of 2. Within noise of the previous version (+0.1%).
